# PacificBiosciences/pb-StarPhase

Measured on AMD Instinct MI355X. Metric: HiFi reads/sec diplotyped (HLA+CYP2D6), higher is better.
Workload: dtype int32; 1 GPU; BASELINE configs[1] + configs[2] as ONE sample per step: HLA-A/-B 10000 HiFi reads vs IMGT/HLA v0.14.1 (11,199 DNA alleles) + CYP2D6 2000 targeted reads (39 templates), the six configs[2] scenarios in turn; a new sample uploaded every step; reads -> diplotypes; hla_reads=10000, cyp2d6_reads=2000, cyp2d6_lanes=6, hla_lanes=2, cyp2d6_consensus=launch pairs

## Files before the change

pb-starphase_amd/csrc/sp_api.hip:

```cpp
#include "sp_internal.h"
#include <algorithm>
#include <thread>
#include <atomic>
#include <cstring>
#include <new>
#include <unistd.h>

extern "C" {

int32_t sp_abi_version(void) { return SP_ABI_VERSION; }

int32_t sp_device_count(int32_t* count) {
    int n = 0;
    hipError_t e = hipGetDeviceCount(&n);
    if (count) *count = (e == hipSuccess) ? n : 0;
    return e == hipSuccess ? SP_OK : SP_ERR_NO_DEVICE;
}

int32_t sp_ctx_create(int32_t device, void* stream, sp_ctx** out) {
    if (!out) return SP_ERR_INVALID_ARG;
    *out = nullptr;
    static std::atomic<int> effective{-1};
    bool by_library = false;
    if (effective.load() < 0) {
        bool hip_up = false;
        char link[64];
        for (int fd = 0; fd < 1024 && !hip_up; ++fd) {
            char path[64]; std::snprintf(path, sizeof path, "/proc/self/fd/%d", fd);
            const ssize_t k = readlink(path, link, sizeof link - 1);
            if (k > 0) { link[k] = 0; hip_up = std::strcmp(link, "/dev/kfd") == 0; }
        }
        const char* had = std::getenv("GPU_MAX_HW_QUEUES");
        if (!had && !hip_up) { (void)setenv("GPU_MAX_HW_QUEUES", "16", 0); by_library = true; }
        const char* now = std::getenv("GPU_MAX_HW_QUEUES");
        effective.store(now ? std::atoi(now) : (hip_up ? 0 : 4));
    }
    const int hw_queues = effective.load() > 0 ? effective.load() : 4;
    int n = 0;
    if (hipGetDeviceCount(&n) != hipSuccess || n <= 0 || device < 0 || device >= n) return SP_ERR_NO_DEVICE;
    if (hipSetDevice(device) != hipSuccess) return SP_ERR_NO_DEVICE;
    hipDeviceProp_t prop;
    if (hipGetDeviceProperties(&prop, device) != hipSuccess) return SP_ERR_NO_DEVICE;
    if (std::strncmp(prop.gcnArchName, "gfx950", 6) != 0) return SP_ERR_NO_DEVICE;
    sp_ctx* ctx = new (std::nothrow) sp_ctx();
    if (!ctx) return SP_ERR_OUT_OF_MEMORY;
    ctx->device = device;
    ctx->num_cus = prop.multiProcessorCount > 0 ? prop.multiProcessorCount : 256;
    static bool set_here = false;
    if (by_library) set_here = true;
    ctx->hw_queues = hw_queues; ctx->hw_queues_by_library = set_here;
    ctx->hw_queues_effective = effective.load();
    { const char* kc = std::getenv("SP_K8_COMPOUND"); if (kc && *kc) ctx->k8_compound = std::atoi(kc); }
    { const char* ks = std::getenv("SP_K8_SIDE_ORDERS"); if (ks && *ks) ctx->k8_side_orders = std::max(0, std::min(3, std::atoi(ks))); }
    { const char* kp = std::getenv("SP_K8_PERSISTENT"); if (kp && *kp) ctx->k8_persistent = std::atoi(kp); }
    if (effective.load() == 0)
        ctx->warning = "the HIP runtime was initialised before the library's first context and GPU_MAX_HW_QUEUES was not set: the process's streams share the runtime's 4 hardware queues; "
                       "export GPU_MAX_HW_QUEUES=16 (or more) before the process initialises HIP";
    else if (hw_queues < 16)
        ctx->warning = "GPU_MAX_HW_QUEUES=" + std::to_string(hw_queues) + ": the library's streams share " + std::to_string(hw_queues) +
                       " hardware queues; export GPU_MAX_HW_QUEUES=16 (or more) before the process initialises HIP";
    if (stream) { ctx->stream = (hipStream_t)stream; ctx->own_stream = false; }
    else {
        if (hipStreamCreateWithFlags(&ctx->stream, hipStreamNonBlocking) != hipSuccess) { delete ctx; return SP_ERR_HIP; }
        ctx->own_stream = true;
    }
    if (hipEventCreate(&ctx->ev0) != hipSuccess || hipEventCreate(&ctx->ev1) != hipSuccess) { delete ctx; return SP_ERR_HIP; }
    *out = ctx;
    return SP_OK;
}

int32_t sp_ctx_get_info(const sp_ctx* ctx, sp_ctx_info* out) {
    if (!ctx || !out) return SP_ERR_INVALID_ARG;
    std::memset(out, 0, sizeof *out);
    out->device = ctx->device; out->num_cus = ctx->num_cus; out->hw_queues = ctx->hw_queues; out->hw_queues_set_by_library = ctx->hw_queues_by_library ? 1 : 0;
    std::snprintf(out->warning, sizeof out->warning, "%s", ctx->warning.c_str());
    return SP_OK;
}

static int32_t upload_finish(sp_seqset* s);
void sp_ctx_destroy(sp_ctx* ctx) {
    if (!ctx) return;
    for (sp_ctx*& h : ctx->helper) if (h) { sp_ctx_destroy(h); h = nullptr; }
    hipSetDevice(ctx->device);
    if (ctx->uploading) (void)upload_finish(ctx->uploading);
    if (ctx->copy_stream) { hipStreamSynchronize(ctx->copy_stream); hipStreamDestroy(ctx->copy_stream); ctx->copy_stream = nullptr; }
    if (ctx->ctl_stream) { hipStreamSynchronize(ctx->ctl_stream); hipStreamDestroy(ctx->ctl_stream); ctx->ctl_stream = nullptr; }
    if (ctx->ev_fork) hipEventDestroy(ctx->ev_fork);
    if (ctx->ev_join) hipEventDestroy(ctx->ev_join);
    hipStreamSynchronize(ctx->stream);
    for (sp_seqset* s : ctx->live_sets) {
        for (void* p : { (void*)s->d_words, (void*)s->d_nplane, (void*)s->d_word_off, (void*)s->d_len, (void*)s->d_kcode, (void*)s->d_kpos, (void*)s->d_koff }) if (p) ctx->dev_cap.erase(p);
        s->ctx = nullptr;
    }
    for (auto& kv : ctx->dev_cap) (void)hipFree(kv.first);
    if (ctx->scratch) hipFree(ctx->scratch);
    for (auto& kv : ctx->pool) if (kv.second.first) hipFree(kv.second.first);
    for (auto& kv : ctx->host_pool) if (kv.second.first) hipHostFree(kv.second.first);
    sp_profile_flush(ctx);
    for (hipEvent_t e : ctx->prof_free) hipEventDestroy(e);
    if (ctx->ev0) hipEventDestroy(ctx->ev0);
    if (ctx->ev1) hipEventDestroy(ctx->ev1);
    if (ctx->own_stream && ctx->stream) hipStreamDestroy(ctx->stream);
    delete ctx;
}

}
sp_ctx* sp_ctx_helper(sp_ctx* ctx, int i) {
    if (i < 0 || i > 6) return nullptr;
    if (!ctx->helper[i] && sp_ctx_create(ctx->device, nullptr, &ctx->helper[i]) != SP_OK) ctx->helper[i] = nullptr;
    if (ctx->helper[i]) { ctx->helper[i]->profiling = ctx->profiling; ctx->helper[i]->k5_block_pairs = ctx->k5_block_pairs; ctx->helper[i]->k8_persistent = ctx->k8_persistent; ctx->helper[i]->k8_side_orders = ctx->k8_side_orders; ctx->helper[i]->k8_compound = ctx->k8_compound; ctx->helper[i]->k8_side_max_blocks = ctx->k8_side_max_blocks; ctx->helper[i]->mm2_rescore = ctx->mm2_rescore; ctx->helper[i]->profile_rescore_counts = ctx->profile_rescore_counts; ctx->helper[i]->k1_best_n = ctx->k1_best_n; }
    return ctx->helper[i];
}
void sp_profile_merge(sp_ctx* into, sp_ctx* from) {
    sp_profile_flush(from);
    for (auto& kv : from->prof) { ProfileEntry& e = into->prof[kv.first]; e.ms += kv.second.ms; e.launches += kv.second.launches; e.cells += kv.second.cells; }
    from->prof.clear();
}
extern "C" {

int32_t sp_struct_size(const char* name) {
    if (!name) return -1;
#define SP_SZ(T) if (std::strcmp(name, #T) == 0) return (int32_t)sizeof(T);
    SP_SZ(sp_ctx_info)
    SP_SZ(sp_pair)
    SP_SZ(sp_aln)
    SP_SZ(sp_hla_db_desc)
    SP_SZ(sp_hla_realign)
    SP_SZ(sp_k1_seed_hit)
    SP_SZ(sp_hla_best)
    SP_SZ(sp_chain_problem)
    SP_SZ(sp_chain_result)
    SP_SZ(sp_region_hit)
    SP_SZ(sp_cyp_problem)
    SP_SZ(sp_cyp_call)
    SP_SZ(sp_cyp_locus)
    SP_SZ(sp_cyp_gene_def)
    SP_SZ(sp_cyp_config)
    SP_SZ(sp_cyp_db_stats)
    SP_SZ(sp_variant_problem)
    SP_SZ(sp_variant_result)
    SP_SZ(sp_sv_definitions)
    SP_SZ(sp_cons_config)
    SP_SZ(sp_cons_result)
    SP_SZ(sp_cons_problem)
    SP_SZ(sp_cons_output)
    SP_SZ(sp_priority_problem)
    SP_SZ(sp_priority_job)
    SP_SZ(sp_hla_call_config)
    SP_SZ(sp_hla_call)
    SP_SZ(sp_diplotype_settings)
    SP_SZ(sp_sample_inputs)
    SP_SZ(sp_starphase_timing)
    SP_SZ(sp_cyp_read_mapping)
    SP_SZ(sp_database_metadata)
    SP_SZ(sp_database_stats)
    SP_SZ(sp_gene_region)
    SP_SZ(sp_variant_detail)
    SP_SZ(sp_bam_read)
    SP_SZ(sp_affine_opts)
    SP_SZ(sp_affine_aln)
    SP_SZ(sp_k1_seed_info)
    SP_SZ(sp_cyp_region_variants)
    SP_SZ(sp_chain_build_info)
    SP_SZ(sp_variant_gene_stats)
    SP_SZ(sp_vcf_allele)
    SP_SZ(sp_vcf_deletion)
    SP_SZ(sp_mapping_stats)
    SP_SZ(sp_hla_rev_hit)
    SP_SZ(sp_batch_options)
    SP_SZ(sp_starphase_batch_timing)
    SP_SZ(sp_hla_alleles_stats)
    SP_SZ(sp_hla_cfg_mapping)
    SP_SZ(sp_hla_cfg_gene)
    SP_SZ(sp_pileup_col)
    SP_SZ(sp_support_summary)
    SP_SZ(sp_support_entry)
    SP_SZ(sp_pileup_ins)
    SP_SZ(sp_support_hap)
    SP_SZ(sp_support_hap_head)
#undef SP_SZ
    return -1;
}

const char* sp_last_error(const sp_ctx* ctx) { return ctx ? ctx->err.c_str() : "null context"; }

int32_t sp_ctx_synchronize(sp_ctx* ctx) {
    if (!ctx) return SP_ERR_INVALID_ARG;
    SP_HIP_CHECK(ctx, hipStreamSynchronize(ctx->stream));
    return SP_OK;
}

int32_t sp_ctx_set_option(sp_ctx* ctx, const char* name, int64_t value) {
    if (!ctx || !name) return SP_ERR_INVALID_ARG;
    if (std::strcmp(name, "hla_split_genes") == 0) { ctx->split_genes = value != 0; return SP_OK; }
    if (std::strcmp(name, "k1_best_n") == 0) { if (value < 0 || value > 8) return sp_fail(ctx, SP_ERR_INVALID_ARG, "sp_ctx_set_option: k1_best_n is 0..8"); ctx->k1_best_n = (int)value; for (sp_ctx* h : ctx->helper) if (h) h->k1_best_n = ctx->k1_best_n; return SP_OK; }
    if (std::strcmp(name, "profile_rescore_counts") == 0) { ctx->profile_rescore_counts = value != 0; for (sp_ctx* h : ctx->helper) if (h) h->profile_rescore_counts = ctx->profile_rescore_counts; return SP_OK; }
    if (std::strcmp(name, "mm2_rescore") == 0) { ctx->mm2_rescore = (int)value; for (sp_ctx* h : ctx->helper) if (h) h->mm2_rescore = ctx->mm2_rescore; return SP_OK; }
    if (std::strcmp(name, "k8_side_orders") == 0) { if (value < 0 || value > 3) return sp_fail(ctx, SP_ERR_INVALID_ARG, "sp_ctx_set_option: k8_side_orders is 0 .. 3"); ctx->k8_side_orders = (int)value; for (sp_ctx* h : ctx->helper) if (h) h->k8_side_orders = ctx->k8_side_orders; return SP_OK; }
    if (std::strcmp(name, "k8_compound") == 0) { ctx->k8_compound = (int)value; for (sp_ctx* h : ctx->helper) if (h) h->k8_compound = ctx->k8_compound; return SP_OK; }
    if (std::strcmp(name, "k8_side_max_blocks") == 0) { if (value < 0) return sp_fail(ctx, SP_ERR_INVALID_ARG, "sp_ctx_set_option: k8_side_max_blocks >= 0"); ctx->k8_side_max_blocks = (int)value; for (sp_ctx* h : ctx->helper) if (h) h->k8_side_max_blocks = ctx->k8_side_max_blocks; return SP_OK; }
    if (std::strcmp(name, "k8_persistent") == 0) { if (value < 0 || value > 2) return sp_fail(ctx, SP_ERR_INVALID_ARG, "sp_ctx_set_option: k8_persistent is 0 (never), 1 (whenever a batch fits) or 2 (the library decides)"); ctx->k8_persistent = (int)value; ctx->k8_persist_backoff = 0; ctx->k8_persist_failures = 0; for (sp_ctx* h : ctx->helper) if (h) h->k8_persistent = ctx->k8_persistent; return SP_OK; }
    if (std::strcmp(name, "cons_retry_ladder") == 0) { ctx->cons_retry_ladder = value != 0; for (sp_ctx* h : ctx->helper) if (h) h->cons_retry_ladder = ctx->cons_retry_ladder; return SP_OK; }
    if (std::strcmp(name, "k5_block_pairs") == 0) { if (value < 0 || value > (1 << 20)) return sp_fail(ctx, SP_ERR_INVALID_ARG, "sp_ctx_set_option: k5_block_pairs is 0..1048576"); ctx->k5_block_pairs = (int)value; for (sp_ctx* h : ctx->helper) if (h) h->k5_block_pairs = ctx->k5_block_pairs; return SP_OK; }
    if (std::strcmp(name, "cyp_cohort_min_group") == 0) { if (value < 1 || value > 64) return sp_fail(ctx, SP_ERR_INVALID_ARG, "sp_ctx_set_option: cyp_cohort_min_group is 1..64"); ctx->cyp_cohort_min_group = (int)value; return SP_OK; }
    if (std::strcmp(name, "cyp_cohort_streams") == 0) { if (value < 1 || value > 8) return sp_fail(ctx, SP_ERR_INVALID_ARG, "sp_ctx_set_option: cyp_cohort_streams is 1..8"); ctx->cyp_cohort_streams = (int)value; return SP_OK; }
    if (std::strcmp(name, "hla_split_streams") == 0) { if (value < 1 || value > 4) return sp_fail(ctx, SP_ERR_INVALID_ARG, "sp_ctx_set_option: hla_split_streams is 1..4"); ctx->split_streams = (int)value; return SP_OK; }
    return sp_fail(ctx, SP_ERR_INVALID_ARG, std::string("sp_ctx_set_option: unknown option ") + name);
}

int32_t sp_profile_reset(sp_ctx* ctx) {
    if (!ctx) return SP_ERR_INVALID_ARG;
    for (sp_ctx* h : ctx->helper) if (h) sp_profile_reset(h);
    sp_profile_flush(ctx); ctx->prof.clear();
    unsigned long long* c = sp_counters(ctx);
    if (c) { hipSetDevice(ctx->device); hipMemsetAsync(c, 0, SPC_N * sizeof(unsigned long long), ctx->stream); }
    return SP_OK;
}

int32_t sp_profile_get(sp_ctx* ctx, const char* kernel, double* total_ms, uint64_t* launches, uint64_t* cells) {
    if (!ctx || !kernel) return SP_ERR_INVALID_ARG;
    sp_profile_flush(ctx);
    for (sp_ctx* h : ctx->helper) if (h) sp_profile_merge(ctx, h);
    static const struct { const char* name; int idx; } counters[] = {
        {"count:k1_cells_active", SPC_K1_ACTIVE}, {"count:k1_cells_executed", SPC_K1_EXECUTED}, {"count:k1_cells_resumed", SPC_K1_RESUMED},
        {"count:k1_cells_bytes", SPC_K1_BYTES}, {"count:cons_launches", SPC_CONS_LAUNCHES}, {"count:cons_columns", SPC_CONS_COLUMNS},
        {"count:dbg0", 6}, {"count:dbg1", 7}, {"count:dbg2", 8}, {"count:dbg3", 9}, {"count:dbg4", 10}, {"count:dbg5", 11}, {"count:dbg6", 12}, {"count:dbg7", 13} };
    for (const auto& c : counters) if (std::strcmp(kernel, c.name) == 0) {
        unsigned long long v = 0; unsigned long long* d = sp_counters(ctx);
        if (d) { hipSetDevice(ctx->device); if (hipMemcpyAsync(&v, d + c.idx, 8, hipMemcpyDeviceToHost, ctx->stream) != hipSuccess || hipStreamSynchronize(ctx->stream) != hipSuccess) return sp_fail(ctx, SP_ERR_HIP, "sp_profile_get: counter read failed"); }
        for (sp_ctx* h : ctx->helper) if (h) {
            unsigned long long hv = 0; unsigned long long* hd = sp_counters(h);
            if (hd && hipMemcpyAsync(&hv, hd + c.idx, 8, hipMemcpyDeviceToHost, h->stream) == hipSuccess && hipStreamSynchronize(h->stream) == hipSuccess) v += hv;
        }
        if (total_ms) *total_ms = 0.0;
        if (launches) *launches = 0;
        if (cells) *cells = v;
        return SP_OK;
    }
    if (std::strcmp(kernel, "pool:device") == 0) {
        uint64_t allocs = ctx->pool_allocs, bytes = ctx->scratch_bytes;
        for (const auto& b : ctx->pool) bytes += b.second.second;
        for (sp_ctx* h : ctx->helper) if (h) { allocs += h->pool_allocs; bytes += h->scratch_bytes; for (const auto& b : h->pool) bytes += b.second.second; }
        if (total_ms) *total_ms = 0.0;
        if (launches) *launches = allocs;
        if (cells) *cells = bytes;
        return SP_OK;
    }
    auto it = ctx->prof.find(kernel);
    ProfileEntry e; if (it != ctx->prof.end()) e = it->second;
    if (total_ms) *total_ms = e.ms;
    if (launches) *launches = e.launches;
    if (cells) *cells = e.cells;
    return SP_OK;
}


struct sp_upload {
    std::thread th;
    int32_t rc = SP_OK; std::string err;
    int format = SP_SEQ_ASCII;
    const uint8_t* src = nullptr; uint64_t src_bytes = 0;
    std::vector<uint64_t> rel;
    uint8_t* d_stage = nullptr; uint64_t* d_off = nullptr; uint32_t* d_flag = nullptr;
    uint8_t* ring = nullptr; size_t chunk = 0; int slots = 0;
    hipEvent_t slot_ev[4] = { nullptr, nullptr, nullptr, nullptr };
    size_t wbytes = 0;
};

static constexpr size_t UPLOAD_CHUNK = (size_t)8 << 20;
static constexpr int UPLOAD_SLOTS = 4;

static void upload_run(sp_seqset* s) {
    sp_upload* u = s->up; sp_ctx* ctx = s->ctx;
    hipStream_t st = ctx->copy_stream;
    auto bad = [&](hipError_t e, const char* what) { if (e != hipSuccess && u->rc == SP_OK) { u->rc = SP_ERR_HIP; u->err = std::string(what) + ": " + hipGetErrorString(e); } return e != hipSuccess; };
    if (bad(hipSetDevice(ctx->device), "hipSetDevice")) return;
    const uint32_t n = s->n;
    bad(hipMemcpyAsync(s->d_word_off, s->h_word_off.data(), ((size_t)n + 1) * sizeof(uint64_t), hipMemcpyHostToDevice, st), "offsets");
    if (n) bad(hipMemcpyAsync(s->d_len, s->h_len.data(), (size_t)n * sizeof(int32_t), hipMemcpyHostToDevice, st), "lengths");
    bad(hipMemsetAsync(s->d_words, 0, u->wbytes, st), "clear");
    if (u->src_bytes && u->rc == SP_OK) {
        bad(hipMemcpyAsync(u->d_off, u->rel.data(), ((size_t)n + 1) * 8, hipMemcpyHostToDevice, st), "staged offsets");
        bad(hipMemsetAsync(u->d_flag, 0, 4, st), "flag");
        int k = 0;
        for (uint64_t at = 0; at < u->src_bytes && u->rc == SP_OK; at += u->chunk, ++k) {
            const int slot = k % u->slots;
            const size_t len = (size_t)std::min<uint64_t>(u->chunk, u->src_bytes - at);
            if (k >= u->slots && bad(hipEventSynchronize(u->slot_ev[slot]), "staging slot")) break;
            std::memcpy(u->ring + (size_t)slot * u->chunk, u->src + at, len);
            if (bad(hipMemcpyAsync(u->d_stage + at, u->ring + (size_t)slot * u->chunk, len, hipMemcpyHostToDevice, st), "payload")) break;
            bad(hipEventRecord(u->slot_ev[slot], st), "staging event");
        }
        if (u->rc == SP_OK && sp_launch_pack_on(st, ctx->num_cus, u->format, u->d_stage, u->d_off, s->d_word_off, s->d_len, n, s->d_words, nullptr, u->d_flag) != SP_OK) { u->rc = SP_ERR_HIP; u->err = "pack kernel launch"; }
        uint32_t flag = 0;
        if (u->rc == SP_OK && u->format != SP_SEQ_PACKED2) {
            bad(hipMemcpyAsync(&flag, u->d_flag, 4, hipMemcpyDeviceToHost, st), "flag read");
            bad(hipStreamSynchronize(st), "upload");
            if (u->rc == SP_OK && flag) {
                s->has_n = true;
                if (!(s->d_nplane = (uint32_t*)sp_dev_alloc(ctx, u->wbytes))) { u->rc = SP_ERR_OUT_OF_MEMORY; u->err = "seqset nplane"; }
                else {
                    bad(hipMemsetAsync(s->d_nplane, 0, u->wbytes, st), "clear N plane");
                    if (sp_launch_pack_on(st, ctx->num_cus, u->format, u->d_stage, u->d_off, s->d_word_off, s->d_len, n, nullptr, s->d_nplane, u->d_flag) != SP_OK) { u->rc = SP_ERR_HIP; u->err = "pack kernel launch"; }
                }
            }
        }
    }
    bad(hipStreamSynchronize(st), "upload");
}

static int32_t upload_finish(sp_seqset* s) {
    sp_upload* u = s->up;
    if (!u) return s->up_rc == SP_OK ? SP_OK : sp_fail(s->ctx, s->up_rc, "seqset upload: " + s->up_err);
    if (u->th.joinable()) u->th.join();
    sp_ctx* ctx = s->ctx;
    if (ctx->uploading == s) ctx->uploading = nullptr;
    s->up_rc = u->rc; s->up_err = u->err;
    for (hipEvent_t e : u->slot_ev) if (e) hipEventDestroy(e);
    delete u; s->up = nullptr;
    return s->up_rc == SP_OK ? SP_OK : sp_fail(ctx, s->up_rc, "seqset upload: " + s->up_err);
}

static int32_t upload_start(sp_ctx* ctx, int32_t format, const void* data, const uint64_t* offsets, const uint32_t* lengths, uint32_t n, sp_seqset** out) {
    if (!ctx || !out || (n && (!data || !offsets)) || format < SP_SEQ_ASCII || format > SP_SEQ_PACKED2 || (format != SP_SEQ_ASCII && n && !lengths)) return SP_ERR_INVALID_ARG;
    *out = nullptr;
    hipSetDevice(ctx->device);
    if (ctx->uploading) (void)upload_finish(ctx->uploading);
    sp_seqset* s = new (std::nothrow) sp_seqset();
    if (!s) return sp_fail(ctx, SP_ERR_OUT_OF_MEMORY, "seqset");
    s->ctx = ctx; s->n = n;
    s->h_len.resize(n); s->h_word_off.resize((size_t)n + 1);
    uint64_t total_words = 0;
    const uint64_t per_byte = format == SP_SEQ_ASCII ? 1 : format == SP_SEQ_BAM4 ? 2 : 4;
    for (uint32_t i = 0; i < n; ++i) {
        if (offsets[i + 1] < offsets[i]) { delete s; return sp_fail(ctx, SP_ERR_INVALID_ARG, "seqset: offsets must not decrease"); }
        const uint64_t bytes = offsets[i + 1] - offsets[i];
        uint64_t len = lengths ? lengths[i] : bytes;
        if (len > bytes * per_byte) { delete s; return sp_fail(ctx, SP_ERR_INVALID_ARG, "seqset: a sequence is longer than its bytes"); }
        if (len > 65534) { len = 0; s->n_skipped += 1; }
        s->h_len[i] = (int32_t)len;
        s->max_len = std::max<int32_t>(s->max_len, (int32_t)len);
        s->h_word_off[i] = total_words;
        const uint64_t w = (len + 15) / 16 + 2;
        total_words += (w + 3) & ~3ull;
    }
    s->h_word_off[n] = total_words;
    { std::lock_guard<std::mutex> g(ctx->dev_cache_mu); ctx->live_sets.insert(s); }
    auto fail = [&](const char* what) { sp_seqset_free(s); return sp_fail(ctx, SP_ERR_OUT_OF_MEMORY, what); };
    const size_t wbytes = (total_words + SP_SEQ_PAD_WORDS) * sizeof(uint32_t);
    if (!(s->d_words = (uint32_t*)sp_dev_alloc(ctx, wbytes))) return fail("seqset words");
    if (!(s->d_word_off = (uint64_t*)sp_dev_alloc(ctx, ((size_t)n + 1) * sizeof(uint64_t)))) return fail("seqset offsets");
    if (!(s->d_len = (int32_t*)sp_dev_alloc(ctx, std::max<size_t>(1, n) * sizeof(int32_t)))) return fail("seqset lengths");
    if (!ctx->copy_stream && hipStreamCreateWithFlags(&ctx->copy_stream, hipStreamNonBlocking) != hipSuccess) { sp_seqset_free(s); return sp_fail(ctx, SP_ERR_HIP, "copy stream"); }
    sp_upload* u = new (std::nothrow) sp_upload();
    if (!u) return fail("seqset upload");
    s->up = u; u->format = format; u->wbytes = wbytes;
    const uint64_t src_bytes = n ? offsets[n] - offsets[0] : 0;
    u->src = (const uint8_t*)data + (n ? offsets[0] : 0); u->src_bytes = src_bytes;
    if (src_bytes) {
        u->rel.resize((size_t)n + 1);
        for (uint32_t i = 0; i <= n; ++i) u->rel[i] = offsets[i] - offsets[0];
        u->chunk = std::min<size_t>(UPLOAD_CHUNK, (size_t)((src_bytes + 4095) & ~4095ull));
        u->slots = UPLOAD_SLOTS;
        u->d_stage = (uint8_t*)sp_pool(ctx, "upload_ascii", src_bytes);
        u->d_off = (uint64_t*)sp_pool(ctx, "upload_off", ((size_t)n + 1) * 8);
        u->d_flag = (uint32_t*)sp_pool(ctx, "upload_flag", 4);
        u->ring = (uint8_t*)sp_host_pool(ctx, "upload_ring", UPLOAD_CHUNK * UPLOAD_SLOTS);
        if (!u->d_stage || !u->d_off || !u->d_flag || !u->ring) return fail("seqset staging");
        for (int k = 0; k < u->slots; ++k) if (hipEventCreateWithFlags(&u->slot_ev[k], hipEventDisableTiming) != hipSuccess) { sp_seqset_free(s); return sp_fail(ctx, SP_ERR_HIP, "staging events"); }
    }
    ctx->uploading = s;
    try { u->th = std::thread(upload_run, s); }
    catch (...) { ctx->uploading = nullptr; sp_seqset_free(s); return sp_fail(ctx, SP_ERR_OUT_OF_MEMORY, "seqset upload thread"); }
    *out = s;
    return SP_OK;
}

int32_t sp_seqset_upload_async(sp_ctx* ctx, int32_t format, const void* data, const uint64_t* offsets, const uint32_t* lengths, uint32_t n, sp_seqset** out) {
    return upload_start(ctx, format, data, offsets, lengths, n, out);
}

int32_t sp_seqset_wait(sp_seqset* s) {
    if (!s) return SP_ERR_INVALID_ARG;
    return upload_finish(s);
}

int32_t sp_seqset_upload_format(sp_ctx* ctx, int32_t format, const void* data, const uint64_t* offsets, const uint32_t* lengths, uint32_t n, sp_seqset** out) {
    const int32_t rc = upload_start(ctx, format, data, offsets, lengths, n, out);
    if (rc != SP_OK) return rc;
    const int32_t rc2 = upload_finish(*out);
    if (rc2 != SP_OK) { sp_seqset_free(*out); *out = nullptr; }
    return rc2;
}

int32_t sp_seqset_upload(sp_ctx* ctx, const char* bases, const uint64_t* offsets, uint32_t n, sp_seqset** out) {
    return sp_seqset_upload_format(ctx, SP_SEQ_ASCII, bases, offsets, nullptr, n, out);
}

}
static size_t dev_round(size_t bytes) {
    size_t g = 4096; while (g * 16 < bytes) g <<= 1;
    return (std::max<size_t>(bytes, 1) + g - 1) / g * g;
}
void* sp_dev_alloc(sp_ctx* ctx, size_t bytes) {
    const size_t want = dev_round(bytes);
    {
        std::lock_guard<std::mutex> g(ctx->dev_cache_mu);
        auto it = ctx->dev_cache.lower_bound(want);
        if (it != ctx->dev_cache.end() && it->first <= 2 * want) { void* p = it->second; ctx->dev_cache_bytes -= it->first; ctx->dev_cache.erase(it); return p; }
    }
    void* p = nullptr;
    if (hipMalloc(&p, want) != hipSuccess) {
        std::vector<void*> idle;
        { std::lock_guard<std::mutex> g(ctx->dev_cache_mu); for (auto& kv : ctx->dev_cache) { idle.push_back(kv.second); ctx->dev_cap.erase(kv.second); } ctx->dev_cache.clear(); ctx->dev_cache_bytes = 0; }
        for (void* q : idle) (void)hipFree(q);
        if (hipMalloc(&p, want) != hipSuccess) return nullptr;
    }
    std::lock_guard<std::mutex> g(ctx->dev_cache_mu);
    ctx->dev_cap[p] = want;
    return p;
}
void sp_dev_release(sp_ctx* ctx, void* p) {
    if (!p) return;
    constexpr size_t MAX_BYTES = (size_t)2 << 30, MAX_BUFFERS = 4096;
    {
        std::lock_guard<std::mutex> g(ctx->dev_cache_mu);
        auto it = ctx->dev_cap.find(p);
        if (it == ctx->dev_cap.end()) { (void)hipFree(p); return; }
        if (ctx->dev_cache.size() < MAX_BUFFERS && ctx->dev_cache_bytes + it->second <= MAX_BYTES) { ctx->dev_cache.emplace(it->second, p); ctx->dev_cache_bytes += it->second; return; }
        ctx->dev_cap.erase(it);
    }
    (void)hipFree(p);
}
extern "C" {

int32_t sp_seqset_skipped(const sp_seqset* s, uint32_t* n_skipped) { if (!s || !n_skipped) return SP_ERR_INVALID_ARG; *n_skipped = s->n_skipped; return SP_OK; }

void sp_seqset_free(sp_seqset* s) {
    if (!s) return;
    if (s->ctx) hipSetDevice(s->ctx->device);
    if (s->up) { (void)upload_finish(s); }
    if (s->ctx) {
        (void)hipStreamSynchronize(s->ctx->stream);
        { std::lock_guard<std::mutex> g(s->ctx->dev_cache_mu); s->ctx->live_sets.erase(s); }
        sp_dev_release(s->ctx, s->d_words); sp_dev_release(s->ctx, s->d_nplane); sp_dev_release(s->ctx, s->d_word_off); sp_dev_release(s->ctx, s->d_len);
        sp_dev_release(s->ctx, s->d_kcode); sp_dev_release(s->ctx, s->d_kpos); sp_dev_release(s->ctx, s->d_koff);
    } else {
        if (s->d_words) hipFree(s->d_words);
        if (s->d_nplane) hipFree(s->d_nplane);
        if (s->d_word_off) hipFree(s->d_word_off);
        if (s->d_len) hipFree(s->d_len);
        if (s->d_kcode) hipFree(s->d_kcode);
        if (s->d_kpos) hipFree(s->d_kpos);
        if (s->d_koff) hipFree(s->d_koff);
    }
    delete s;
}

int32_t sp_seqset_count(const sp_seqset* s, uint32_t* n) { if (!s || !n) return SP_ERR_INVALID_ARG; *n = s->n; return SP_OK; }
int32_t sp_seqset_length(const sp_seqset* s, uint32_t idx, uint32_t* len) {
    if (!s || !len || idx >= s->n) return SP_ERR_INVALID_ARG;
    *len = (uint32_t)s->h_len[idx]; return SP_OK;
}

}

void sp_profile_flush(sp_ctx* ctx) {
    for (auto& p : ctx->prof_pending) {
        hipEventSynchronize(p.e1);
        float ms = 0; hipEventElapsedTime(&ms, p.e0, p.e1);
        auto& e = ctx->prof[p.name]; e.ms += ms; e.launches += 1; e.cells += p.cells;
        ctx->prof_free.push_back(p.e0); ctx->prof_free.push_back(p.e1);
    }
    ctx->prof_pending.clear();
}

int sp_seqset_build_index(sp_ctx* ctx, sp_seqset* s);
static void kmer_tables(const sp_seqset* s, std::vector<uint64_t>& koff, std::vector<uint32_t>& kcode, std::vector<int32_t>& kpos);

int sp_seqset_fetch_host(sp_ctx* ctx, sp_seqset* s) {
    if (!s->h_words.empty()) return SP_OK;
    hipSetDevice(ctx->device);
    const size_t plane_words = (size_t)s->h_word_off[s->n] + SP_SEQ_PAD_WORDS;
    s->h_words.assign(plane_words * (s->has_n ? 2 : 1), 0);
    if (hipMemcpy(s->h_words.data(), s->d_words, plane_words * 4, hipMemcpyDeviceToHost) != hipSuccess) return sp_fail(ctx, SP_ERR_HIP, "fetch packed words");
    if (s->has_n && hipMemcpy(s->h_words.data() + plane_words, s->d_nplane, plane_words * 4, hipMemcpyDeviceToHost) != hipSuccess) return sp_fail(ctx, SP_ERR_HIP, "fetch N plane");
    return SP_OK;
}

int sp_seqset_make_small(sp_ctx* ctx, const char* prefix, const char* bases, const uint64_t* offsets, uint32_t n, bool with_index, sp_seqset* out) {
    hipSetDevice(ctx->device);
    *out = sp_seqset();
    sp_seqset& s = *out;
    s.ctx = ctx; s.n = n;
    s.h_len.resize(n); s.h_word_off.resize((size_t)n + 1);
    uint64_t total_words = 0;
    for (uint32_t i = 0; i < n; ++i) {
        const uint64_t len = offsets[i + 1] - offsets[i];
        if (offsets[i + 1] < offsets[i] || len > 65534) return sp_fail(ctx, SP_ERR_TOO_LONG, "seqset: sequence longer than 65,534 bases");
        s.h_len[i] = (int32_t)len; s.max_len = std::max<int32_t>(s.max_len, (int32_t)len);
        s.h_word_off[i] = total_words;
        total_words += (((len + 15) / 16 + 2) + 3) & ~3ull;
    }
    s.h_word_off[n] = total_words;
    const size_t plane_words = (size_t)total_words + SP_SEQ_PAD_WORDS;
    std::vector<uint32_t> words(plane_words, 0), nplane(plane_words, 0);
    std::atomic<bool> any_n(false);
    auto pack_one = [&](uint32_t i) {
        const char* src = bases + offsets[i];
        uint32_t* w = words.data() + s.h_word_off[i]; uint32_t* np = nplane.data() + s.h_word_off[i];
        for (int b = 0; b < s.h_len[i]; ++b) {
            uint32_t c = 0;
            switch (src[b]) { case 'A': case 'a': c = 0; break; case 'C': case 'c': c = 1; break; case 'G': case 'g': c = 2; break; case 'T': case 't': c = 3; break;
                              default: np[b >> 4] |= 1u << ((b & 15) << 1); any_n.store(true, std::memory_order_relaxed); }
            w[b >> 4] |= c << ((b & 15) << 1);
        }
    };
    const uint32_t pack_threads = n >= 32 ? std::min<uint32_t>(8, std::max<uint32_t>(1, std::thread::hardware_concurrency())) : 1;
    if (pack_threads > 1) {
        std::vector<std::thread> pool;
        for (uint32_t t = 0; t < pack_threads; ++t) pool.emplace_back([&, t]() { for (uint32_t i = t; i < n; i += pack_threads) pack_one(i); });
        for (auto& th : pool) th.join();
    } else for (uint32_t i = 0; i < n; ++i) pack_one(i);
    s.has_n = any_n.load();
    s.h_words = words;
    if (s.has_n) s.h_words.insert(s.h_words.end(), nplane.begin(), nplane.end());
    std::vector<uint64_t> koff; std::vector<uint32_t> kcode; std::vector<int32_t> kpos;
    if (with_index) kmer_tables(&s, koff, kcode, kpos);
    auto up16 = [](size_t x) { return (x + 15) & ~(size_t)15; };
    const size_t b_words = plane_words * 4, b_npl = s.has_n ? plane_words * 4 : 0, b_off = ((size_t)n + 1) * 8, b_len = std::max<size_t>(1, n) * 4;
    const size_t b_kc = with_index ? std::max<size_t>(1, kcode.size()) * 4 : 0, b_kp = with_index ? std::max<size_t>(1, kpos.size()) * 4 : 0;
    const size_t b_ko = with_index ? koff.size() * 8 : 0;
    const size_t o_words = 0, o_npl = o_words + up16(b_words), o_off = o_npl + up16(b_npl), o_len = o_off + up16(b_off);
    const size_t o_kc = o_len + up16(b_len), o_kp = o_kc + up16(b_kc), o_ko = o_kp + up16(b_kp), total = o_ko + up16(b_ko);
    const std::string px(prefix);
    char* dev = (char*)sp_pool(ctx, (px + "_all").c_str(), total);
    char* stage = (char*)sp_host_pool(ctx, (px + "_stage").c_str(), total);
    if (!dev || !stage) return sp_fail(ctx, SP_ERR_OUT_OF_MEMORY, "small seqset");
    std::memcpy(stage + o_words, words.data(), b_words);
    if (s.has_n) std::memcpy(stage + o_npl, nplane.data(), b_npl);
    std::memcpy(stage + o_off, s.h_word_off.data(), b_off);
    if (n) std::memcpy(stage + o_len, s.h_len.data(), (size_t)n * 4);
    if (with_index) {
        if (!kcode.empty()) { std::memcpy(stage + o_kc, kcode.data(), kcode.size() * 4); std::memcpy(stage + o_kp, kpos.data(), kpos.size() * 4); }
        std::memcpy(stage + o_ko, koff.data(), b_ko);
    }
    s.d_words = (uint32_t*)(dev + o_words);
    s.d_nplane = s.has_n ? (uint32_t*)(dev + o_npl) : nullptr;
    s.d_word_off = (uint64_t*)(dev + o_off);
    s.d_len = (int32_t*)(dev + o_len);
    if (with_index) { s.d_kcode = (uint32_t*)(dev + o_kc); s.d_kpos = (int32_t*)(dev + o_kp); s.d_koff = (uint64_t*)(dev + o_ko); s.has_index = true; }
    hipMemcpyAsync(dev, stage, total, hipMemcpyHostToDevice, ctx->stream);
    SP_HIP_CHECK(ctx, hipStreamSynchronize(ctx->stream));
    return SP_OK;
}

std::string sp_seqset_decode(sp_ctx* ctx, const sp_seqset* s, uint32_t i) {
    if (sp_seqset_fetch_host(ctx, const_cast<sp_seqset*>(s)) != SP_OK || i >= s->n) return std::string();
    const size_t plane_words = (size_t)s->h_word_off[s->n] + SP_SEQ_PAD_WORDS;
    const uint32_t* w = s->h_words.data() + s->h_word_off[i];
    const uint32_t* np = s->has_n ? s->h_words.data() + plane_words + s->h_word_off[i] : nullptr;
    std::string out((size_t)s->h_len[i], 'N');
    for (int h = 0; h < s->h_len[i]; ++h) {
        const uint32_t sh = (uint32_t)(h & 15) << 1;
        if (np && ((np[h >> 4] >> sh) & 1u)) continue;
        out[h] = "ACGT"[(w[h >> 4] >> sh) & 3u];
    }
    return out;
}

static void kmer_tables(const sp_seqset* s, std::vector<uint64_t>& koff, std::vector<uint32_t>& kcode, std::vector<int32_t>& kpos) {
    const size_t plane_words = (size_t)s->h_word_off[s->n] + SP_SEQ_PAD_WORDS;
    koff.assign((size_t)s->n + 1, 0); kcode.clear(); kpos.clear();
    std::vector<std::vector<uint32_t>> codes(s->n); std::vector<std::vector<int32_t>> poss(s->n);
    auto one = [&](uint32_t i) {
        std::vector<uint32_t>& c0 = codes[i]; std::vector<int32_t>& p0 = poss[i];
        std::vector<uint32_t> c1; std::vector<int32_t> p1;
        const uint32_t* w = s->h_words.data() + s->h_word_off[i];
        const uint32_t* np = s->has_n ? s->h_words.data() + plane_words + s->h_word_off[i] : nullptr;
        const int len = s->h_len[i];
        for (int j = 0; j + SP_KMER <= len; ++j) {
            const int wi = j >> 4; const int sh = (j & 15) << 1;
            auto fetch = [&](const uint32_t* p) -> uint32_t {
                uint64_t v = ((uint64_t)p[wi + 1] << 32) | p[wi];
                return (uint32_t)(v >> sh);
            };
            if (np && fetch(np)) continue;
            c0.push_back(fetch(w)); p0.push_back(j);
        }
        const size_t m = c0.size();
        c1.resize(m); p1.resize(m);
        for (int pass = 0; pass < 3; ++pass) {
            const int shift = pass * 11; const uint32_t mask = pass == 2 ? 0x3FFu : 0x7FFu;
            uint32_t count[2049] = {0};
            for (size_t x = 0; x < m; ++x) ++count[((c0[x] >> shift) & mask) + 1];
            for (int b = 0; b < 2048; ++b) count[b + 1] += count[b];
            for (size_t x = 0; x < m; ++x) { const uint32_t at = count[(c0[x] >> shift) & mask]++; c1[at] = c0[x]; p1[at] = p0[x]; }
            c0.swap(c1); p0.swap(p1);
        }
    };
    const uint32_t n_threads = s->n >= 32 ? std::min<uint32_t>(8, std::max<uint32_t>(1, std::thread::hardware_concurrency())) : 1;
    if (n_threads > 1) {
        std::vector<std::thread> pool;
        for (uint32_t t = 0; t < n_threads; ++t) pool.emplace_back([&, t]() { for (uint32_t i = t; i < s->n; i += n_threads) one(i); });
        for (auto& th : pool) th.join();
    } else for (uint32_t i = 0; i < s->n; ++i) one(i);
    size_t total = 0;
    for (uint32_t i = 0; i < s->n; ++i) { koff[i] = total; total += codes[i].size(); }
    koff[s->n] = total;
    kcode.resize(total); kpos.resize(total);
    for (uint32_t i = 0; i < s->n; ++i) if (!codes[i].empty()) {
        std::memcpy(kcode.data() + koff[i], codes[i].data(), codes[i].size() * 4); std::memcpy(kpos.data() + koff[i], poss[i].data(), poss[i].size() * 4);
    }
}

int sp_seqset_build_index(sp_ctx* ctx, sp_seqset* s) {
    if (s->has_index) return SP_OK;
    hipSetDevice(ctx->device);
    const size_t plane_words = (size_t)s->h_word_off[s->n] + SP_SEQ_PAD_WORDS;
    if (s->h_words.empty()) {
        s->h_words.assign(plane_words * (s->has_n ? 2 : 1), 0);
        hipMemcpy(s->h_words.data(), s->d_words, plane_words * 4, hipMemcpyDeviceToHost);
        if (s->has_n) hipMemcpy(s->h_words.data() + plane_words, s->d_nplane, plane_words * 4, hipMemcpyDeviceToHost);
    }
    std::vector<uint64_t> koff; std::vector<uint32_t> kcode; std::vector<int32_t> kpos;
    kmer_tables(s, koff, kcode, kpos);
    size_t ne = std::max<size_t>(1, kcode.size());
    sp_ctx* owner = s->ctx ? s->ctx : ctx;
    s->d_kcode = (uint32_t*)sp_dev_alloc(owner, ne * 4); s->d_kpos = (int32_t*)sp_dev_alloc(owner, ne * 4); s->d_koff = (uint64_t*)sp_dev_alloc(owner, koff.size() * 8);
    if (!s->d_kcode || !s->d_kpos || !s->d_koff)
        return sp_fail(ctx, SP_ERR_OUT_OF_MEMORY, "k-mer index");
    if (!kcode.empty()) {
        hipMemcpy(s->d_kcode, kcode.data(), kcode.size() * 4, hipMemcpyHostToDevice);
        hipMemcpy(s->d_kpos, kpos.data(), kpos.size() * 4, hipMemcpyHostToDevice);
    }
    hipMemcpy(s->d_koff, koff.data(), koff.size() * 8, hipMemcpyHostToDevice);
    s->has_index = true;
    return SP_OK;
}

extern "C" {

int32_t sp_anchor_batch_topk(sp_ctx* ctx, const sp_seqset* A, const sp_seqset* B,
                             const uint32_t* a_idx, const uint32_t* b_idx, uint64_t n_pairs, int32_t topk,
                             int32_t* diag_out, int32_t* votes_out) {
    if (!ctx || !A || !B || (n_pairs && (!a_idx || !b_idx || !diag_out || !votes_out))) return SP_ERR_INVALID_ARG;
    if (topk < 1 || topk > 8) return sp_fail(ctx, SP_ERR_INVALID_ARG, "anchor: topk must be 1..8");
    if (n_pairs == 0) return SP_OK;
    hipSetDevice(ctx->device);
    for (uint64_t i = 0; i < n_pairs; ++i) if (a_idx[i] >= A->n || b_idx[i] >= B->n) return sp_fail(ctx, SP_ERR_INVALID_ARG, "anchor: index out of range");
    int rc = sp_seqset_build_index(ctx, const_cast<sp_seqset*>(A));
    if (rc) return rc;
    const size_t nb = n_pairs * 4, nbk = nb * (size_t)topk;
    uint32_t* d_a = (uint32_t*)sp_pool(ctx, "anchor_a", nb); uint32_t* d_b = (uint32_t*)sp_pool(ctx, "anchor_b", nb);
    int32_t* d_d = (int32_t*)sp_pool(ctx, "anchor_d", nbk); int32_t* d_v = (int32_t*)sp_pool(ctx, "anchor_v", nbk);
    if (!d_a || !d_b || !d_d || !d_v) return sp_fail(ctx, SP_ERR_OUT_OF_MEMORY, "anchor buffers");
    hipMemcpyAsync(d_a, a_idx, nb, hipMemcpyHostToDevice, ctx->stream);
    hipMemcpyAsync(d_b, b_idx, nb, hipMemcpyHostToDevice, ctx->stream);
    rc = sp_launch_anchor(ctx, A, B, d_a, d_b, n_pairs, d_d, d_v, topk);
    if (rc == SP_OK) {
        hipMemcpyAsync(diag_out, d_d, nbk, hipMemcpyDeviceToHost, ctx->stream);
        hipMemcpyAsync(votes_out, d_v, nbk, hipMemcpyDeviceToHost, ctx->stream);
        if (hipStreamSynchronize(ctx->stream) != hipSuccess) rc = sp_fail(ctx, SP_ERR_HIP, "anchor: stream sync failed");
    }
    return rc;
}

int32_t sp_anchor_batch(sp_ctx* ctx, const sp_seqset* A, const sp_seqset* B,
                        const uint32_t* a_idx, const uint32_t* b_idx, uint64_t n_pairs,
                        int32_t* diag_out, int32_t* votes_out) {
    return sp_anchor_batch_topk(ctx, A, B, a_idx, b_idx, n_pairs, 1, diag_out, votes_out);
}

int32_t sp_align_batch(sp_ctx* ctx, const sp_seqset* A, const sp_seqset* B,
                       const sp_pair* pairs, uint64_t n_pairs,
                       sp_aln* out, uint32_t* events, uint32_t events_stride) {
    if (!ctx || !A || !B || (n_pairs && (!pairs || !out))) return SP_ERR_INVALID_ARG;
    if (events && (events_stride == 0 || events_stride > SP_MAX_ED)) return sp_fail(ctx, SP_ERR_INVALID_ARG, "align: events_stride must be 1..SP_MAX_ED");
    if (n_pairs == 0) return SP_OK;
    hipSetDevice(ctx->device);
    std::vector<CellDesc> cells(n_pairs);
    for (uint64_t i = 0; i < n_pairs; ++i) {
        if (pairs[i].a >= A->n || pairs[i].b >= B->n) return sp_fail(ctx, SP_ERR_INVALID_ARG, "align: index out of range");
        if (pairs[i].max_ed < 0 || pairs[i].max_ed > SP_MAX_ED) return sp_fail(ctx, SP_ERR_INVALID_ARG, "align: max_ed must be 0..SP_MAX_ED");
        cells[i] = CellDesc{pairs[i].a, pairs[i].b, pairs[i].diag, pairs[i].max_ed, 0, -1};
    }
    CellDesc* d_cells = (CellDesc*)sp_pool(ctx, "align_cells", n_pairs * sizeof(CellDesc)); sp_aln* d_out = (sp_aln*)sp_pool(ctx, "align_out", n_pairs * sizeof(sp_aln));
    uint32_t* d_ev = events ? (uint32_t*)sp_pool(ctx, "align_ev", n_pairs * (size_t)events_stride * 4) : nullptr;
    int rc = SP_OK;
    if (!d_cells || !d_out || (events && !d_ev)) {
        rc = sp_fail(ctx, SP_ERR_OUT_OF_MEMORY, "align buffers");
    } else {
        hipMemcpyAsync(d_cells, cells.data(), n_pairs * sizeof(CellDesc), hipMemcpyHostToDevice, ctx->stream);
        if (events) hipMemsetAsync(d_ev, 0, n_pairs * (size_t)events_stride * 4, ctx->stream);
        rc = sp_launch_cells(ctx, A, B, d_cells, n_pairs, d_out, d_ev, events_stride, events ? "align_trace" : "align", 2);
        if (rc == SP_OK) {
            hipMemcpyAsync(out, d_out, n_pairs * sizeof(sp_aln), hipMemcpyDeviceToHost, ctx->stream);
            if (events) hipMemcpyAsync(events, d_ev, n_pairs * (size_t)events_stride * 4, hipMemcpyDeviceToHost, ctx->stream);
            if (hipStreamSynchronize(ctx->stream) != hipSuccess) rc = sp_fail(ctx, SP_ERR_HIP, std::string("align: ") + hipGetErrorString(hipGetLastError()));
        }
    }
    return rc;
}

}
```

pb-starphase_amd/csrc/sp_hla_seed.hip:

```cpp
#include <cstring>
#include <cstdio>
#include "sp_internal.h"
#include <rocprim/rocprim.hpp>
#include <algorithm>
#include <cmath>

#ifndef SP_DP_EXP
#define SP_DP_EXP 0
#endif
namespace {

constexpr int MZ_K = 19, MZ_W = 19;
constexpr uint64_t MZ_MASK = (1ull << (2 * MZ_K)) - 1;
constexpr int MIN_MID_OCC = 50, MAX_MID_OCC = 500, MAX_MAX_OCC = 4095;
constexpr float MID_OCC_FRAC = 2e-4f;
constexpr int CH_MAX_GAP = 10000, CH_BW = 500, CH_MAX_SKIP = 25, CH_MAX_ITER = 5000, CH_MIN_CNT = 3, CH_MIN_SCORE = 40;
constexpr float MASK_LEVEL = 0.5f, PRI_RATIO = 0.8f;
constexpr int MIN_DP_MAX = 200;

constexpr int BUCKET_BITS = 18;
constexpr uint64_t H_PAL = 1ull << 40;
constexpr uint64_t H_NONE = ~0ull;
constexpr int TILE = 1024, HALO = MZ_W - 1;
constexpr int SEL_CAP = SP_K1_SEL;
constexpr int PRIM_CAP = 64;

struct IndexView {
    const uint64_t* keys; const uint32_t* start; const uint32_t* occ; const uint32_t* bucket;
    uint32_t n_keys; int32_t mid_occ; uint32_t n_seqs;
};

__host__ __device__ __forceinline__ uint64_t mix64(uint64_t key) {
    key = (~key + (key << 21)) & MZ_MASK;
    key = key ^ key >> 24;
    key = ((key + (key << 3)) + (key << 8)) & MZ_MASK;
    key = key ^ key >> 14;
    key = ((key + (key << 2)) + (key << 4)) & MZ_MASK;
    key = key ^ key >> 28;
    key = (key + (key << 31)) & MZ_MASK;
    return key;
}
__device__ __forceinline__ uint64_t rev_digits(uint64_t v) {
    v = ((v >> 2) & 0x3333333333333333ull) | ((v & 0x3333333333333333ull) << 2);
    v = ((v >> 4) & 0x0F0F0F0F0F0F0F0Full) | ((v & 0x0F0F0F0F0F0F0F0Full) << 4);
    return __builtin_bswap64(v);
}
__device__ __forceinline__ uint64_t bits38(const uint32_t* __restrict__ w, int start) {
    const int wi = start >> 4, sh = (start & 15) << 1;
    const uint64_t lo = (uint64_t)w[wi] | ((uint64_t)w[wi + 1] << 32);
    uint64_t e = lo >> sh;
    if (sh) e |= (uint64_t)w[wi + 2] << (64 - sh);
    return e & MZ_MASK;
}
__device__ __forceinline__ uint64_t kmer_hash(const uint32_t* __restrict__ w, const uint32_t* __restrict__ np, int len, int i, uint8_t& z) {
    z = 0;
    if (i < MZ_K - 1 || i >= len) return H_NONE;
    const int start = i - (MZ_K - 1);
    if (np && bits38(np, start)) return H_NONE;
    const uint64_t e = bits38(w, start);
    const uint64_t fw = rev_digits(e) >> (64 - 2 * MZ_K), rv = (~e) & MZ_MASK;
    if (fw == rv) return H_PAL;
    z = fw < rv ? 0 : 1;
    return mix64(z ? rv : fw);
}
__device__ __forceinline__ bool is_minimizer(const uint64_t* __restrict__ h, int c) {
    const uint64_t hp = h[c];
    if (hp >= H_PAL) return false;
    int l = 0; bool lb = false;
    for (; l < HALO; ++l) { const uint64_t v = h[c - 1 - l]; if (v == H_NONE) { lb = true; break; } if (v < hp) break; }
    int r = 0; bool rb = false, tie = false;
    for (; r < HALO; ++r) { const uint64_t v = h[c + 1 + r]; if (v == H_NONE) { rb = true; break; } if (v < hp) break; if (v == hp) tie = true; }
    if (l + r >= MZ_W - 1) return true;
    return lb && rb && !tie;
}
#ifndef SP_MZ_QUICK
#define SP_MZ_QUICK 5
#endif
constexpr int MZ_QUICK = SP_MZ_QUICK;
__device__ __forceinline__ void tile_minimizers(const uint64_t* __restrict__ h, int lo, int len, uint8_t* __restrict__ mzf, uint16_t* __restrict__ cand, uint32_t* __restrict__ n_cand) {
    if (threadIdx.x == 0) *n_cand = 0;
    __syncthreads();
    for (int j = threadIdx.x; j < TILE; j += 256) {
        const int c = HALO + j;
        const uint64_t hp = h[c];
        uint8_t f = 0;
        if (lo + j < len && hp < H_PAL) {
            int l = MZ_QUICK, r = MZ_QUICK; bool lb = false, rb = false, tie = false;
#pragma unroll
            for (int x = MZ_QUICK - 1; x >= 0; --x) {
                const uint64_t vl = h[c - 1 - x], vr = h[c + 1 + x];
                if (vl == H_NONE) { l = x; lb = true; } else if (vl < hp) { l = x; lb = false; }
                if (vr == H_NONE) { r = x; rb = true; } else if (vr < hp) { r = x; rb = false; }
            }
            if (l < MZ_QUICK && r < MZ_QUICK) {
                if (lb && rb) { for (int x = 0; x < r; ++x) tie |= h[c + 1 + x] == hp; f = tie ? 0 : 1; }
            } else cand[atomicAdd(n_cand, 1u)] = (uint16_t)c;
        }
        mzf[j] = f;
    }
    __syncthreads();
    const uint32_t nc = *n_cand;
    for (uint32_t i = threadIdx.x; i < nc; i += 256) { const int c = cand[i]; mzf[c - HALO] = is_minimizer(h, c) ? 1 : 0; }
    __syncthreads();
}
__device__ __forceinline__ uint32_t block_rank(bool flag, uint32_t* wave_tot, uint32_t& total) {
    const unsigned long long b = __ballot(flag);
    const int lane = threadIdx.x & 63, wave = threadIdx.x >> 6, nw = blockDim.x >> 6;
    const uint32_t within = (uint32_t)__builtin_popcountll(b & ((1ull << lane) - 1ull));
    __syncthreads();
    if (lane == 0) wave_tot[wave] = (uint32_t)__builtin_popcountll(b);
    __syncthreads();
    uint32_t base = 0, tot = 0;
    for (int x = 0; x < nw; ++x) { const uint32_t c = wave_tot[x]; if (x < wave) base += c; tot += c; }
    total = tot;
    return base + within;
}
__device__ __forceinline__ void index_lookup(const IndexView& ix, uint64_t hash, uint32_t& st, uint32_t& n) {
    const uint32_t b = (uint32_t)(hash >> (2 * MZ_K - BUCKET_BITS));
    uint32_t lo = ix.bucket[b], hi = ix.bucket[b + 1];
    while (lo < hi) { const uint32_t mid = (lo + hi) >> 1; if (ix.keys[mid] < hash) lo = mid + 1; else hi = mid; }
    if (lo < ix.n_keys && lo < ix.bucket[b + 1] && ix.keys[lo] == hash) { st = ix.start[lo]; n = ix.start[lo + 1] - st; } else { st = 0; n = 0; }
}

template <bool FILL>
__global__ __launch_bounds__(256) void mz_sketch_kernel(SeqSetView S, const uint32_t* __restrict__ seq_of, uint32_t n, uint32_t* __restrict__ cnt, const uint64_t* __restrict__ off,
                                                        uint64_t* __restrict__ keys, uint32_t* __restrict__ occ) {
    __shared__ uint64_t h[TILE + 2 * HALO];
    __shared__ uint8_t zs[TILE + 2 * HALO];
    __shared__ uint8_t mzf[TILE];
    __shared__ uint16_t cand[TILE];
    __shared__ uint32_t wave_tot[4], n_cand;
    const uint32_t rid = blockIdx.x;
    if (rid >= n) return;
    const uint32_t s = seq_of ? seq_of[rid] : rid;
    const int len = S.len[s];
    const uint32_t* w = S.words + S.word_off[s];
    const uint32_t* np = S.nplane ? S.nplane + S.word_off[s] : nullptr;
    uint32_t running = 0;
    for (int lo = 0; lo < len; lo += TILE) {
        __syncthreads();
        for (int c = threadIdx.x; c < TILE + 2 * HALO; c += 256) { uint8_t z; h[c] = kmer_hash(w, np, len, lo - HALO + c, z); zs[c] = z; }
        __syncthreads();
        tile_minimizers(h, lo, len, mzf, cand, &n_cand);
        for (int j = 0; j < TILE; j += 256) {
            const int c = HALO + j + (int)threadIdx.x, pos = lo + j + (int)threadIdx.x;
            const bool flag = pos < len && mzf[j + (int)threadIdx.x] != 0;
            uint32_t total;
            const uint32_t rk = block_rank(flag, wave_tot, total);
            if (FILL && flag) {
                keys[off[rid] + running + rk] = h[c];
                occ[off[rid] + running + rk] = rid << 17 | (uint32_t)pos << 1 | zs[c];
            }
            running += total;
        }
    }
    if (!FILL && threadIdx.x == 0) cnt[rid] = running;
}

struct SeedCounters { unsigned long long seeds, anchors; uint32_t max_anchors, max_seeds, overflow_reads, seed_overflow, rev_selected, wide_cells; unsigned long long t[8]; };
#ifdef SP_K1S_TIMING
#define K1S_T(i) do { if (threadIdx.x == 0) { const unsigned long long now_ = wall_clock64(); atomicAdd(&ctr->t[i], now_ - t_last); t_last = now_; } } while (0)
#else
#define K1S_T(i) do { } while (0)
#endif
#ifdef SP_K1S_TIMING
#define K1S_TW(i) do { if (lane == 0) { const unsigned long long now_ = wall_clock64(); atomicAdd(&ctr->t[i], now_ - t_last); t_last = now_; } } while (0)
#else
#define K1S_TW(i) do { } while (0)
#endif

__global__ __launch_bounds__(256) void k1s_seed_kernel(SeqSetView reads, IndexView ix, uint32_t n_reads, int sd_cap, uint4* __restrict__ seeds, uint32_t seed_cap,
                                                       uint2* __restrict__ read_seed, uint32_t* __restrict__ read_anchors, SeedCounters* __restrict__ ctr) {
    extern __shared__ uint32_t lds[];
    uint64_t* h = reinterpret_cast<uint64_t*>(lds);
    uint32_t* sd_q = lds + 2 * (TILE + 2 * HALO);
    uint32_t* sd_st = sd_q + sd_cap;
    uint16_t* sd_n = reinterpret_cast<uint16_t*>(sd_st + sd_cap);
    uint8_t* zs = reinterpret_cast<uint8_t*>(sd_n + sd_cap);
    uint8_t* keep = zs + TILE + 2 * HALO + 8;
    __shared__ uint32_t wave_tot[4], s_sum[4], n_cand;
    __shared__ unsigned long long s_base;
    __shared__ uint8_t mzf[TILE];
    __shared__ uint16_t cand[TILE];
    const uint32_t r = blockIdx.x;
    if (r >= n_reads) return;
    const int len = reads.len[r];
    const uint32_t* w = reads.words + reads.word_off[r];
    const uint32_t* np = reads.nplane ? reads.nplane + reads.word_off[r] : nullptr;
    uint32_t ns = 0; bool over = false;
    for (int lo = 0; lo < len; lo += TILE) {
        __syncthreads();
        for (int c = threadIdx.x; c < TILE + 2 * HALO; c += 256) { uint8_t z; h[c] = kmer_hash(w, np, len, lo - HALO + c, z); zs[c] = z; }
        __syncthreads();
        tile_minimizers(h, lo, len, mzf, cand, &n_cand);
        for (int j = 0; j < TILE; j += 256) {
            const int c = HALO + j + (int)threadIdx.x, pos = lo + j + (int)threadIdx.x;
            bool flag = pos < len && mzf[j + (int)threadIdx.x] != 0;
            uint32_t st = 0, n = 0;
            if (flag) { index_lookup(ix, h[c], st, n); flag = n > 0; }
            uint32_t total;
            const uint32_t rk = block_rank(flag, wave_tot, total);
            if (flag && ns + rk < (uint32_t)sd_cap) { sd_q[ns + rk] = (uint32_t)pos << 1 | zs[c]; sd_st[ns + rk] = st; sd_n[ns + rk] = (uint16_t)(n > 0xFFFFu ? 0xFFFFu : n); }
            if (ns + total > (uint32_t)sd_cap) over = true;
            ns += total;
        }
    }
    if (over) ns = (uint32_t)sd_cap;
    __syncthreads();
    const int max_occ = ix.mid_occ;
    for (uint32_t j = threadIdx.x; j < ns; j += 256) {
        const uint32_t nj = sd_n[j];
        uint8_t k = 1;
        if ((int)nj > max_occ) {
            int a = (int)j - 1; while (a >= 0 && (int)sd_n[a] > max_occ) --a;
            uint32_t b = j + 1; while (b < ns && (int)sd_n[b] > max_occ) ++b;
            const int ps = a < 0 ? 0 : (int)(sd_q[a] >> 1), pe = b == ns ? len : (int)(sd_q[b] >> 1);
            int kp = (2 * (pe - ps) + 499) / 1000;
            if (kp > 128) kp = 128;
            k = 0;
            if (kp > 0 && nj <= (uint32_t)MAX_MAX_OCC) {
                int rank = 0;
                for (uint32_t x = (uint32_t)(a + 1); x < b && rank < kp; ++x) { const uint32_t nx = sd_n[x]; if (nx < nj || (nx == nj && x < j)) ++rank; }
                k = rank < kp ? 1 : 0;
            }
        }
        keep[j] = k;
    }
    __syncthreads();
    uint32_t kept = 0, mine = 0;
    for (uint32_t j = threadIdx.x; j < ns; j += 256) if (keep[j]) { ++kept; mine += sd_n[j]; }
    for (int o = 32; o > 0; o >>= 1) { kept += __shfl_xor(kept, o); mine += __shfl_xor(mine, o); }
    __syncthreads();
    if ((threadIdx.x & 63) == 0) { wave_tot[threadIdx.x >> 6] = kept; s_sum[threadIdx.x >> 6] = mine; }
    __syncthreads();
    kept = wave_tot[0] + wave_tot[1] + wave_tot[2] + wave_tot[3];
    const uint32_t tot = s_sum[0] + s_sum[1] + s_sum[2] + s_sum[3];
    __syncthreads();
    if (threadIdx.x == 0) s_base = kept ? atomicAdd(&ctr->seeds, (unsigned long long)kept) : 0ull;
    __syncthreads();
    const unsigned long long base = s_base;
    const bool fits = base + kept <= seed_cap;
    uint32_t done = 0;
    for (uint32_t j0 = 0; j0 < ns && fits; j0 += 256) {
        const uint32_t j = j0 + threadIdx.x;
        const bool flag = j < ns && keep[j];
        uint32_t total;
        const uint32_t rk = block_rank(flag, wave_tot, total);
        if (flag) seeds[base + done + rk] = make_uint4(sd_q[j], sd_st[j], sd_n[j], 0u);
        done += total;
    }
    if (threadIdx.x == 0) {
        read_seed[r] = fits ? make_uint2((uint32_t)base, kept) : make_uint2(0u, 0u);
        read_anchors[r] = fits ? tot : 0u;
        if (fits && tot) { atomicAdd(&ctr->anchors, (unsigned long long)tot); atomicMax(&ctr->max_anchors, tot); atomicMax(&ctr->max_seeds, kept); }
        if (over) atomicAdd(&ctr->overflow_reads, 1u);
        if (!fits) atomicAdd(&ctr->seed_overflow, 1u);
    }
}

struct SChain { int32_t score, f_end; uint32_t key, end, first, cnt; };
struct SGroup { uint32_t read, key, off, cnt; };
struct SSel { int32_t rid, rev, score, cnt, diag, qs, qe, rs, re, n_chains; };
struct SDp { uint32_t key; int32_t f; int16_t p; uint16_t t; };

constexpr int CH_THREADS = 256;
constexpr int WIN_KEYS = 12288;

__device__ __forceinline__ int32_t chain_sc(uint32_t ai, uint32_t aj, const int32_t* __restrict__ pen) {
    const int32_t dq = (int32_t)(ai & 0xFFFFu) - (int32_t)(aj & 0xFFFFu);
    if (dq <= 0 || dq > CH_MAX_GAP) return INT32_MIN;
    const int32_t dr = (int32_t)(ai >> 16) - (int32_t)(aj >> 16);
    if (dr == 0) return INT32_MIN;
    const int32_t dd = dr > dq ? dr - dq : dq - dr;
    if (dd > CH_BW) return INT32_MIN;
    const int32_t dg = dr < dq ? dr : dq;
    int32_t sc = MZ_K < dg ? MZ_K : dg;
    if (dd || dg > MZ_K) sc -= pen[dd];
    return sc;
}

__device__ __forceinline__ uint32_t block_scan(uint32_t v, uint32_t* wave_tot, uint32_t& total) {
    uint32_t incl = v;
    for (int o = 1; o < 64; o <<= 1) { const uint32_t t = __shfl_up(incl, o); if ((int)(threadIdx.x & 63) >= o) incl += t; }
    __syncthreads();
    if ((threadIdx.x & 63) == 63) wave_tot[threadIdx.x >> 6] = incl;
    __syncthreads();
    uint32_t base = 0, tot = 0;
    for (int wv = 0; wv < CH_THREADS / 64; ++wv) { const uint32_t c = wave_tot[wv]; if (wv < (int)(threadIdx.x >> 6)) base += c; tot += c; }
    total = tot;
    return base + incl;
}

__device__ __forceinline__ int block_argmax(bool have, unsigned long long k1, unsigned long long k2, int idx, unsigned long long* r1, unsigned long long* r2, int* ri) {
    for (int o = 32; o > 0; o >>= 1) {
        const bool oh = __shfl_xor((int)have, o) != 0;
        const unsigned long long o1 = __shfl_xor(k1, o), o2 = __shfl_xor(k2, o); const int oi = __shfl_xor(idx, o);
        if (oh && (!have || o1 > k1 || (o1 == k1 && o2 > k2))) { have = true; k1 = o1; k2 = o2; idx = oi; }
    }
    __syncthreads();
    if ((threadIdx.x & 63) == 0) { const int wv = threadIdx.x >> 6; r1[wv] = k1; r2[wv] = k2; ri[wv] = have ? idx : -1; }
    __syncthreads();
    int best = -1; unsigned long long b1 = 0, b2 = 0;
    for (int wv = 0; wv < CH_THREADS / 64; ++wv) if (ri[wv] >= 0 && (best < 0 || r1[wv] > b1 || (r1[wv] == b1 && r2[wv] > b2))) { best = ri[wv]; b1 = r1[wv]; b2 = r2[wv]; }
    return best;
}

__device__ __forceinline__ void chain_interval(const SChain& c, int qlen, int& qs, int& qe, int& rs, int& re) {
    rs = (int)(c.first >> 16) + 1 - MZ_K; re = (int)(c.end >> 16) + 1;
    const int s = (int)(c.first & 0xFFFFu) + 1 - MZ_K, e = (int)(c.end & 0xFFFFu) + 1;
    if (c.key >> 15) { qs = qlen - e; qe = qlen - s; } else { qs = s; qe = e; }
}

struct BatchCursors { unsigned long long groups_anchors; uint32_t chains, dp_chunk, big_items, big_members, big_chunk, pad; };
struct SBigItem { SGroup g; uint32_t member_off, n_members, pad0, pad1; };
struct SMember { uint32_t read, key, shift, pad; };

__global__ __launch_bounds__(CH_THREADS) void k1s_group_kernel(SeqSetView reads, IndexView ix, uint32_t r0, uint32_t n_batch, const uint4* __restrict__ seeds, const uint2* __restrict__ read_seed,
                                                               uint32_t* __restrict__ anchors, uint32_t anchor_cap, SGroup* __restrict__ groups, uint32_t group_cap,
                                                               uint3* __restrict__ read_chain, BatchCursors* __restrict__ cur, SeedCounters* __restrict__ ctr) {
    extern __shared__ uint32_t tab[];
    __shared__ uint32_t s_hist[256], s_hista[256], s_first[256];
    __shared__ uint32_t s_scan[CH_THREADS / 64];
    __shared__ unsigned long long s_base;
    const int tid = threadIdx.x;
    const uint32_t r = r0 + blockIdx.x;
    if (blockIdx.x >= n_batch) return;
    const uint2 rs_ = read_seed[r];
    const uint32_t s0 = rs_.x, K = rs_.y;
    const int qlen = reads.len[r];
    uint32_t n_groups_read = 0, n_anchors_read = 0;
    unsigned long long t_last = 0;
#ifdef SP_K1S_TIMING
    t_last = wall_clock64();
#endif
    (void)t_last;
    bool any_rev = false;
    for (int rev = 0; rev < 2 && K; ++rev) {
        if (rev == 1 && !any_rev) break;
        for (uint32_t rid_lo = 0; rid_lo < ix.n_seqs; rid_lo += WIN_KEYS) {
            const uint32_t rid_hi = rid_lo + WIN_KEYS < ix.n_seqs ? rid_lo + WIN_KEYS : ix.n_seqs, W = rid_hi - rid_lo;
            __syncthreads();
            for (uint32_t i = tid; i < W; i += CH_THREADS) tab[i] = 0;
            __syncthreads();
            uint32_t other = 0;
            for (uint32_t s = 0; s < K; ++s) {
                const uint4 sd = seeds[s0 + s];
                const uint32_t strand = sd.x & 1u;
                for (uint32_t k = tid; k < sd.z; k += CH_THREADS) {
                    const uint32_t o = ix.occ[sd.y + k], rid = o >> 17;
                    if (rid < rid_lo || rid >= rid_hi) continue;
                    if ((int)((o & 1u) != strand) == rev) atomicAdd(&tab[rid - rid_lo], 1u); else ++other;
                }
            }
            if (rev == 0) any_rev |= __syncthreads_or(other != 0) != 0; else __syncthreads();
            K1S_T(0);
            const uint32_t per = (W + CH_THREADS - 1) / CH_THREADS, lo = (uint32_t)tid * per, hi = lo + per < W ? lo + per : W;
            s_hist[tid] = 0; s_hista[tid] = 0;
            __syncthreads();
            uint32_t my_g = 0;
            for (uint32_t i = lo; i < hi; ++i) { const uint32_t c = tab[i]; if (c >= (uint32_t)CH_MIN_CNT) { ++my_g; const uint32_t k = 255 - (c > 255 ? 255 : c); atomicAdd(&s_hist[k], 1u); atomicAdd(&s_hista[k], c); } }
            __syncthreads();
            uint32_t tot_a, tot_g;
            {
                const uint32_t vg = s_hist[tid], va = s_hista[tid];
                const uint32_t ig = block_scan(vg, s_scan, tot_g), ia = block_scan(va, s_scan, tot_a);
                __syncthreads();
                s_hist[tid] = ig - vg; s_hista[tid] = ia - va; s_first[tid] = ig - vg;
                __syncthreads();
            }
            (void)my_g;
            if (tot_g == 0) { K1S_T(1); continue; }
            if (tid == 0) s_base = atomicAdd(&cur->groups_anchors, (unsigned long long)tot_g << 32 | tot_a);
            __syncthreads();
            const unsigned long long base = s_base;
            const uint32_t base_g = (uint32_t)(base >> 32), base_a = (uint32_t)base;
            const bool fits = (unsigned long long)base_a + tot_a <= anchor_cap && (unsigned long long)base_g + tot_g <= group_cap;
            if (!fits) { if (tid == 0) atomicAdd(&ctr->overflow_reads, 1u); continue; }
            for (uint32_t i = lo; i < hi; ++i) {
                const uint32_t c = tab[i];
                if (c < (uint32_t)CH_MIN_CNT) { tab[i] = 0xFFFFFFFFu; continue; }
                const uint32_t k = 255 - (c > 255 ? 255 : c);
                const uint32_t slot = atomicAdd(&s_hist[k], 1u);
                const uint32_t a_off = base_a + (c < 255 ? s_hista[k] + (slot - s_first[k]) * c : atomicAdd(&s_hista[k], c));
                SGroup g; g.read = r; g.key = (uint32_t)rev << 15 | (rid_lo + i); g.off = a_off; g.cnt = c;
                groups[base_g + slot] = g;
                tab[i] = a_off;
            }
            __syncthreads();
            K1S_T(1);
            for (uint32_t s = 0; s < K; ++s) {
                const uint4 sd = seeds[s0 + s];
                const uint32_t strand = sd.x & 1u, qpos = sd.x >> 1;
                const uint32_t qp = rev ? (uint32_t)(qlen - ((int)qpos + 1 - MZ_K) - 1) : qpos;
                for (uint32_t k = tid; k < sd.z; k += CH_THREADS) {
                    const uint32_t o = ix.occ[sd.y + k], rid = o >> 17;
                    if ((int)((o & 1u) != strand) == rev && rid >= rid_lo && rid < rid_hi && tab[rid - rid_lo] != 0xFFFFFFFFu) {
                        const uint32_t slot = atomicAdd(&tab[rid - rid_lo], 1u);
                        anchors[slot] = ((o >> 1) & 0xFFFFu) << 16 | (qp & 0xFFFFu);
                    }
                }
            }
            __syncthreads();
            K1S_T(2);
            n_groups_read += tot_g; n_anchors_read += tot_a;
            K1S_T(3);
        }
    }
    if (tid == 0) {
        const uint32_t cap = n_groups_read ? n_anchors_read / CH_MIN_CNT : 0u;
        const uint32_t off = cap ? atomicAdd(&cur->chains, cap) : 0u;
        read_chain[r] = make_uint3(off, cap, 0u);
    }
}

constexpr int DP_REG_MAX = 26;
constexpr int DP_BIG_MAX = 4096;
constexpr int DP_BIG_WORDS = 3 * DP_BIG_MAX;
constexpr int DP_WAVE_WORDS = DP_REG_MAX * 32 * 2;

template <int N> __device__ __forceinline__ void sort_network(uint32_t (&k)[N]) {
#pragma unroll
    for (int size = 2; size <= N; size <<= 1) {
#pragma unroll
        for (int stride = size >> 1; stride > 0; stride >>= 1) {
#pragma unroll
            for (int i = 0; i < N; ++i) {
                const int l = i ^ stride;
                if (l > i) {
                    const bool up = (i & size) == 0;
                    const uint32_t a = k[i], b = k[l];
                    const uint32_t lo = a < b ? a : b, hi = a < b ? b : a;
                    k[i] = up ? lo : hi; k[l] = up ? hi : lo;
                }
            }
        }
    }
}
template <int N> __device__ __forceinline__ uint32_t pick_key(const uint32_t (&k)[N], int idx) {
    uint32_t v = k[0];
#pragma unroll
    for (int i = 1; i < N; ++i) v = idx == i ? k[i] : v;
    return v;
}

__device__ __forceinline__ void emit_chains(bool have, const SGroup& grp, int sc, int zf, uint32_t end_key, uint32_t first_key, int cnt, SChain* __restrict__ chains, uint32_t chain_cap,
                                            uint3* __restrict__ read_chain, int lane) {
    unsigned long long todo = __ballot(have);
    while (todo) {
        const int leader = __builtin_ctzll(todo);
        const uint32_t r0 = (uint32_t)__builtin_amdgcn_readlane((int)grp.read, leader);
        const unsigned long long same = __ballot(have && grp.read == r0);
        uint32_t base = 0;
        if (lane == leader) base = atomicAdd(&read_chain[r0].z, (uint32_t)__builtin_popcountll(same));
        base = (uint32_t)__builtin_amdgcn_readlane((int)base, leader);
        if (have && grp.read == r0) {
            const uint3 rc = read_chain[r0];
            const uint32_t at = base + (uint32_t)__builtin_popcountll(same & ((1ull << lane) - 1ull));
            if (at < rc.y && rc.x + at < chain_cap) { SChain c; c.score = sc; c.f_end = zf; c.key = grp.key; c.end = end_key; c.first = first_key; c.cnt = (uint32_t)cnt; chains[rc.x + at] = c; }
        }
        todo &= ~same;
    }
}

template <int NS, int ND>
__device__ __forceinline__ void dp_in_registers(const SGroup& grp, int n, const uint32_t* __restrict__ anchors, const int32_t* __restrict__ pen, uint32_t* __restrict__ wl, int lane,
                                                SChain* __restrict__ chains, uint32_t chain_cap, uint3* __restrict__ read_chain) {
    uint32_t k[NS];
#pragma unroll
    for (int i = 0; i < NS; ++i) k[i] = i < n ? anchors[grp.off + i] : 0xFFFFFFFFu;
#if SP_DP_EXP == 1
    if (k[0] == 12345u) wl[lane] = k[NS - 1];
    return;
#endif
    sort_network<NS>(k);
#if SP_DP_EXP == 2
    if (k[0] == 12345u) wl[lane] = k[NS - 1];
    return;
#endif
    int f[ND]; int p[ND];
#pragma unroll
    for (int i = 0; i < ND; ++i) {
        int fi = MZ_K, pi = 0xFF;
        const int ri = (int)(k[i] >> 16), qi = (int)(k[i] & 0xFFFFu);
#pragma unroll
        for (int j = i - 1; j >= 0; --j) {
            const int dq = qi - (int)(k[j] & 0xFFFFu), dr = ri - (int)(k[j] >> 16);
            const int dd = dr > dq ? dr - dq : dq - dr, dg = dr < dq ? dr : dq;
            const bool ok = dq > 0 && dq <= CH_MAX_GAP && dr != 0 && dr <= CH_MAX_GAP && dd <= CH_BW;
            const int cand = f[j] + (MZ_K < dg ? MZ_K : dg) - pen[dd <= CH_BW ? dd : 0];
            const bool better = ok && cand > fi;
            fi = better ? cand : fi; pi = better ? j : pi;
        }
        f[i] = fi; p[i] = pi;
        if (i < n) wl[i * 64 + lane] = (uint32_t)fi << 8 | (uint32_t)pi;
    }
#if SP_DP_EXP == 3
    return;
#endif
    auto F = [&](int i) { return (int)((wl[i * 64 + lane] >> 8) & 0xFFFFu); };
    auto P = [&](int i) { const int v = (int)(wl[i * 64 + lane] & 0xFFu); return v == 0xFF ? -1 : v; };
    auto T = [&](int i) { return (int)(wl[i * 64 + lane] >> 24); };
    auto setT = [&](int i, int t) { wl[i * 64 + lane] = (wl[i * 64 + lane] & 0x00FFFFFFu) | (uint32_t)t << 24; };
    bool active = n > 0;
    while (__ballot(active)) {
        bool have = false; int sc = 0, zf = 0, cnt = 0; uint32_t end_key = 0, first_key = 0;
        if (active) {
            int zi = -1;
            for (int i = 0; i < n; ++i) { const uint32_t v = wl[i * 64 + lane]; const int fi = (int)((v >> 8) & 0xFFFFu); if ((v >> 24) == 0 && fi >= CH_MIN_SCORE && (zi < 0 || fi >= zf)) { zi = i; zf = fi; } }
            if (zi < 0) active = false;
            else {
                int i = zi, end_i = -1, max_i = zi, max_s = 0;
                do {
                    setT(i, 2); end_i = i = P(i);
                    const int s2 = i < 0 ? zf : zf - F(i);
                    if (s2 > max_s) { max_s = s2; max_i = i; }
                    else if (max_s - s2 > CH_BW) break;
                } while (i >= 0 && (T(i) & 3) == 0);
                for (i = zi; i >= 0 && i != end_i; i = P(i)) setT(i, 0);
                end_i = max_i;
                int first = zi;
                for (i = zi; i != end_i; i = P(i)) { setT(i, 1); first = i; ++cnt; }
                sc = i < 0 ? zf : zf - F(i);
                if (cnt == 0) setT(zi, 4);
                have = sc >= CH_MIN_SCORE && cnt >= CH_MIN_CNT;
                if (have) { end_key = pick_key<NS>(k, zi); first_key = pick_key<NS>(k, first); }
            }
        }
        emit_chains(have, grp, sc, zf, end_key, first_key, cnt, chains, chain_cap, read_chain, lane);
    }
}

__device__ __forceinline__ void wave_sync_lds() {
    __builtin_amdgcn_fence(__ATOMIC_RELEASE, "wavefront");
    __builtin_amdgcn_wave_barrier();
    __builtin_amdgcn_fence(__ATOMIC_ACQUIRE, "wavefront");
}
__device__ __forceinline__ void dp_in_lds_rows(const SGroup& grp, int n, int mx, const uint32_t* __restrict__ anchors, const int32_t* __restrict__ pen, unsigned long long* __restrict__ wl, int lane,
                                               SChain* __restrict__ chains, uint32_t chain_cap, uint3* __restrict__ read_chain) {
    uint32_t k[32];
#pragma unroll
    for (int i = 0; i < 32; ++i) k[i] = i < n ? anchors[grp.off + i] : 0xFFFFFFFFu;
    sort_network<32>(k);
    const int n_all = n, col = lane & 31;
    for (int half = 0; half < 2; ++half) {
    n = (lane >> 5) == half ? n_all : 0;
#pragma unroll
    for (int i = 0; i < DP_REG_MAX; ++i) if (i < n) wl[i * 32 + col] = k[i];
    for (int i = 0; i < mx; ++i) {
        if (i >= n) continue;
        const uint32_t ki = (uint32_t)wl[i * 32 + col];
        const int ri = (int)(ki >> 16), qi = (int)(ki & 0xFFFFu);
        int fi = MZ_K, pi = 0xFF;
#pragma unroll 4
        for (int j = i - 1; j >= 0; --j) {
            const unsigned long long e = wl[j * 32 + col];
            const int dq = qi - (int)((uint32_t)e & 0xFFFFu), dr = ri - (int)((uint32_t)e >> 16);
            const int dd = dr > dq ? dr - dq : dq - dr, dg = dr < dq ? dr : dq;
            const bool ok = dq > 0 && dq <= CH_MAX_GAP && dr != 0 && dr <= CH_MAX_GAP && dd <= CH_BW;
            const int cand = (int)((e >> 32) & 0xFFFFu) + (MZ_K < dg ? MZ_K : dg) - pen[dd <= CH_BW ? dd : 0];
            const bool better = ok && cand > fi;
            fi = better ? cand : fi; pi = better ? j : pi;
        }
        wl[i * 32 + col] = (unsigned long long)ki | (unsigned long long)fi << 32 | (unsigned long long)pi << 48;
    }
    auto F = [&](int i) { return (int)((wl[i * 32 + col] >> 32) & 0xFFFFu); };
    auto P = [&](int i) { const int v = (int)((wl[i * 32 + col] >> 48) & 0xFFu); return v == 0xFF ? -1 : v; };
    auto T = [&](int i) { return (int)(wl[i * 32 + col] >> 56); };
    auto setT = [&](int i, int t) { wl[i * 32 + col] = (wl[i * 32 + col] & 0x00FFFFFFFFFFFFFFull) | (unsigned long long)t << 56; };
    bool active = n > 0;
    while (__ballot(active)) {
        bool have = false; int sc = 0, zf = 0, cnt = 0; uint32_t end_key = 0, first_key = 0;
        if (active) {
            int zi = -1;
            for (int i = 0; i < n; ++i) { const unsigned long long v = wl[i * 32 + col]; const int fi = (int)((v >> 32) & 0xFFFFu); if ((v >> 56) == 0 && fi >= CH_MIN_SCORE && (zi < 0 || fi >= zf)) { zi = i; zf = fi; } }
            if (zi < 0) active = false;
            else {
                int i = zi, end_i = -1, max_i = zi, max_s = 0;
                do {
                    setT(i, 2); end_i = i = P(i);
                    const int s2 = i < 0 ? zf : zf - F(i);
                    if (s2 > max_s) { max_s = s2; max_i = i; }
                    else if (max_s - s2 > CH_BW) break;
                } while (i >= 0 && (T(i) & 3) == 0);
                for (i = zi; i >= 0 && i != end_i; i = P(i)) setT(i, 0);
                end_i = max_i;
                int first = zi;
                for (i = zi; i != end_i; i = P(i)) { setT(i, 1); first = i; ++cnt; }
                sc = i < 0 ? zf : zf - F(i);
                if (cnt == 0) setT(zi, 4);
                have = sc >= CH_MIN_SCORE && cnt >= CH_MIN_CNT;
                if (have) { end_key = (uint32_t)wl[zi * 32 + col]; first_key = (uint32_t)wl[first * 32 + col]; }
            }
        }
        emit_chains(have, grp, sc, zf, end_key, first_key, cnt, chains, chain_cap, read_chain, lane);
    }
    wave_sync_lds();
    }
}

template <int CTRL, int ROW_MASK> __device__ __forceinline__ int dpp_move(int fill, int src) { return __builtin_amdgcn_update_dpp(fill, src, CTRL, ROW_MASK, 0xf, false); }
__device__ __forceinline__ int wave_prefix_max(int v) {
    const int NEG = INT32_MIN;
    int t;
    t = dpp_move<0x111, 0xf>(NEG, v); v = t > v ? t : v;
    t = dpp_move<0x112, 0xf>(NEG, v); v = t > v ? t : v;
    t = dpp_move<0x114, 0xf>(NEG, v); v = t > v ? t : v;
    t = dpp_move<0x118, 0xf>(NEG, v); v = t > v ? t : v;
    t = dpp_move<0x142, 0xa>(NEG, v); v = t > v ? t : v;
    t = dpp_move<0x143, 0xc>(NEG, v); v = t > v ? t : v;
    return v;
}
__device__ __forceinline__ void wave_prefix_maps(int& a, int& b) {
    const int NEG = -(1 << 20);
#define SP_MAP_STEP(CTRL, MASK) { const int ta = dpp_move<CTRL, MASK>(0, a), tb = dpp_move<CTRL, MASK>(NEG, b); const int nb = tb + a > b ? tb + a : b; a = ta + a; b = nb; }
    SP_MAP_STEP(0x111, 0xf) SP_MAP_STEP(0x112, 0xf) SP_MAP_STEP(0x114, 0xf) SP_MAP_STEP(0x118, 0xf) SP_MAP_STEP(0x142, 0xa) SP_MAP_STEP(0x143, 0xc)
#undef SP_MAP_STEP
}

__device__ __forceinline__ void wave_sync() {
    __builtin_amdgcn_fence(__ATOMIC_RELEASE, "wavefront");
    __builtin_amdgcn_wave_barrier();
    __builtin_amdgcn_fence(__ATOMIC_ACQUIRE, "wavefront");
}

__device__ __forceinline__ void dp_by_wave(const SGroup& grp, SDp* __restrict__ a, const uint32_t* __restrict__ anchors, const int32_t* __restrict__ pen,
                                           SChain* __restrict__ chains, uint32_t chain_cap, uint3* __restrict__ read_chain, int lane, SeedCounters* __restrict__ ctr,
                                           bool member, const SGroup& mine, uint32_t shift) {
    const int n = (int)grp.cnt;
    unsigned long long t_last = 0;
#ifdef SP_K1S_TIMING
    t_last = wall_clock64();
#endif
    (void)t_last; (void)ctr;
    for (int i = lane; i < n; i += 64) a[i].key = anchors[grp.off + i];
    wave_sync();
    for (int i = lane; i < n; i += 64) { const uint32_t kx = a[i].key; int rk = 0; for (int j = 0; j < n; ++j) rk += a[j].key < kx ? 1 : 0; a[i].f = rk; }
    wave_sync();
    for (int i = lane; i < n; i += 64) { uint32_t* dst = reinterpret_cast<uint32_t*>(&a[a[i].f].p); *dst = a[i].key; }
    wave_sync();
    for (int i = lane; i < n; i += 64) { a[i].key = *reinterpret_cast<uint32_t*>(&a[i].p); }
    wave_sync();
    for (int i = lane; i < n; i += 64) { a[i].t = 0; a[i].p = -1; a[i].f = 0; }
    wave_sync();
    int st = 0, max_ii = -1;
    for (int i = 0; i < n; ++i) {
        const uint32_t ai = a[i].key; const int ri = (int)(ai >> 16);
        while (st < i && ri > (int)(a[st].key >> 16) + CH_MAX_GAP) ++st;
        if (i - st > CH_MAX_ITER) st = i - CH_MAX_ITER;
        int max_f = MZ_K, max_j = -1, n_skip = 0, end_j = st - 1;
        for (int jb = i - 1; jb >= st; jb -= 64) {
            const int j = jb - lane;
            const bool in = j >= st;
            SDp aj; aj.key = 0; aj.f = 0; aj.p = -1; aj.t = 0;
            if (in) aj = a[j];
            int32_t sc = in ? chain_sc(ai, aj.key, pen) : INT32_MIN;
            const bool valid = sc != INT32_MIN;
            const int v = valid ? sc + aj.f : INT32_MIN;
            if (valid && aj.p >= 0) a[aj.p].t = (uint16_t)(i + 1);
            wave_sync();
            const bool marked = in && a[j].t == (uint16_t)(i + 1);
            int before = dpp_move<0x138, 0xf>(INT32_MIN, wave_prefix_max(v));
            before = before > max_f ? before : max_f;
            const bool isnew = valid && v > before;
            int ca = isnew ? -1 : (valid && marked ? 1 : 0), cb = isnew ? 0 : -(1 << 20);
            wave_prefix_maps(ca, cb);
            const int n_after = n_skip + ca > cb ? n_skip + ca : cb;
            const unsigned long long brk = __ballot(valid && !isnew && marked && n_after > CH_MAX_SKIP);
            const int lb = brk ? __builtin_ctzll(brk) : 64;
            const unsigned long long news = __ballot(isnew) & (lb >= 63 ? ~0ull : ((2ull << lb) - 1ull));
            if (news) { const int ln = 63 - __builtin_clzll(news); max_f = __builtin_amdgcn_readlane(v, ln); max_j = jb - ln; }
            if (brk) { end_j = jb - lb; n_skip = __builtin_amdgcn_readlane(n_after, lb); break; }
            const int last = jb - st < 63 ? jb - st : 63;
            n_skip = __builtin_amdgcn_readlane(n_after, last);
            end_j = st - 1;
        }
        if (max_ii < 0 || ri - (int)(a[max_ii].key >> 16) > CH_MAX_GAP) {
            int bf = INT32_MIN, bj = -1;
            for (int j = i - 1 - lane; j >= st; j -= 64) { const int fj = a[j].f; if (fj > bf) { bf = fj; bj = j; } }
            for (int o = 32; o > 0; o >>= 1) { const int of = __shfl_xor(bf, o), oj = __shfl_xor(bj, o); if (of > bf || (of == bf && oj > bj)) { bf = of; bj = oj; } }
            max_ii = bj;
        }
        if (max_ii >= 0 && max_ii < end_j) {
            const int32_t tmp = chain_sc(ai, a[max_ii].key, pen);
            if (tmp != INT32_MIN && max_f < tmp + a[max_ii].f) { max_f = tmp + a[max_ii].f; max_j = max_ii; }
        }
        wave_sync();
        if (lane == 0) { a[i].f = max_f; a[i].p = (int16_t)max_j; }
        wave_sync();
        if (max_ii < 0 || (ri - (int)(a[max_ii].key >> 16) <= CH_MAX_GAP && a[max_ii].f < max_f)) max_ii = i;
    }
    for (int i = lane; i < n; i += 64) a[i].t = 0;
    wave_sync();
    for (;;) {
        int zf = INT32_MIN, zi = -1;
        for (int i = lane; i < n; i += 64) { const int fi = a[i].f; if (a[i].t == 0 && fi >= CH_MIN_SCORE && (fi > zf || (fi == zf && i > zi))) { zf = fi; zi = i; } }
        for (int o = 32; o > 0; o >>= 1) { const int of = __shfl_xor(zf, o), oi = __shfl_xor(zi, o); if (of > zf || (of == zf && oi > zi)) { zf = of; zi = oi; } }
        if (zi < 0) break;
        int i = zi, end_i = -1, max_i = zi, max_s = 0;
        do {
            a[i].t = 2;
            end_i = i = a[i].p;
            const int s2 = i < 0 ? zf : zf - a[i].f;
            if (s2 > max_s) { max_s = s2; max_i = i; }
            else if (max_s - s2 > CH_BW) break;
        } while (i >= 0 && (a[i].t & 3) == 0);
        for (i = zi; i >= 0 && i != end_i; i = a[i].p) a[i].t = 0;
        end_i = max_i;
        int cnt = 0, first = zi;
        for (i = zi; i != end_i; i = a[i].p) { a[i].t = 1; first = i; ++cnt; }
        const int sc = i < 0 ? zf : zf - a[i].f;
        if (cnt == 0) a[zi].t = 4;
        wave_sync();
        emit_chains(member && sc >= CH_MIN_SCORE && cnt >= CH_MIN_CNT, mine, sc, zf, a[zi].key + (shift << 16), a[first].key + (shift << 16), cnt, chains, chain_cap, read_chain, lane);
    }
    wave_sync();
}

__device__ __forceinline__ int rl(int v, int lane_idx) { return __builtin_amdgcn_readlane(v, __builtin_amdgcn_readfirstlane(lane_idx)); }

__device__ __forceinline__ void dp_by_wave_regs(const SGroup& grp, const uint32_t* __restrict__ anchors, const int32_t* __restrict__ pen, SChain* __restrict__ chains, uint32_t chain_cap,
                                                uint3* __restrict__ read_chain, int lane, bool member, const SGroup& mine, uint32_t shift) {
    const int n = (int)grp.cnt;
    const int my_j = 63 - lane;
    uint32_t raw = lane < n ? anchors[grp.off + lane] : 0xFFFFFFFFu;
    int rank = 0;
    for (int x = 0; x < n; ++x) { const uint32_t kx = (uint32_t)__builtin_amdgcn_readlane((int)raw, x); rank += kx < raw ? 1 : 0; }
    const int dst = lane < n ? 63 - rank : lane - n;
    const uint32_t key = (uint32_t)__builtin_amdgcn_ds_permute(dst << 2, (int)raw);
    int f = 0, p = -1;
    int st = 0, max_ii = -1;
    for (int i = 0; i < n; ++i) {
        const uint32_t ai = (uint32_t)rl((int)key, 63 - i); const int ri = (int)(ai >> 16);
        while (st < i && ri > (int)((uint32_t)rl((int)key, 63 - st) >> 16) + CH_MAX_GAP) ++st;
        int max_f = MZ_K, max_j = -1, end_j = st - 1;
        if (i > st && i <= CH_MAX_SKIP) {
            const bool in = my_j >= st && my_j < i;
            const int32_t sc = in ? chain_sc(ai, key, pen) : INT32_MIN;
            const int v = sc != INT32_MIN ? sc + f : INT32_MIN;
            const int m = __builtin_amdgcn_readlane(wave_prefix_max(v), 63);
            if (m > max_f) { max_f = m; max_j = 63 - (int)__builtin_ctzll(__ballot(v == m)); }
        } else if (i > st) {
            const bool in = my_j >= st && my_j < i;
            const int32_t sc = in ? chain_sc(ai, key, pen) : INT32_MIN;
            const bool valid = sc != INT32_MIN;
            const int v = valid ? sc + f : INT32_MIN;
            const bool sends = valid && p >= 0;
            const int got = __builtin_amdgcn_ds_permute((sends ? 63 - p : 63 - i) << 2, sends ? 1 : 0);
            const bool marked = in && got == 1;
            int before = dpp_move<0x138, 0xf>(INT32_MIN, wave_prefix_max(v));
            before = before > max_f ? before : max_f;
            const bool isnew = valid && v > before;
            int ca = isnew ? -1 : (valid && marked ? 1 : 0), cb = isnew ? 0 : -(1 << 20);
            wave_prefix_maps(ca, cb);
            const int n_after = ca > cb ? ca : cb;
            const unsigned long long brk = __ballot(valid && !isnew && marked && n_after > CH_MAX_SKIP);
            const int lb = brk ? __builtin_ctzll(brk) : 64;
            const unsigned long long news = __ballot(isnew) & (lb >= 63 ? ~0ull : ((2ull << lb) - 1ull));
            if (news) { const int ln = 63 - __builtin_clzll(news); max_f = rl(v, ln); max_j = 63 - ln; }
            if (brk) end_j = 63 - lb;
        }
        if (max_ii < 0 || ri - (int)((uint32_t)rl((int)key, 63 - max_ii) >> 16) > CH_MAX_GAP) {
            const bool in = my_j >= st && my_j < i;
            int bk = in ? (f << 8 | my_j) : -1;
            for (int o = 32; o > 0; o >>= 1) { const int t = __shfl_xor(bk, o); bk = t > bk ? t : bk; }
            max_ii = bk < 0 ? -1 : (bk & 0xFF);
        }
        if (max_ii >= 0 && max_ii < end_j) {
            const int32_t tmp = chain_sc(ai, (uint32_t)rl((int)key, 63 - max_ii), pen);
            const int fm = rl(f, 63 - max_ii);
            if (tmp != INT32_MIN && max_f < tmp + fm) { max_f = tmp + fm; max_j = max_ii; }
        }
        if (my_j == i) { f = max_f; p = max_j; }
        if (max_ii < 0 || (ri - (int)((uint32_t)rl((int)key, 63 - max_ii) >> 16) <= CH_MAX_GAP && rl(f, 63 - max_ii) < max_f)) max_ii = i;
    }
    int t = 0;
    for (;;) {
        int bk = (my_j < n && t == 0 && f >= CH_MIN_SCORE) ? (f << 8 | my_j) : -1;
        for (int o = 32; o > 0; o >>= 1) { const int x = __shfl_xor(bk, o); bk = x > bk ? x : bk; }
        if (bk < 0) break;
        const int zi = bk & 0xFF, zf = bk >> 8;
        int i = zi, end_i = -1, max_i = zi, max_s = 0;
        do {
            if (my_j == i) t = 2;
            end_i = i = rl(p, 63 - i);
            const int s2 = i < 0 ? zf : zf - rl(f, 63 - i);
            if (s2 > max_s) { max_s = s2; max_i = i; }
            else if (max_s - s2 > CH_BW) break;
        } while (i >= 0 && (rl(t, 63 - i) & 3) == 0);
        for (i = zi; i >= 0 && i != end_i; i = rl(p, 63 - i)) { if (my_j == i) t = 0; }
        end_i = max_i;
        int cnt = 0, first = zi;
        for (i = zi; i != end_i; i = rl(p, 63 - i)) { if (my_j == i) t = 1; first = i; ++cnt; }
        const int sc = i < 0 ? zf : zf - rl(f, 63 - i);
        if (cnt == 0 && my_j == zi) t = 4;
        const uint32_t end_key = (uint32_t)rl((int)key, 63 - zi), first_key = (uint32_t)rl((int)key, 63 - first);
        emit_chains(member && sc >= CH_MIN_SCORE && cnt >= CH_MIN_CNT, mine, sc, zf, end_key + (shift << 16), first_key + (shift << 16), cnt, chains, chain_cap, read_chain, lane);
    }
}

__global__ __launch_bounds__(CH_THREADS) void k1s_dp_kernel(const SGroup* __restrict__ groups, const uint32_t* __restrict__ anchors, const int32_t* __restrict__ pen_tab,
                                                            BatchCursors* __restrict__ cur, SChain* __restrict__ chains, uint32_t chain_cap, uint3* __restrict__ read_chain,
                                                            SBigItem* __restrict__ items, SMember* __restrict__ members, uint32_t big_cap, SeedCounters* __restrict__ ctr) {
    extern __shared__ uint32_t lds[];
    int32_t* pen = reinterpret_cast<int32_t*>(lds);
    const int tid = threadIdx.x, lane = tid & 63, wave = tid >> 6;
    uint32_t* wl = lds + 512 + wave * DP_WAVE_WORDS;
    for (int i = tid; i <= CH_BW; i += CH_THREADS) pen[i] = pen_tab[i];
    __syncthreads();
    const uint32_t n_groups = (uint32_t)(cur->groups_anchors >> 32);
    unsigned long long t_last = 0;
#ifdef SP_K1S_TIMING
    t_last = wall_clock64();
#endif
    (void)t_last;
    const uint32_t n_tasks = (n_groups + 63) / 64;
    uint32_t pow2 = 1; while (pow2 < n_tasks) pow2 <<= 1;
    const uint32_t n_waves = gridDim.x * (CH_THREADS / 64);
    for (uint32_t k = blockIdx.x * (CH_THREADS / 64) + wave; k < pow2; k += n_waves) {
        const uint32_t task = (k * 0x9E3779B1u) & (pow2 - 1);
        if (task >= n_tasks) continue;
        const uint32_t g0 = task * 64;
        const uint32_t gi = g0 + lane;
        SGroup grp; grp.read = 0; grp.key = 0; grp.off = 0; grp.cnt = 0;
        if (gi < n_groups) grp = groups[gi];
        const int n = (int)grp.cnt;
        const int small_n = n <= DP_REG_MAX ? n : 0;
        int mx = small_n;
        for (int o = 32; o > 0; o >>= 1) { const int t = __shfl_xor(mx, o); mx = t > mx ? t : mx; }
        K1S_TW(7);
#if SP_DP_EXP == 5
        if (mx > 8) { }
        else
#endif
        if (mx > 8) dp_in_lds_rows(grp, small_n, mx, anchors, pen, reinterpret_cast<unsigned long long*>(wl), lane, chains, chain_cap, read_chain);
        else if (mx > 4) dp_in_registers<8, 8>(grp, small_n, anchors, pen, wl, lane, chains, chain_cap, read_chain);
        else if (mx > 0) dp_in_registers<4, 4>(grp, small_n, anchors, pen, wl, lane, chains, chain_cap, read_chain);
#ifdef SP_K1S_TIMING
        if (lane == 0) { const unsigned long long now_ = wall_clock64(); atomicAdd(&ctr->t[mx > 8 ? 5 : 4], now_ - t_last); t_last = now_; }
#endif
#if SP_DP_EXP == 4
        const unsigned long long big = 0;
#else
        const unsigned long long big = __ballot(n > DP_REG_MAX);
#endif
        if (!big) continue;
        unsigned long long h1 = 0, h2 = 0; uint32_t min_r = 0;
        for (unsigned long long todo = big; todo; todo &= todo - 1) {
            const int l = __builtin_ctzll(todo);
            const uint32_t off = (uint32_t)__builtin_amdgcn_readlane((int)grp.off, l), cnt = (uint32_t)__builtin_amdgcn_readlane((int)grp.cnt, l);
            uint32_t mn = 0xFFFFu;
            for (uint32_t i = lane; i < cnt; i += 64) { const uint32_t r = anchors[off + i] >> 16; mn = r < mn ? r : mn; }
            for (int o = 32; o > 0; o >>= 1) { const uint32_t t = (uint32_t)__shfl_xor((int)mn, o); mn = t < mn ? t : mn; }
            unsigned long long s1 = 0, s2 = 0;
            for (uint32_t i = lane; i < cnt; i += 64) {
                const unsigned long long x = anchors[off + i] - (mn << 16);
                s1 += mix64((x ^ 0x9E3779B97F4A7C15ull) & MZ_MASK) * 0x9E3779B97F4A7C15ull + x;
                unsigned long long y = (x + 0x632BE59BD9B4E019ull) * 0xD6E8FEB86659FD93ull; y ^= y >> 32; y *= 0xD6E8FEB86659FD93ull; y ^= y >> 32;
                s2 += y;
            }
            for (int o = 32; o > 0; o >>= 1) { s1 += __shfl_xor(s1, o); s2 += __shfl_xor(s2, o); }
            if (lane == l) { h1 = s1; h2 = s2; min_r = mn; }
        }
        int rep = -1;
        for (unsigned long long todo = big; todo; todo &= todo - 1) {
            const int l = __builtin_ctzll(todo);
            const unsigned long long b1 = __shfl(h1, l), b2 = __shfl(h2, l);
            const int bn = __builtin_amdgcn_readlane(n, l);
            if (rep < 0 && n > DP_REG_MAX && n == bn && h1 == b1 && h2 == b2) rep = l;
        }
        const unsigned long long reps = __ballot(n > DP_REG_MAX && rep == lane);
        uint32_t item0 = 0, mem0 = 0;
        if (lane == 0) { item0 = atomicAdd(&cur->big_items, (uint32_t)__builtin_popcountll(reps)); mem0 = atomicAdd(&cur->big_members, (uint32_t)__builtin_popcountll(big)); }
        item0 = (uint32_t)__builtin_amdgcn_readfirstlane((int)item0); mem0 = (uint32_t)__builtin_amdgcn_readfirstlane((int)mem0);
        uint32_t k_item = 0, k_mem = 0;
        for (unsigned long long todo = reps; todo; todo &= todo - 1) {
            const int l = __builtin_ctzll(todo);
            const unsigned long long mem = __ballot(n > DP_REG_MAX && rep == l);
            const uint32_t rep_min = (uint32_t)__builtin_amdgcn_readlane((int)min_r, l);
            if (item0 + k_item < big_cap && mem0 + k_mem + (uint32_t)__builtin_popcountll(mem) <= big_cap) {
                if (rep == l && n > DP_REG_MAX) {
                    SMember m; m.read = grp.read; m.key = grp.key; m.shift = min_r - rep_min; m.pad = 0;
                    members[mem0 + k_mem + (uint32_t)__builtin_popcountll(mem & ((1ull << lane) - 1ull))] = m;
                }
                if (lane == l) { SBigItem it; it.g = grp; it.member_off = mem0 + k_mem; it.n_members = (uint32_t)__builtin_popcountll(mem); it.pad0 = it.pad1 = 0; items[item0 + k_item] = it; }
            } else if (lane == l) atomicAdd(&ctr->overflow_reads, 1u);
            ++k_item; k_mem += (uint32_t)__builtin_popcountll(mem);
        }
        K1S_TW(6);
    }
}

template <bool LONG>
__global__ __launch_bounds__(LONG ? 64 : CH_THREADS) void k1s_dp_big_kernel(const SBigItem* __restrict__ items, const SMember* __restrict__ members, const uint32_t* __restrict__ anchors,
                                                                            const int32_t* __restrict__ pen_tab, BatchCursors* __restrict__ cur, uint32_t big_cap, SChain* __restrict__ chains,
                                                                            uint32_t chain_cap, uint3* __restrict__ read_chain, SeedCounters* __restrict__ ctr) {
    extern __shared__ uint32_t lds[];
    int32_t* pen = reinterpret_cast<int32_t*>(lds);
    const int tid = threadIdx.x, lane = tid & 63, wave = tid >> 6;
    uint32_t* wl = lds + 512;
    for (int i = tid; i <= CH_BW; i += (int)blockDim.x) pen[i] = pen_tab[i];
    __syncthreads();
    const uint32_t n_items = cur->big_items < big_cap ? cur->big_items : big_cap;
    uint32_t pow2 = 1; while (pow2 < n_items) pow2 <<= 1;
    const uint32_t n_waves = gridDim.x * (blockDim.x / 64);
    for (uint32_t k = blockIdx.x * (blockDim.x / 64) + wave; k < pow2; k += n_waves) {
        const uint32_t x = (k * 0x9E3779B1u) & (pow2 - 1);
        if (x >= n_items) continue;
        const SBigItem it = items[x];
        if ((it.g.cnt > 64) != LONG) continue;
        if (LONG && it.g.cnt > (uint32_t)DP_BIG_MAX) { if (lane == 0) atomicAdd(&ctr->overflow_reads, 1u); continue; }
        for (uint32_t m0 = 0; m0 < it.n_members; m0 += 64) {
            const bool member = m0 + lane < it.n_members;
            SGroup mine = it.g; uint32_t shift = 0;
            if (member) { const SMember m = members[it.member_off + m0 + lane]; mine.read = m.read; mine.key = m.key; shift = m.shift; }
            if (!LONG) dp_by_wave_regs(it.g, anchors, pen, chains, chain_cap, read_chain, lane, member, mine, shift);
            else dp_by_wave(it.g, reinterpret_cast<SDp*>(wl), anchors, pen, chains, chain_cap, read_chain, lane, ctr, member, mine, shift);
        }
    }
}

__global__ __launch_bounds__(CH_THREADS) void k1s_select_kernel(SeqSetView reads, uint32_t r0, uint32_t n_batch, const SChain* __restrict__ chains, int32_t* __restrict__ parent,
                                                                const uint3* __restrict__ read_chain, SSel* __restrict__ sel, uint32_t* __restrict__ sel_cnt,
                                                                SeedCounters* __restrict__ ctr, int best_n, SChain* __restrict__ dbg_chains, int32_t* __restrict__ dbg_parent,
                                                                uint32_t* __restrict__ dbg_n, uint32_t dbg_read) {
    __shared__ unsigned long long s_r1[CH_THREADS / 64], s_r2[CH_THREADS / 64];
    __shared__ int s_ri[CH_THREADS / 64];
    __shared__ int s_prim[PRIM_CAP];
    __shared__ int s_sel[PRIM_CAP + 8];
    const int tid = threadIdx.x;
    if (blockIdx.x >= n_batch) return;
    const uint32_t r = r0 + blockIdx.x;
    const int qlen = reads.len[r];
    const uint3 rc = read_chain[r];
    uint32_t nc = rc.z;
    if (nc > rc.y) { nc = rc.y; if (tid == 0) atomicAdd(&ctr->overflow_reads, 1u); }
    const SChain* sc_chain = chains + rc.x; int32_t* sc_parent = parent + rc.x;
    auto k1_of = [](const SChain& c) { return (unsigned long long)(uint32_t)c.score << 32 | (uint32_t)c.f_end; };
    auto k2_of = [](const SChain& c) { return (unsigned long long)c.key << 32 | c.end; };
    for (uint32_t i = tid; i < nc; i += CH_THREADS) sc_parent[i] = -1;
    __syncthreads();
    int n_prim = 0;
    while (n_prim < PRIM_CAP) {
        bool have = false; unsigned long long b1 = 0, b2 = 0; int bi = -1;
        for (uint32_t i = tid; i < nc; i += CH_THREADS) if (sc_parent[i] == -1) {
            const SChain c = sc_chain[i]; const unsigned long long a1 = k1_of(c), a2 = k2_of(c);
            if (!have || a1 > b1 || (a1 == b1 && a2 > b2)) { have = true; b1 = a1; b2 = a2; bi = (int)i; }
        }
        const int P = block_argmax(have, b1, b2, bi, s_r1, s_r2, s_ri);
        if (P < 0) break;
        if (tid == 0) { sc_parent[P] = P; s_prim[n_prim] = P; }
        ++n_prim;
        const SChain pc = sc_chain[P];
        int pqs, pqe, prs, pre; chain_interval(pc, qlen, pqs, pqe, prs, pre);
        __syncthreads();
        for (uint32_t i = tid; i < nc; i += CH_THREADS) if (sc_parent[i] == -1) {
            int qs, qe, rs, re; chain_interval(sc_chain[i], qlen, qs, qe, rs, re);
            const int mn = (pqe - pqs) < (qe - qs) ? (pqe - pqs) : (qe - qs);
            const int ol = (qe < pqe ? qe : pqe) - (qs > pqs ? qs : pqs);
            if (ol > 0 && (float)ol > MASK_LEVEL * (float)mn) sc_parent[i] = P;
        }
        __syncthreads();
    }
    int n_sec = 0;
    for (; n_sec < best_n; ++n_sec) {
        bool have = false; unsigned long long b1 = 0, b2 = 0; int bi = -1;
        for (uint32_t i = tid; i < nc; i += CH_THREADS) {
            const int p = sc_parent[i];
            if (p < 0 || p == (int)i) continue;
            const SChain c = sc_chain[i], pc = sc_chain[p];
            if (!((float)c.score >= (float)pc.score * PRI_RATIO || c.score + 2 * MZ_K >= pc.score)) continue;
            int qs, qe, rs, re, pqs, pqe, prs, pre; chain_interval(c, qlen, qs, qe, rs, re); chain_interval(pc, qlen, pqs, pqe, prs, pre);
            if (qs == pqs && qe == pqe && (c.key & 0x7FFFu) == (pc.key & 0x7FFFu) && rs == prs && re == pre) continue;
            const unsigned long long a1 = k1_of(c), a2 = k2_of(c);
            if (!have || a1 > b1 || (a1 == b1 && a2 > b2)) { have = true; b1 = a1; b2 = a2; bi = (int)i; }
        }
        const int S = block_argmax(have, b1, b2, bi, s_r1, s_r2, s_ri);
        if (S < 0) break;
        if (tid == 0) { sc_parent[S] = -2 - sc_parent[S]; s_sel[n_prim + n_sec] = S; }
        __syncthreads();
    }
    __syncthreads();
    if (dbg_chains && r == dbg_read) {
        for (uint32_t i = tid; i < nc; i += CH_THREADS) { dbg_chains[i] = sc_chain[i]; dbg_parent[i] = sc_parent[i]; }
        if (tid == 0) *dbg_n = nc;
    }
    if (tid == 0) {
        int n = 0;
        for (int i = 0; i < n_prim; ++i) s_sel[n++] = s_prim[i];
        for (int i = 0; i < n_sec; ++i) s_sel[n++] = s_sel[n_prim + i];
        for (int i = 1; i < n; ++i) {
            const int x = s_sel[i]; const SChain cx = sc_chain[x]; int j = i - 1;
            while (j >= 0) { const SChain cj = sc_chain[s_sel[j]]; if (k1_of(cj) > k1_of(cx) || (k1_of(cj) == k1_of(cx) && k2_of(cj) > k2_of(cx))) break; s_sel[j + 1] = s_sel[j]; --j; }
            s_sel[j + 1] = x;
        }
        if (n > SEL_CAP || n_prim >= PRIM_CAP) atomicAdd(&ctr->overflow_reads, 1u);
        if (n > SEL_CAP) n = SEL_CAP;
        uint32_t n_rev = 0;
        for (int i = 0; i < n; ++i) {
            const SChain c = sc_chain[s_sel[i]];
            SSel o; o.rid = (int32_t)(c.key & 0x7FFFu); o.rev = (int32_t)(c.key >> 15); o.score = c.score; o.cnt = (int32_t)c.cnt; o.n_chains = (int32_t)nc;
            chain_interval(c, qlen, o.qs, o.qe, o.rs, o.re);
            const int d0 = (int)(c.first & 0xFFFFu) - (int)(c.first >> 16), d1 = (int)(c.end & 0xFFFFu) - (int)(c.end >> 16);
            o.diag = (d0 + d1) >> 1;
            sel[(size_t)r * SEL_CAP + i] = o;
            n_rev += (uint32_t)o.rev;
        }
        sel_cnt[r] = (uint32_t)n;
        if (n_rev) atomicAdd(&ctr->rev_selected, n_rev);
    }
}

__global__ void k1s_cells_kernel(const SSel* __restrict__ sel, const uint32_t* __restrict__ sel_cnt, uint32_t n_reads, const uint32_t* __restrict__ rid_allele,
                                 const int32_t* __restrict__ allele_len, int rev, CellDesc* __restrict__ cells) {
    const uint32_t x = blockIdx.x * blockDim.x + threadIdx.x;
    if (x >= n_reads * SEL_CAP) return;
    const uint32_t r = x / SEL_CAP, s = x % SEL_CAP;
    CellDesc c; c.a = 0; c.b = r; c.diag = SP_NO_DIAG; c.max_ed = 0; c.b_lo = 0; c.b_hi = -1;
    if (s < sel_cnt[r]) {
        const SSel q = sel[x];
        if (q.rev == rev) {
            c.a = rid_allele[q.rid]; c.diag = q.diag;
            int cap = (int)(0.03 * (double)allele_len[c.a]) + 1; if (cap > SP_MAX_ED) cap = SP_MAX_ED;
            c.max_ed = cap;
        }
    }
    cells[x] = c;
}
constexpr int K1S_WIDE_SHIFT = 32;
__global__ void k1s_rescore_cells_kernel(const CellDesc* __restrict__ cells, const sp_aln* __restrict__ alns, uint32_t n, CellDesc* __restrict__ out, int wide, SeedCounters* __restrict__ ctr) {
    const uint32_t x = blockIdx.x * blockDim.x + threadIdx.x;
    if (x >= n) return;
    CellDesc c = cells[x];
    const sp_aln a = alns[x];
    bool is_wide = false;
    if (c.diag != SP_NO_DIAG && a.ok) { const int shift = (a.b_end - a.a_end) - (a.b_start - a.a_start); is_wide = shift > K1S_WIDE_SHIFT || shift < -K1S_WIDE_SHIFT; }
    if (c.diag == SP_NO_DIAG || !a.ok || is_wide != (wide != 0)) { c.diag = wide ? SP_NO_DIAG : 0; c.max_ed = -1; }
    else { c.diag = ((a.b_start - a.a_start) + (a.b_end - a.a_end)) / 2; c.max_ed = 127; }
    out[x] = c;
    if (!wide && is_wide && ctr) atomicAdd(&ctr->wide_cells, 1u);
}
__global__ void k1s_merge_wide_kernel(const CellDesc* __restrict__ wide_cells, const sp_affine_aln* __restrict__ af_wide, uint32_t n, sp_affine_aln* __restrict__ af) {
    const uint32_t x = blockIdx.x * blockDim.x + threadIdx.x;
    if (x < n && wide_cells[x].diag != SP_NO_DIAG) af[x] = af_wide[x];
}
__global__ void k1s_merge_rev_kernel(const SSel* __restrict__ sel, const uint32_t* __restrict__ sel_cnt, uint32_t n_reads, const sp_aln* __restrict__ aln_rev,
                                     const sp_affine_aln* __restrict__ af_rev, sp_aln* __restrict__ aln, sp_affine_aln* __restrict__ af) {
    const uint32_t x = blockIdx.x * blockDim.x + threadIdx.x;
    if (x >= n_reads * SEL_CAP) return;
    const uint32_t r = x / SEL_CAP, s = x % SEL_CAP;
    if (s < sel_cnt[r] && sel[x].rev) { aln[x] = aln_rev[x]; af[x] = af_rev[x]; }
}
__global__ __launch_bounds__(256) void k1s_revcomp_kernel(SeqSetView reads, const SSel* __restrict__ sel, const uint32_t* __restrict__ sel_cnt, uint32_t* __restrict__ words,
                                                          uint32_t* __restrict__ nplane) {
    const uint32_t r = blockIdx.x;
    bool need = false;
    for (uint32_t s = 0; s < sel_cnt[r]; ++s) need |= sel[(size_t)r * SEL_CAP + s].rev != 0;
    const int len = reads.len[r];
    const uint64_t wo = reads.word_off[r];
    const int nw = (len + 15) >> 4;
    if (!need) return;
    const uint32_t* w = reads.words + wo; const uint32_t* np = reads.nplane ? reads.nplane + wo : nullptr;
    for (int x = threadIdx.x; x < nw + 2; x += 256) {
        uint32_t out = 0, outn = 0;
        for (int b = 0; b < 16; ++b) {
            const int pos = x * 16 + b, src = len - 1 - pos;
            if (pos >= len) break;
            const uint32_t base = (w[src >> 4] >> ((src & 15) << 1)) & 3u;
            out |= (3u - base) << (b << 1);
            if (np) outn |= ((np[src >> 4] >> ((src & 15) << 1)) & 1u) << (b << 1);
        }
        if (np) { const uint32_t m = outn | (outn << 1); out &= ~m; }
        words[wo + x] = out;
        if (nplane) nplane[wo + x] = outn;
    }
}

__device__ __forceinline__ double seed_score_value(int len, int nm, int unmapped) { double num = (double)(nm + unmapped); if (num < 0.1) num = 0.1; return num / (double)len; }

__global__ void k1s_pick_kernel(SeqSetView reads, const SSel* __restrict__ sel, const uint32_t* __restrict__ sel_cnt, uint32_t n_reads, const sp_aln* __restrict__ alns,
                                const sp_affine_aln* __restrict__ afs, const uint32_t* __restrict__ rid_allele, const int32_t* __restrict__ allele_len, int best_n,
                                int32_t* __restrict__ best_out, sp_k1_seed_info* __restrict__ info, sp_aln* __restrict__ win_aln, sp_affine_aln* __restrict__ win_af,
                                sp_k1_seed_hit* __restrict__ dbg_hits, uint32_t* __restrict__ dbg_n, uint32_t dbg_read, sp_hla_rev_hit* __restrict__ rev_out) {
    const uint32_t r = blockIdx.x * blockDim.x + threadIdx.x;
    if (r >= n_reads) return;
    const int qlen = reads.len[r];
    const uint32_t ns = sel_cnt[r];
    struct Hit { int slot, rid, rev, score, dp, nm, qs, qe, rs, re, tl, parent; };
    Hit h[SEL_CAP]; int nh = 0;
    for (uint32_t s = 0; s < ns; ++s) {
        const size_t x = (size_t)r * SEL_CAP + s;
        const SSel q = sel[x]; const sp_aln a = alns[x]; const sp_affine_aln f = afs[x];
        if (!a.ok || f.score < MIN_DP_MAX || f.score <= 0) continue;
        Hit t; t.slot = (int)s; t.rid = q.rid; t.rev = q.rev; t.score = q.score; t.dp = f.score; t.nm = f.nm; t.rs = f.b_start; t.re = f.b_end;
        if (q.rev) { t.qs = qlen - f.a_end; t.qe = qlen - f.a_start; } else { t.qs = f.a_start; t.qe = f.a_end; }
        t.tl = allele_len[rid_allele[q.rid]]; t.parent = 0;
        int j = nh - 1;
        while (j >= 0 && h[j].dp < t.dp) { h[j + 1] = h[j]; --j; }
        h[j + 1] = t; ++nh;
    }
    for (int i = 0; i < nh; ++i) {
        h[i].parent = i;
        for (int j = 0; j < i; ++j) {
            if (h[j].parent != j) continue;
            const int mn = (h[j].qe - h[j].qs) < (h[i].qe - h[i].qs) ? (h[j].qe - h[j].qs) : (h[i].qe - h[i].qs);
            const int ol = (h[i].qe < h[j].qe ? h[i].qe : h[j].qe) - (h[i].qs > h[j].qs ? h[i].qs : h[j].qs);
            if (ol > 0 && (float)ol > MASK_LEVEL * (float)mn) { h[i].parent = j; break; }
        }
    }
    int pick = -1, n_out = 0, n2 = 0; double best = 1.0;
    int rpick = -1; double rbest = 1.0;
    for (int i = 0; i < nh; ++i) {
        const int p = h[i].parent;
        bool keep = p == i;
        if (!keep && ((float)h[i].score >= (float)h[p].score * PRI_RATIO || h[i].score + 2 * MZ_K >= h[p].score) && n2 < best_n &&
            !(h[i].qs == h[p].qs && h[i].qe == h[p].qe && h[i].rid == h[p].rid && h[i].rs == h[p].rs && h[i].re == h[p].re)) { keep = true; ++n2; }
        if (!keep) continue;
        const int tl = h[i].tl, um = tl - (h[i].re - h[i].rs), nm = h[i].nm;
        const double pen = seed_score_value(tl, nm, um), ed = seed_score_value(tl - um, nm, 0);
        if (pen <= 0.5 && ed <= 0.03 && ed < best) { best = ed; pick = i; }
        if (rev_out && tl > 0 && tl - um > 0 && pen <= 0.5 && ed <= 0.03 && ed < rbest) { rbest = ed; rpick = i; }
        if (dbg_hits && r == dbg_read) {
            sp_k1_seed_hit d; const size_t x = (size_t)r * SEL_CAP + h[i].slot; const SSel q = sel[x]; const sp_aln a = alns[x];
            d.allele = (int32_t)rid_allele[h[i].rid]; d.rev = h[i].rev; d.chain_score = q.score; d.n_seeds = q.cnt; d.t_len = tl; d.sel_rank = h[i].slot; d.diag = q.diag;
            d.ok = a.ok; d.cell_nm = a.nm; d.a_start = a.a_start; d.a_end = a.a_end; d.b_start = a.b_start; d.b_end = a.b_end;
            d.dp_max = h[i].dp; d.nm = nm; d.t_start = h[i].rs; d.t_end = h[i].re; d.q_start = h[i].qs; d.q_end = h[i].qe; d.primary = p == i ? 1 : 0;
            dbg_hits[n_out] = d;
        }
        ++n_out;
    }
    if (dbg_hits && r == dbg_read) *dbg_n = (uint32_t)n_out;
    sp_k1_seed_info o; o.n_chains = ns ? sel[(size_t)r * SEL_CAP].n_chains : 0; o.n_selected = (int32_t)ns; o.n_mappings = n_out; o.pick = pick; o.chain_score = 0; o.rev = 0;
    sp_aln wa; wa.ok = 0; wa.nm = 0; wa.a_start = wa.a_end = wa.b_start = wa.b_end = wa.a_len = wa.b_len = 0;
    sp_affine_aln wf; wf.score = 0; wf.nm = 0; wf.a_start = wf.a_end = wf.b_start = wf.b_end = 0;
    int32_t b = -1;
    if (pick >= 0) {
        const size_t x = (size_t)r * SEL_CAP + h[pick].slot;
        o.chain_score = h[pick].score; o.rev = h[pick].rev;
        if (!h[pick].rev) { b = (int32_t)rid_allele[h[pick].rid]; wa = alns[x]; wf = afs[x]; }
    }
    best_out[r] = b; info[r] = o; win_aln[r] = wa; win_af[r] = wf;
    if (rev_out) {
        sp_hla_rev_hit v; v.allele = -1; v.t_len = v.nm = v.t_start = v.t_end = v.reserved_ = 0;
        if (rpick >= 0 && h[rpick].rev) { v.allele = (int32_t)rid_allele[h[rpick].rid]; v.t_len = h[rpick].tl; v.nm = h[rpick].nm; v.t_start = h[rpick].rs; v.t_end = h[rpick].re; }
        rev_out[r] = v;
    }
}

}

struct K1Seed {
    uint32_t n_seqs = 0, n_keys = 0; uint64_t n_mz = 0; int32_t mid_occ = 0;
    uint32_t* d_rid_allele = nullptr;
    uint64_t* d_keys = nullptr; uint32_t* d_start = nullptr; uint32_t* d_occ = nullptr; uint32_t* d_bucket = nullptr; int32_t* d_pen = nullptr;
    IndexView view() const { return IndexView{ d_keys, d_start, d_occ, d_bucket, n_keys, mid_occ, n_seqs }; }
};

void sp_k1_seed_free(K1Seed* s) {
    if (!s) return;
    (void)hipFree(s->d_rid_allele); (void)hipFree(s->d_keys); (void)hipFree(s->d_start); (void)hipFree(s->d_occ); (void)hipFree(s->d_bucket); (void)hipFree(s->d_pen);
    delete s;
}

void sp_k1_seed_stats(const K1Seed* s, int64_t out[4]) { out[0] = (int64_t)s->n_mz; out[1] = s->n_keys; out[2] = s->mid_occ; out[3] = s->n_seqs; }

template <typename T> static T* seed_dev_copy(const std::vector<T>& v) {
    T* d = nullptr;
    if (hipMalloc(&d, std::max<size_t>(1, v.size()) * sizeof(T)) != hipSuccess) return nullptr;
    if (!v.empty()) (void)hipMemcpy(d, v.data(), v.size() * sizeof(T), hipMemcpyHostToDevice);
    return d;
}

int sp_k1_seed_build(sp_ctx* ctx, const sp_seqset* alleles, K1Seed** out) {
    *out = nullptr;
    (void)hipSetDevice(ctx->device);
    std::vector<uint32_t> rid_allele;
    for (uint32_t a = 0; a < alleles->n; ++a) if (alleles->h_len[a] > 0) rid_allele.push_back(a);
    const uint32_t n = (uint32_t)rid_allele.size();
    if (n == 0) return sp_fail(ctx, SP_ERR_INVALID_ARG, "seeded K1: the database has no DNA allele");
    if (n >= (1u << 15) || alleles->max_len > 65535) return sp_fail(ctx, SP_ERR_TOO_LONG, "seeded K1: at most 32,767 DNA alleles of at most 65,535 bases");
    K1Seed* s = new (std::nothrow) K1Seed();
    if (!s) return sp_fail(ctx, SP_ERR_OUT_OF_MEMORY, "seeded K1: index");
    s->n_seqs = n;
    std::vector<void*> temps;
    auto grab = [&](size_t bytes) -> void* { void* q = nullptr; if (hipMalloc(&q, std::max<size_t>(bytes, 16)) != hipSuccess) return nullptr; temps.push_back(q); return q; };
    auto fail = [&](const char* what) { for (void* q : temps) (void)hipFree(q); sp_k1_seed_free(s); return sp_fail(ctx, SP_ERR_HIP, what); };
    hipStream_t st = ctx->stream;
    s->d_rid_allele = seed_dev_copy(rid_allele);
    uint32_t* d_cnt = (uint32_t*)grab((size_t)n * 4); uint64_t* d_off = (uint64_t*)grab(((size_t)n + 1) * 8);
    if (!s->d_rid_allele || !d_cnt || !d_off) return fail("seeded K1: index buffers");
    hipLaunchKernelGGL(mz_sketch_kernel<false>, dim3(n), dim3(256), 0, st, alleles->view(), s->d_rid_allele, n, d_cnt, (const uint64_t*)nullptr, (uint64_t*)nullptr, (uint32_t*)nullptr);
    std::vector<uint32_t> cnt(n);
    if (hipMemcpyAsync(cnt.data(), d_cnt, (size_t)n * 4, hipMemcpyDeviceToHost, st) != hipSuccess || hipStreamSynchronize(st) != hipSuccess) return fail("seeded K1: sketch counts");
    std::vector<uint64_t> off((size_t)n + 1, 0);
    for (uint32_t i = 0; i < n; ++i) off[i + 1] = off[i] + cnt[i];
    const uint64_t total = off[n];
    if (total == 0 || total >= (1ull << 32)) return fail("seeded K1: nothing to index");
    s->n_mz = total;
    uint64_t* d_k = (uint64_t*)grab(total * 8); uint64_t* d_ks = (uint64_t*)grab(total * 8); uint32_t* d_o = (uint32_t*)grab(total * 4);
    if (!d_k || !d_ks || !d_o || hipMalloc(&s->d_occ, total * 4) != hipSuccess) return fail("seeded K1: index tables");
    if (hipMemcpyAsync(d_off, off.data(), ((size_t)n + 1) * 8, hipMemcpyHostToDevice, st) != hipSuccess) return fail("seeded K1: offsets");
    hipLaunchKernelGGL(mz_sketch_kernel<true>, dim3(n), dim3(256), 0, st, alleles->view(), s->d_rid_allele, n, (uint32_t*)nullptr, d_off, d_k, d_o);
    size_t bytes = 0;
    if (rocprim::radix_sort_pairs(nullptr, bytes, d_k, d_ks, d_o, s->d_occ, (size_t)total, 0, 2 * MZ_K, st) != hipSuccess) return fail("seeded K1: sort size");
    void* ws = grab(bytes);
    if (!ws || rocprim::radix_sort_pairs(ws, bytes, d_k, d_ks, d_o, s->d_occ, (size_t)total, 0, 2 * MZ_K, st) != hipSuccess) return fail("seeded K1: sort");
    std::vector<uint64_t> ks(total);
    if (hipMemcpyAsync(ks.data(), d_ks, total * 8, hipMemcpyDeviceToHost, st) != hipSuccess || hipStreamSynchronize(st) != hipSuccess) return fail("seeded K1: sorted keys");
    std::vector<uint64_t> keys; std::vector<uint32_t> start;
    for (uint64_t i = 0; i < total; ++i) if (i == 0 || ks[i] != ks[i - 1]) { keys.push_back(ks[i]); start.push_back((uint32_t)i); }
    start.push_back((uint32_t)total);
    const size_t nk = keys.size();
    s->n_keys = (uint32_t)nk;
    {
        std::vector<uint32_t> c(nk);
        for (size_t i = 0; i < nk; ++i) c[i] = start[i + 1] - start[i];
        std::sort(c.begin(), c.end());
        int64_t kth = (int64_t)((1.0 - (double)MID_OCC_FRAC) * (double)nk);
        if (kth >= (int64_t)nk) kth = (int64_t)nk - 1;
        int32_t mid = (int32_t)c[(size_t)kth] + 1;
        if (mid < MIN_MID_OCC) mid = MIN_MID_OCC;
        if (mid > MAX_MID_OCC) mid = MAX_MID_OCC;
        s->mid_occ = mid;
    }
    std::vector<uint32_t> bucket(((size_t)1 << BUCKET_BITS) + 1, 0);
    {
        size_t k = 0;
        for (size_t b = 0; b <= ((size_t)1 << BUCKET_BITS); ++b) {
            while (k < nk && (keys[k] >> (2 * MZ_K - BUCKET_BITS)) < b) ++k;
            bucket[b] = (uint32_t)k;
        }
    }
    std::vector<int32_t> pen(CH_BW + 1, 0);
    {
        const float pen_gap = 0.01f * 0.8f * (float)MZ_K;
        for (int dd = 1; dd <= CH_BW; ++dd) { const float lin = pen_gap * (float)dd; const float lg = log2f((float)(dd + 1)); pen[dd] = (int32_t)(lin + .5f * lg); }
    }
    s->d_keys = seed_dev_copy(keys); s->d_start = seed_dev_copy(start); s->d_bucket = seed_dev_copy(bucket); s->d_pen = seed_dev_copy(pen);
    for (void* q : temps) (void)hipFree(q);
    temps.clear();
    if (!s->d_keys || !s->d_start || !s->d_bucket || !s->d_pen) { sp_k1_seed_free(s); return sp_fail(ctx, SP_ERR_OUT_OF_MEMORY, "seeded K1: index upload"); }
    *out = s;
    return SP_OK;
}

int sp_k1_seed_sketch(sp_ctx* ctx, const sp_seqset* set, uint32_t idx, uint64_t* hash, int32_t* end_pos, uint8_t* strand, uint32_t cap, uint32_t* n_out) {
    (void)hipSetDevice(ctx->device);
    const uint32_t maxn = (uint32_t)std::max(1, set->h_len[idx]);
    uint32_t* d_seq = (uint32_t*)sp_pool(ctx, "k1s_sk_seq", 4); uint32_t* d_cnt = (uint32_t*)sp_pool(ctx, "k1s_sk_cnt", 4); uint64_t* d_off = (uint64_t*)sp_pool(ctx, "k1s_sk_off", 8);
    uint64_t* d_k = (uint64_t*)sp_pool(ctx, "k1s_sk_k", (size_t)maxn * 8); uint32_t* d_o = (uint32_t*)sp_pool(ctx, "k1s_sk_o", (size_t)maxn * 4);
    if (!d_seq || !d_cnt || !d_off || !d_k || !d_o) return sp_fail(ctx, SP_ERR_OUT_OF_MEMORY, "sketch buffers");
    const uint64_t zero = 0;
    SP_HIP_CHECK(ctx, hipMemcpyAsync(d_seq, &idx, 4, hipMemcpyHostToDevice, ctx->stream));
    SP_HIP_CHECK(ctx, hipMemcpyAsync(d_off, &zero, 8, hipMemcpyHostToDevice, ctx->stream));
    hipLaunchKernelGGL(mz_sketch_kernel<false>, dim3(1), dim3(256), 0, ctx->stream, set->view(), d_seq, 1u, d_cnt, (const uint64_t*)nullptr, (uint64_t*)nullptr, (uint32_t*)nullptr);
    hipLaunchKernelGGL(mz_sketch_kernel<true>, dim3(1), dim3(256), 0, ctx->stream, set->view(), d_seq, 1u, (uint32_t*)nullptr, d_off, d_k, d_o);
    uint32_t n = 0;
    SP_HIP_CHECK(ctx, hipMemcpyAsync(&n, d_cnt, 4, hipMemcpyDeviceToHost, ctx->stream));
    SP_HIP_CHECK(ctx, hipStreamSynchronize(ctx->stream));
    *n_out = n;
    const uint32_t m = std::min(n, cap);
    std::vector<uint64_t> k(m); std::vector<uint32_t> o(m);
    if (m) { SP_HIP_CHECK(ctx, hipMemcpy(k.data(), d_k, (size_t)m * 8, hipMemcpyDeviceToHost)); SP_HIP_CHECK(ctx, hipMemcpy(o.data(), d_o, (size_t)m * 4, hipMemcpyDeviceToHost)); }
    for (uint32_t i = 0; i < m; ++i) { if (hash) hash[i] = k[i]; if (end_pos) end_pos[i] = (int32_t)((o[i] >> 1) & 0xFFFFu); if (strand) strand[i] = (uint8_t)(o[i] & 1u); }
    return SP_OK;
}

int sp_k1_seed_map(sp_ctx* ctx, const K1Seed* idx, const sp_seqset* alleles, const sp_seqset* reads, int best_n, int32_t* d_best, sp_k1_seed_info* d_info,
                   sp_aln* d_win_aln, sp_affine_aln* d_win_af, const K1SeedDebug* dbg, sp_hla_rev_hit* d_rev) {
    const uint32_t R = reads->n;
    if (R == 0) return SP_OK;
    (void)hipSetDevice(ctx->device);
    if (reads->max_len > 65535) return sp_fail(ctx, SP_ERR_TOO_LONG, "seeded K1: reads of up to 65,535 bases");
    const IndexView ix = idx->view();
    SeedCounters* d_ctr = (SeedCounters*)sp_pool(ctx, "k1s_ctr", sizeof(SeedCounters));
    uint2* d_read_seed = (uint2*)sp_pool(ctx, "k1s_read_seed", (size_t)R * 8);
    uint32_t* d_read_anchors = (uint32_t*)sp_pool(ctx, "k1s_read_anchors", (size_t)R * 4);
    if (!d_ctr || !d_read_seed || !d_read_anchors) return sp_fail(ctx, SP_ERR_OUT_OF_MEMORY, "seeded K1: buffers");
    const int sd_cap = std::min(13000, reads->max_len / 6 + 64);
    const size_t seed_lds = (size_t)(2 * (TILE + 2 * HALO)) * 4 + (size_t)sd_cap * (4 + 4 + 2 + 1) + (TILE + 2 * HALO) + 64;
    SP_HIP_CHECK(ctx, hipFuncSetAttribute((const void*)k1s_seed_kernel, hipFuncAttributeMaxDynamicSharedMemorySize, (int)seed_lds));
    SeedCounters hc;
    uint32_t seed_cap = (uint32_t)std::min<size_t>(0xFFFFFFF0u, (size_t)R * 96 + 4096);
    uint4* d_seeds = nullptr;
    for (int attempt = 0; attempt < 2; ++attempt) {
        d_seeds = (uint4*)sp_pool(ctx, "k1s_seeds", (size_t)seed_cap * 16);
        if (!d_seeds) return sp_fail(ctx, SP_ERR_OUT_OF_MEMORY, "seeded K1: seed list");
        SP_HIP_CHECK(ctx, hipMemsetAsync(d_ctr, 0, sizeof(SeedCounters), ctx->stream));
        {
            ProfScope ps(ctx, "k1s_seeds", R);
            hipLaunchKernelGGL(k1s_seed_kernel, dim3(R), dim3(256), seed_lds, ctx->stream, reads->view(), ix, R, sd_cap, d_seeds, seed_cap, d_read_seed, d_read_anchors, d_ctr);
        }
        SP_HIP_CHECK(ctx, hipGetLastError());
        SP_HIP_CHECK(ctx, hipMemcpyAsync(&hc, d_ctr, sizeof(hc), hipMemcpyDeviceToHost, ctx->stream));
        SP_HIP_CHECK(ctx, hipStreamSynchronize(ctx->stream));
        if (hc.seed_overflow == 0) break;
        if (attempt == 1 || hc.seeds > 0xFFFFFFF0ull) return sp_fail(ctx, SP_ERR_OUT_OF_MEMORY, "seeded K1: seed list overflow");
        seed_cap = (uint32_t)hc.seeds + 1024;
    }
    uint32_t* d_sel_cnt = (uint32_t*)sp_pool(ctx, "k1s_sel_cnt", (size_t)R * 4);
    SSel* d_sel = (SSel*)sp_pool(ctx, "k1s_sel", (size_t)R * SEL_CAP * sizeof(SSel));
    uint3* d_read_chain = (uint3*)sp_pool(ctx, "k1s_read_chain", (size_t)R * sizeof(uint3));
    BatchCursors* d_cur = (BatchCursors*)sp_pool(ctx, "k1s_cursors", sizeof(BatchCursors));
    uint32_t* h_anchors = (uint32_t*)sp_host_pool(ctx, "k1s_read_anchors", (size_t)R * 4);
    if (!d_sel_cnt || !d_sel || !d_read_chain || !d_cur || !h_anchors) return sp_fail(ctx, SP_ERR_OUT_OF_MEMORY, "seeded K1: selection");
    SP_HIP_CHECK(ctx, hipMemcpyAsync(h_anchors, d_read_anchors, (size_t)R * 4, hipMemcpyDeviceToHost, ctx->stream));
    SP_HIP_CHECK(ctx, hipStreamSynchronize(ctx->stream));
    const uint64_t batch_anchors = std::max<uint64_t>(hc.max_anchors, 64ull << 20);
    const uint64_t a_cap = std::min<uint64_t>(hc.anchors, batch_anchors + hc.max_anchors), g_cap = a_cap / CH_MIN_CNT + 1;
    if (a_cap >= (1ull << 32)) return sp_fail(ctx, SP_ERR_TOO_LONG, "seeded K1: a read with more than 4 G anchors");
    uint32_t r_batch_max = 0;
    for (uint32_t r0 = 0; r0 < R;) { uint64_t a = 0; uint32_t r1 = r0; while (r1 < R && (r1 == r0 || a + h_anchors[r1] <= batch_anchors)) a += h_anchors[r1++]; r_batch_max = std::max(r_batch_max, r1 - r0); r0 = r1; }
    const uint64_t c_cap = g_cap;
    uint32_t* d_anchors = (uint32_t*)sp_pool(ctx, "k1s_anchors", std::max<uint64_t>(a_cap, 1) * 4);
    SGroup* d_groups = (SGroup*)sp_pool(ctx, "k1s_groups", g_cap * sizeof(SGroup));
    SChain* d_chains = (SChain*)sp_pool(ctx, "k1s_chains", c_cap * sizeof(SChain));
    int32_t* d_parent = (int32_t*)sp_pool(ctx, "k1s_parent", c_cap * 4);
    const uint64_t big_cap = a_cap / (DP_REG_MAX + 1) + 64;
    SBigItem* d_items = (SBigItem*)sp_pool(ctx, "k1s_big_items", big_cap * sizeof(SBigItem));
    SMember* d_members = (SMember*)sp_pool(ctx, "k1s_big_members", big_cap * sizeof(SMember));
    if (!d_anchors || !d_groups || !d_chains || !d_parent || !d_items || !d_members) return sp_fail(ctx, SP_ERR_OUT_OF_MEMORY, "seeded K1: chain buffers");
    const size_t group_lds = (size_t)WIN_KEYS * 4, dp_lds = (size_t)(512 + (CH_THREADS / 64) * DP_WAVE_WORDS) * 4;
    SP_HIP_CHECK(ctx, hipFuncSetAttribute((const void*)k1s_group_kernel, hipFuncAttributeMaxDynamicSharedMemorySize, (int)group_lds));
    SP_HIP_CHECK(ctx, hipFuncSetAttribute((const void*)k1s_dp_kernel, hipFuncAttributeMaxDynamicSharedMemorySize, (int)dp_lds));
    const size_t big_lds = (size_t)(512 + DP_BIG_WORDS) * 4;
    SP_HIP_CHECK(ctx, hipFuncSetAttribute((const void*)k1s_dp_big_kernel<true>, hipFuncAttributeMaxDynamicSharedMemorySize, (int)big_lds));
    SChain* dbg_chains = nullptr; int32_t* dbg_parent = nullptr; uint32_t* dbg_n = nullptr;
    if (dbg) {
        dbg_chains = (SChain*)sp_pool(ctx, "k1s_dbg_chains", g_cap * sizeof(SChain)); dbg_parent = (int32_t*)sp_pool(ctx, "k1s_dbg_parent", g_cap * 4);
        dbg_n = (uint32_t*)sp_pool(ctx, "k1s_dbg_n", 8);
        if (!dbg_chains || !dbg_parent || !dbg_n) return sp_fail(ctx, SP_ERR_OUT_OF_MEMORY, "seeded K1: debug buffers");
        SP_HIP_CHECK(ctx, hipMemsetAsync(dbg_n, 0, 8, ctx->stream));
    }
    for (uint32_t r0 = 0; r0 < R;) {
        uint64_t a = 0; uint32_t r1 = r0;
        while (r1 < R && (r1 == r0 || a + h_anchors[r1] <= batch_anchors)) a += h_anchors[r1++];
        const uint32_t nb_reads = r1 - r0;
        SP_HIP_CHECK(ctx, hipMemsetAsync(d_cur, 0, sizeof(BatchCursors), ctx->stream));
        {
            ProfScope ps(ctx, "k1s_groups", a);
            hipLaunchKernelGGL(k1s_group_kernel, dim3(nb_reads), dim3(CH_THREADS), group_lds, ctx->stream, reads->view(), ix, r0, nb_reads, d_seeds, d_read_seed, d_anchors, (uint32_t)a_cap,
                               d_groups, (uint32_t)g_cap, d_read_chain, d_cur, d_ctr);
        }
        {
            ProfScope ps(ctx, "k1s_dp", a);
            hipLaunchKernelGGL(k1s_dp_kernel, dim3((unsigned)ctx->num_cus * 8), dim3(CH_THREADS), dp_lds, ctx->stream, d_groups, d_anchors, idx->d_pen, d_cur, d_chains, (uint32_t)c_cap, d_read_chain, d_items, d_members, (uint32_t)big_cap, d_ctr);
        }
        {
            ProfScope ps(ctx, "k1s_dp_big", a);
            hipLaunchKernelGGL(k1s_dp_big_kernel<false>, dim3((unsigned)ctx->num_cus * 8), dim3(CH_THREADS), 512 * 4, ctx->stream, d_items, d_members, d_anchors, idx->d_pen, d_cur, (uint32_t)big_cap,
                               d_chains, (uint32_t)c_cap, d_read_chain, d_ctr);
            hipLaunchKernelGGL(k1s_dp_big_kernel<true>, dim3((unsigned)ctx->num_cus * 3), dim3(64), big_lds, ctx->stream, d_items, d_members, d_anchors, idx->d_pen, d_cur, (uint32_t)big_cap,
                               d_chains, (uint32_t)c_cap, d_read_chain, d_ctr);
        }
        {
            ProfScope ps(ctx, "k1s_select", nb_reads);
            hipLaunchKernelGGL(k1s_select_kernel, dim3(nb_reads), dim3(CH_THREADS), 0, ctx->stream, reads->view(), r0, nb_reads, d_chains, d_parent, d_read_chain, d_sel, d_sel_cnt, d_ctr, best_n,
                               dbg_chains, dbg_parent, dbg_n, dbg ? dbg->read : 0xFFFFFFFFu);
        }
        SP_HIP_CHECK(ctx, hipGetLastError());
        r0 = r1;
    }
    const uint64_t NC = (uint64_t)R * SEL_CAP;
    CellDesc* d_cells = (CellDesc*)sp_pool(ctx, "k1s_cells", NC * sizeof(CellDesc)); CellDesc* d_rc = (CellDesc*)sp_pool(ctx, "k1s_rc", NC * sizeof(CellDesc));
    sp_aln* d_aln = (sp_aln*)sp_pool(ctx, "k1s_aln", NC * sizeof(sp_aln)); sp_affine_aln* d_af = (sp_affine_aln*)sp_pool(ctx, "k1s_af_out", NC * sizeof(sp_affine_aln));
    if (!d_cells || !d_rc || !d_aln || !d_af) return sp_fail(ctx, SP_ERR_OUT_OF_MEMORY, "seeded K1: cells");
    const sp_affine_opts ao = { 1, 4, 6, 2, 26, 1, 1 };
    const unsigned nb = (unsigned)((NC + 255) / 256);
    hipLaunchKernelGGL(k1s_cells_kernel, dim3(nb), dim3(256), 0, ctx->stream, d_sel, d_sel_cnt, R, idx->d_rid_allele, alleles->d_len, 0, d_cells);
    const uint32_t ev_stride = (uint32_t)std::min<int64_t>(SP_MAX_ED, (int64_t)(0.03 * (double)alleles->max_len) + 2);
    uint32_t* d_ev = (uint32_t*)sp_pool(ctx, "k1s_ev", NC * (size_t)ev_stride * 4);
    if (!d_ev) return sp_fail(ctx, SP_ERR_OUT_OF_MEMORY, "seeded K1: cell events");
    int rc = sp_launch_cells(ctx, alleles, reads, d_cells, NC, d_aln, d_ev, ev_stride, "k1s_cells", 1);
    if (rc != SP_OK) return rc;
    hipLaunchKernelGGL(k1s_rescore_cells_kernel, dim3(nb), dim3(256), 0, ctx->stream, d_cells, d_aln, (uint32_t)NC, d_rc, 0, d_ctr);
    rc = sp_rescore_mappings(ctx, alleles, reads, d_rc, d_aln, NC, true, ao, 64, d_af, "k1s_af", ev_stride, 0, d_aln, d_ev);
    if (rc != SP_OK) return rc;
    SP_HIP_CHECK(ctx, hipMemcpyAsync(&hc, d_ctr, sizeof(hc), hipMemcpyDeviceToHost, ctx->stream));
    SP_HIP_CHECK(ctx, hipStreamSynchronize(ctx->stream));
#ifdef SP_K1S_TIMING
    fprintf(stderr, "k1s_group phases (100 MHz ticks summed over workgroups): count %llu scan %llu scatter %llu records %llu; dp kernel waves: task + load %llu, up to 8 anchors %llu, 9..26 %llu, signatures of the large %llu\n", hc.t[0], hc.t[1], hc.t[2], hc.t[3], hc.t[7], hc.t[4], hc.t[5], hc.t[6]);
#endif
    if (hc.overflow_reads) {
        ctx->prof["k1s_truncated_reads"].cells += hc.overflow_reads;
        ctx->warning = "seeded K1: " + std::to_string(hc.overflow_reads) + " capacity events (seed / anchor / chain lists of a read cut short) in the last sp_hla_realign_reads call: "
                       "those reads were mapped from truncated lists; k1_best_n 0 (the exhaustive search) has no such bounds";
    }
    if (hc.wide_cells) {
        sp_affine_aln* d_afw = (sp_affine_aln*)sp_pool(ctx, "k1s_af_wide", NC * sizeof(sp_affine_aln));
        if (!d_afw) return sp_fail(ctx, SP_ERR_OUT_OF_MEMORY, "seeded K1: wide re-score");
        hipLaunchKernelGGL(k1s_rescore_cells_kernel, dim3(nb), dim3(256), 0, ctx->stream, d_cells, d_aln, (uint32_t)NC, d_rc, 1, (SeedCounters*)nullptr);
        rc = sp_rescore_mappings(ctx, alleles, reads, d_rc, d_aln, NC, true, ao, 256, d_afw, "k1s_afw", 128, 1);
        if (rc != SP_OK) return rc;
        hipLaunchKernelGGL(k1s_merge_wide_kernel, dim3(nb), dim3(256), 0, ctx->stream, d_rc, d_afw, (uint32_t)NC, d_af);
    }
    if (hc.rev_selected) {
        const size_t words = (size_t)reads->h_word_off[R] + SP_SEQ_PAD_WORDS;
        uint32_t* d_rw = (uint32_t*)sp_pool(ctx, "k1s_rev_words", words * 4);
        uint32_t* d_rn = reads->d_nplane ? (uint32_t*)sp_pool(ctx, "k1s_rev_nplane", words * 4) : nullptr;
        CellDesc* d_cells2 = (CellDesc*)sp_pool(ctx, "k1s_cells_rev", NC * sizeof(CellDesc));
        sp_aln* d_aln2 = (sp_aln*)sp_pool(ctx, "k1s_aln_rev", NC * sizeof(sp_aln)); sp_affine_aln* d_af2 = (sp_affine_aln*)sp_pool(ctx, "k1s_af_rev", NC * sizeof(sp_affine_aln));
        if (!d_rw || (reads->d_nplane && !d_rn) || !d_cells2 || !d_aln2 || !d_af2) return sp_fail(ctx, SP_ERR_OUT_OF_MEMORY, "seeded K1: reverse strand");
        SP_HIP_CHECK(ctx, hipMemsetAsync(d_rw, 0, words * 4, ctx->stream));
        if (d_rn) SP_HIP_CHECK(ctx, hipMemsetAsync(d_rn, 0, words * 4, ctx->stream));
        hipLaunchKernelGGL(k1s_revcomp_kernel, dim3(R), dim3(256), 0, ctx->stream, reads->view(), d_sel, d_sel_cnt, d_rw, d_rn);
        sp_seqset rset;
        rset.ctx = reads->ctx; rset.n = R; rset.has_n = reads->has_n; rset.max_len = reads->max_len; rset.d_words = d_rw; rset.d_nplane = d_rn; rset.d_word_off = reads->d_word_off; rset.d_len = reads->d_len;
        rset.h_len = reads->h_len; rset.h_word_off = reads->h_word_off;
        hipLaunchKernelGGL(k1s_cells_kernel, dim3(nb), dim3(256), 0, ctx->stream, d_sel, d_sel_cnt, R, idx->d_rid_allele, alleles->d_len, 1, d_cells2);
        rc = sp_launch_cells(ctx, alleles, &rset, d_cells2, NC, d_aln2, nullptr, 0, "k1s_cells_rev", 1);
        if (rc != SP_OK) return rc;
        hipLaunchKernelGGL(k1s_rescore_cells_kernel, dim3(nb), dim3(256), 0, ctx->stream, d_cells2, d_aln2, (uint32_t)NC, d_rc, 0, d_ctr);
        rc = sp_rescore_mappings(ctx, alleles, &rset, d_rc, d_aln2, NC, true, ao, 64, d_af2, "k1s_af_rev", 128);
        if (rc != SP_OK) return rc;
        {
            sp_affine_aln* d_afw = (sp_affine_aln*)sp_pool(ctx, "k1s_af_wide", NC * sizeof(sp_affine_aln));
            if (!d_afw) return sp_fail(ctx, SP_ERR_OUT_OF_MEMORY, "seeded K1: wide re-score");
            hipLaunchKernelGGL(k1s_rescore_cells_kernel, dim3(nb), dim3(256), 0, ctx->stream, d_cells2, d_aln2, (uint32_t)NC, d_rc, 1, (SeedCounters*)nullptr);
            rc = sp_rescore_mappings(ctx, alleles, &rset, d_rc, d_aln2, NC, true, ao, 256, d_afw, "k1s_afw_rev", 128, 1);
            if (rc != SP_OK) return rc;
            hipLaunchKernelGGL(k1s_merge_wide_kernel, dim3(nb), dim3(256), 0, ctx->stream, d_rc, d_afw, (uint32_t)NC, d_af2);
        }
        hipLaunchKernelGGL(k1s_merge_rev_kernel, dim3(nb), dim3(256), 0, ctx->stream, d_sel, d_sel_cnt, R, d_aln2, d_af2, d_aln, d_af);
        SP_HIP_CHECK(ctx, hipStreamSynchronize(ctx->stream));
    }
    sp_k1_seed_hit* dbg_hits = nullptr; uint32_t* dbg_nh = nullptr;
    if (dbg) {
        dbg_hits = (sp_k1_seed_hit*)sp_pool(ctx, "k1s_dbg_hits", SEL_CAP * sizeof(sp_k1_seed_hit));
        if (!dbg_hits) return sp_fail(ctx, SP_ERR_OUT_OF_MEMORY, "seeded K1: debug buffers");
        dbg_nh = dbg_n + 1;
    }
    hipLaunchKernelGGL(k1s_pick_kernel, dim3((R + 63) / 64), dim3(64), 0, ctx->stream, reads->view(), d_sel, d_sel_cnt, R, d_aln, d_af, idx->d_rid_allele, alleles->d_len, best_n,
                       d_best, d_info, d_win_aln, d_win_af, dbg_hits, dbg_nh, dbg ? dbg->read : 0u, d_rev);
    SP_HIP_CHECK(ctx, hipGetLastError());
    if (dbg) {
        uint32_t n2[2] = { 0, 0 };
        SP_HIP_CHECK(ctx, hipMemcpyAsync(n2, dbg_n, 8, hipMemcpyDeviceToHost, ctx->stream));
        SP_HIP_CHECK(ctx, hipStreamSynchronize(ctx->stream));
        std::vector<SChain> ch(n2[0]); std::vector<int32_t> par(n2[0]);
        if (n2[0]) { SP_HIP_CHECK(ctx, hipMemcpy(ch.data(), dbg_chains, (size_t)n2[0] * sizeof(SChain), hipMemcpyDeviceToHost)); SP_HIP_CHECK(ctx, hipMemcpy(par.data(), dbg_parent, (size_t)n2[0] * 4, hipMemcpyDeviceToHost)); }
        std::vector<uint32_t> order(n2[0]);
        for (uint32_t i = 0; i < n2[0]; ++i) order[i] = i;
        std::sort(order.begin(), order.end(), [&](uint32_t x, uint32_t y) {
            const unsigned long long x1 = (unsigned long long)(uint32_t)ch[x].score << 32 | (uint32_t)ch[x].f_end, y1 = (unsigned long long)(uint32_t)ch[y].score << 32 | (uint32_t)ch[y].f_end;
            if (x1 != y1) return x1 > y1;
            const unsigned long long x2 = (unsigned long long)ch[x].key << 32 | ch[x].end, y2 = (unsigned long long)ch[y].key << 32 | ch[y].end;
            return x2 > y2; });
        const int qlen = reads->h_len[dbg->read];
        *dbg->n_chains = n2[0];
        for (uint32_t i = 0; i < n2[0] && i < dbg->chain_cap; ++i) {
            const SChain& c = ch[order[i]]; int32_t* o = dbg->chains + (size_t)i * 10;
            int rs = (int)(c.first >> 16) + 1 - MZ_K, re = (int)(c.end >> 16) + 1, s = (int)(c.first & 0xFFFFu) + 1 - MZ_K, e = (int)(c.end & 0xFFFFu) + 1;
            const int rev = (int)(c.key >> 15);
            o[0] = (int32_t)(c.key & 0x7FFFu); o[1] = rev; o[2] = c.score; o[3] = (int32_t)c.cnt; o[4] = rev ? qlen - e : s; o[5] = rev ? qlen - s : e; o[6] = rs; o[7] = re;
            const int32_t p = par[order[i]];
            o[8] = p; o[9] = (p == (int32_t)order[i] || p <= -2) ? 1 : 0;
        }
        *dbg->n_hits = n2[1];
        if (n2[1]) SP_HIP_CHECK(ctx, hipMemcpy(dbg->hits, dbg_hits, (size_t)std::min<uint32_t>(n2[1], SEL_CAP) * sizeof(sp_k1_seed_hit), hipMemcpyDeviceToHost));
        dbg->counters[0] = hc.seeds; dbg->counters[1] = hc.anchors; dbg->counters[2] = hc.max_anchors; dbg->counters[3] = hc.overflow_reads;
    }
    return SP_OK;
}
```

pb-starphase_amd/csrc/sp_internal.h:

```cpp
#pragma once
#include <hip/hip_runtime.h>
#include <stdint.h>
#include <string>
#include <vector>
#include <chrono>
#include <set>
#include <mutex>
#include <map>
#include "../../include/starphase_hip.h"

#define SP_NEG        (-(1 << 28))
#define SP_SEQ_PAD_WORDS 512
#define SP_LDS_TAIL    288
#define SP_WAVE       64
#define SP_MAXOCC     4
#define SP_CELL_NONE  0xFFFFFFFFu
#define SP_PEAK_SPREAD   48
#define SP_PEAK_SUPPRESS 128

struct SeqSetView {
    const uint32_t* words;
    const uint32_t* nplane;
    const uint64_t* word_off;
    const int32_t*  len;
    uint32_t n;
};

struct KmerIndexView {
    const uint32_t* code;
    const int32_t*  pos;
    const uint64_t* off;
};

struct sp_seqset {
    sp_ctx* ctx = nullptr;
    uint32_t n = 0;
    bool has_n = false;
    std::vector<int32_t>  h_len;
    std::vector<uint64_t> h_word_off;
    std::vector<uint32_t> h_words;
    uint32_t* d_words = nullptr;
    uint32_t* d_nplane = nullptr;
    uint64_t* d_word_off = nullptr;
    int32_t*  d_len = nullptr;
    int32_t   max_len = 0;
    uint32_t  n_skipped = 0;
    struct sp_upload* up = nullptr;
    int32_t up_rc = 0; std::string up_err;
    bool has_index = false;
    uint32_t* d_kcode = nullptr; int32_t* d_kpos = nullptr; uint64_t* d_koff = nullptr;
    SeqSetView view() const { return SeqSetView{d_words, d_nplane, d_word_off, d_len, n}; }
    KmerIndexView kview() const { return KmerIndexView{d_kcode, d_kpos, d_koff}; }
};

struct ProfileEntry { double ms = 0; uint64_t launches = 0; uint64_t cells = 0; };

struct sp_ctx {
    int device = 0;
    hipStream_t stream = nullptr;
    bool own_stream = false;
    std::string err;
    bool profiling = true;
    hipEvent_t ev0 = nullptr, ev1 = nullptr;
    std::map<std::string, ProfileEntry> prof;
    struct PendingProf { hipEvent_t e0, e1; const char* name; uint64_t cells; };
    std::vector<PendingProf> prof_pending;
    std::vector<hipEvent_t> prof_free;
    void* scratch = nullptr; size_t scratch_bytes = 0;
    std::map<std::string, std::pair<void*, size_t>> pool;
    uint64_t pool_allocs = 0;
    std::map<std::string, std::pair<void*, size_t>> host_pool;
    std::multimap<size_t, void*> dev_cache; std::map<void*, size_t> dev_cap; size_t dev_cache_bytes = 0; std::mutex dev_cache_mu;
    std::set<sp_seqset*> live_sets;
    int num_cus = 256;
    int hw_queues = 4; bool hw_queues_by_library = false; std::string warning;
    bool split_genes = true;
    int split_streams = 3;
    bool cons_retry_ladder = false;
    hipStream_t copy_stream = nullptr;
    hipStream_t ctl_stream = nullptr;
    hipEvent_t ev_fork = nullptr, ev_join = nullptr;
    int k1_best_n = 5;
    int profile_rescore_counts = 0;
    int mm2_rescore = 1;
    int k8_persistent = 2;
    int hw_queues_effective = 0;
    int k8_side_orders = 1;
    int k8_compound = 1;
    int k8_side_max_blocks = 4096;
    int k8_persist_backoff = 0;
    int k8_persist_failures = 0;
    sp_seqset* uploading = nullptr;
    int k5_block_pairs = 4096;
    int cyp_cohort_min_group = 12;
    int cyp_cohort_streams = 8;
    sp_ctx* helper[7] = { nullptr, nullptr, nullptr, nullptr, nullptr, nullptr, nullptr };
};

struct CellDesc {
    uint32_t a, b;
    int32_t  diag;
    int32_t  max_ed;
    int32_t  b_lo, b_hi;
};

struct K2Dict {
    bool built = false, failed = false;
    uint32_t* d_ids = nullptr;
    uint64_t* d_id_off = nullptr;
    uint32_t* d_code = nullptr;
    uint32_t* d_dict_off = nullptr;
    std::vector<uint32_t> dict_off;
    uint32_t n_dict = 0, max_dict = 0;
};
void* sp_dev_alloc(sp_ctx* ctx, size_t bytes);
void sp_dev_release(sp_ctx* ctx, void* p);
int  sp_k2_dict_build(sp_ctx* ctx, const sp_seqset* set, const uint32_t* d_gene_of, uint32_t n_genes, K2Dict* out);
void sp_k2_dict_free(K2Dict* d);

struct K1Seed;
struct K1SeedDebug {
    uint32_t read;
    int32_t* chains; uint32_t chain_cap; uint32_t* n_chains;
    sp_k1_seed_hit* hits; uint32_t* n_hits;
    uint64_t* counters;
};
int  sp_k1_seed_build(sp_ctx* ctx, const sp_seqset* alleles, K1Seed** out);
void sp_k1_seed_free(K1Seed* s);
void sp_k1_seed_stats(const K1Seed* s, int64_t out[4]);
int  sp_k1_seed_sketch(sp_ctx* ctx, const sp_seqset* set, uint32_t idx, uint64_t* hash, int32_t* end_pos, uint8_t* strand, uint32_t cap, uint32_t* n_out);
int  sp_k1_seed_map(sp_ctx* ctx, const K1Seed* idx, const sp_seqset* alleles, const sp_seqset* reads, int best_n, int32_t* d_best, sp_k1_seed_info* d_info,
                    sp_aln* d_win_aln, sp_affine_aln* d_win_af, const K1SeedDebug* dbg, sp_hla_rev_hit* d_rev = nullptr);

sp_ctx* sp_ctx_helper(sp_ctx* ctx, int i = 0);
void sp_profile_merge(sp_ctx* into, sp_ctx* from);
int sp_launch_anchor(sp_ctx* ctx, const sp_seqset* A, const sp_seqset* B,
                     const uint32_t* d_a_idx, const uint32_t* d_b_idx, uint64_t n_pairs,
                     int32_t* d_diag, int32_t* d_votes, int topk = 1, const char* prof_name = "anchor", uint32_t a_period = 1);
int sp_launch_cells(sp_ctx* ctx, const sp_seqset* A, const sp_seqset* B,
                    const CellDesc* d_cells, uint64_t n_cells,
                    sp_aln* d_out, uint32_t* d_events, uint32_t events_stride, const char* prof_name, int retry_wide = 0);

int sp_launch_affine(sp_ctx* ctx, const sp_seqset* A, const sp_seqset* B, const void* d_pairs , uint64_t n_pairs, const sp_affine_opts& o, int band,
                     sp_affine_aln* d_out, const char* prof_name, const uint32_t* d_n_live = nullptr, const void* d_wins = nullptr, const void* d_mids = nullptr);
int sp_rescore_mappings(sp_ctx* ctx, const sp_seqset* Aw, const sp_seqset* Bw, const CellDesc* d_cells, const sp_aln* d_ref, uint64_t n, bool target_is_a,
                        const sp_affine_opts& o, int band, sp_affine_aln* d_out, const char* prefix, uint32_t stride, int trace_retry_wide = 0, const sp_aln* d_tr_in = nullptr, const uint32_t* d_ev_in = nullptr, int ends_only = 0, int windows = -1, void* d_audit = nullptr);
int sp_launch_affine_map(sp_ctx* ctx, const sp_seqset* A, const sp_seqset* B, const void* d_pairs , uint64_t n_pairs, const sp_affine_opts& o, int band, sp_affine_aln* d_out,
                         uint32_t* d_n_cigar, uint64_t* d_op_off, uint32_t* d_ops, uint64_t ops_cap, unsigned long long* d_cursor, const char* prof_name,
                         const uint32_t* d_n_live = nullptr, const uint32_t* d_list = nullptr, uint64_t prof_cells = ~0ull);
constexpr uint32_t SP_ANCHOR_SKIP = 0xFFFFFFFFu;
int sp_launch_cells_wide(sp_ctx* ctx, const sp_seqset* A, const sp_seqset* B, const CellDesc* d_cells, uint64_t n_cells, sp_aln* d_out);
int sp_launch_pack_on(hipStream_t stream, int num_cus, int format, const void* d_src, const uint64_t* d_off, const uint64_t* d_word_off, const int32_t* d_len, uint32_t n,
                      uint32_t* d_words, uint32_t* d_nplane, uint32_t* d_flag);
int sp_launch_pack(sp_ctx* ctx, const char* d_ascii, const uint64_t* d_off, const uint64_t* d_word_off, const int32_t* d_len, uint32_t n,
                   uint32_t* d_words, uint32_t* d_nplane, uint32_t* d_flag);
int sp_make_segments(sp_ctx* ctx, const sp_seqset* reads, const std::vector<uint32_t>& idx, const std::vector<int32_t>& start,
                     const std::vector<int32_t>& len, const char* prefix, sp_seqset* seg, sp_seqset* hpc);
int sp_seqset_make_small(sp_ctx* ctx, const char* prefix, const char* bases, const uint64_t* offsets, uint32_t n, bool with_index, sp_seqset* out);
int sp_seqset_fetch_host(sp_ctx* ctx, sp_seqset* s);
std::string sp_seqset_decode(sp_ctx* ctx, const sp_seqset* s, uint32_t i);
enum { SPC_K1_ACTIVE = 0, SPC_K1_EXECUTED, SPC_K1_RESUMED, SPC_K1_BYTES, SPC_CONS_LAUNCHES, SPC_CONS_COLUMNS, SPC_N = 16 };
unsigned long long* sp_counters(sp_ctx* ctx);
void* sp_scratch(sp_ctx* ctx, size_t bytes);
void* sp_pool(sp_ctx* ctx, const char* name, size_t bytes);
size_t sp_pool_bytes(const sp_ctx* ctx, const char* name);
void* sp_host_pool(sp_ctx* ctx, const char* name, size_t bytes);
int   sp_fail(sp_ctx* ctx, int code, const std::string& msg);
#define SP_HIP_CHECK(ctx, expr) do { hipError_t _e = (expr); if (_e != hipSuccess) \
    return sp_fail((ctx), SP_ERR_HIP, std::string(#expr) + ": " + hipGetErrorString(_e)); } while (0)

void sp_profile_flush(sp_ctx* ctx);
struct HostMarks {
    sp_ctx* ctx; std::chrono::steady_clock::time_point t;
    explicit HostMarks(sp_ctx* c) : ctx(c), t(std::chrono::steady_clock::now()) {}
    void mark(const char* name) { const auto now = std::chrono::steady_clock::now(); if (ctx->profiling) { auto& e = ctx->prof[name]; e.ms += std::chrono::duration<double, std::milli>(now - t).count(); e.launches += 1; } t = now; }
};
struct HostScope {
    sp_ctx* ctx; const char* name; std::chrono::steady_clock::time_point t0;
    HostScope(sp_ctx* c, const char* n) : ctx(c), name(n), t0(std::chrono::steady_clock::now()) {}
    ~HostScope() { if (ctx->profiling) { auto& e = ctx->prof[name]; e.ms += std::chrono::duration<double, std::milli>(std::chrono::steady_clock::now() - t0).count(); e.launches += 1; } }
};
struct ProfScope {
    sp_ctx* ctx; const char* name; uint64_t cells; hipEvent_t e0 = nullptr, e1 = nullptr;
    ProfScope(sp_ctx* c, const char* n, uint64_t cells_) : ctx(c), name(n), cells(cells_) {
        if (!(ctx->profiling && name)) return;
        auto take = [&]() { hipEvent_t e = nullptr; if (!ctx->prof_free.empty()) { e = ctx->prof_free.back(); ctx->prof_free.pop_back(); } else if (hipEventCreate(&e) != hipSuccess) e = nullptr; return e; };
        e0 = take(); e1 = take();
        if (e0 && e1) hipEventRecord(e0, ctx->stream);
    }
    ~ProfScope() {
        if (!(e0 && e1)) { if (e0) ctx->prof_free.push_back(e0); if (e1) ctx->prof_free.push_back(e1); return; }
        hipEventRecord(e1, ctx->stream);
        ctx->prof_pending.push_back({e0, e1, name, cells});
        if (ctx->prof_pending.size() >= 2048) sp_profile_flush(ctx);
    }
};


int32_t spi_gene_entry_extras(const sp_database* db, const sp_variant_gene* g, std::string* reference_allele, bool* has_sv, std::string* sv_chrom);
std::string spi_hla_allele_fwd(sp_ctx* ctx, const sp_hla_db* db, uint32_t a);
int spi_hla_gene_fwd(const sp_hla_db* db, uint32_t gene);
int32_t spi_hla_map_type_batch(sp_ctx* ctx, const sp_hla_db* db, uint32_t n, const uint32_t* genes, const char* const* consensus_fwd, const uint32_t* consensus_len,
                               int32_t require_dna, int32_t disable_cdna, sp_hla_map** out, std::vector<uint32_t>* item_of);
namespace spj { struct Value; }
void spi_support_ins_json(spj::Value* column, const sp_pileup_ins* ins, uint64_t n_ins, uint64_t col, const sp_cyp_read_mapping* mappings, uint64_t n_mappings,
                          const char* const* names, uint32_t n_names);
void spi_support_hap_json(spj::Value* consensus, const sp_pileup_col* cols, uint32_t length, const sp_support_hap* haps, uint64_t n_haps, const sp_support_hap_head* head,
                          uint64_t target, const sp_cyp_read_mapping* mappings, uint64_t n_mappings, const char* const* names, uint32_t n_names);
int32_t spi_cyp_diplotype_mappings(sp_ctx* ctx, const sp_cyp_problem* pr, const sp_seqset* reads, sp_cyp_call* call, char* consensus, uint32_t cons_cap,
                                   sp_cyp_region_variants* region_variants, std::vector<sp_cyp_read_mapping>* mappings);
int32_t spi_cyp_diplotype_cohort_mappings(sp_ctx* ctx, const sp_cyp_problem* pr, uint32_t n_samples, const sp_seqset* const* reads, sp_cyp_call* calls,
                                          char* consensus, uint32_t cons_cap, sp_cyp_region_variants* region_variants,
                                          std::vector<sp_cyp_read_mapping>* mappings, int32_t* sample_rc);
```

Before: 357,100 reads/s.

## Deduplicate identical anchor patterns per read before chaining DP in seeded K1

The group kernel now hashes each target's anchor list, shifted by its minimum reference coordinate, into a per-read LDS hash table. Targets with identical shifted anchor patterns are collapsed into one representative group that carries a member list. Chaining DP then runs once per pattern class, and the resulting chains are fanned out to every member with a coordinate shift. Before, this signature-based dedup was applied only to large groups inside the DP kernel. The change aims to cut redundant DP work across the thousands of near-identical HLA alleles, at the cost of extra hashing, atomics and buffers in the group kernel, plus a small risk from hash collisions.

```diff
diff --git a/pb-starphase_amd/csrc/sp_api.hip b/pb-starphase_amd/csrc/sp_api.hip
--- a/pb-starphase_amd/csrc/sp_api.hip
+++ b/pb-starphase_amd/csrc/sp_api.hip
@@ -108,7 +108,7 @@
 sp_ctx* sp_ctx_helper(sp_ctx* ctx, int i) {
     if (i < 0 || i > 6) return nullptr;
     if (!ctx->helper[i] && sp_ctx_create(ctx->device, nullptr, &ctx->helper[i]) != SP_OK) ctx->helper[i] = nullptr;
-    if (ctx->helper[i]) { ctx->helper[i]->profiling = ctx->profiling; ctx->helper[i]->k5_block_pairs = ctx->k5_block_pairs; ctx->helper[i]->k8_persistent = ctx->k8_persistent; ctx->helper[i]->k8_side_orders = ctx->k8_side_orders; ctx->helper[i]->k8_compound = ctx->k8_compound; ctx->helper[i]->k8_side_max_blocks = ctx->k8_side_max_blocks; ctx->helper[i]->mm2_rescore = ctx->mm2_rescore; ctx->helper[i]->profile_rescore_counts = ctx->profile_rescore_counts; ctx->helper[i]->k1_best_n = ctx->k1_best_n; }
+    if (ctx->helper[i]) { ctx->helper[i]->profiling = ctx->profiling; ctx->helper[i]->k5_block_pairs = ctx->k5_block_pairs; ctx->helper[i]->k8_persistent = ctx->k8_persistent; ctx->helper[i]->k8_side_orders = ctx->k8_side_orders; ctx->helper[i]->k8_compound = ctx->k8_compound; ctx->helper[i]->k8_side_max_blocks = ctx->k8_side_max_blocks; ctx->helper[i]->mm2_rescore = ctx->mm2_rescore; ctx->helper[i]->profile_rescore_counts = ctx->profile_rescore_counts; ctx->helper[i]->k1_best_n = ctx->k1_best_n; ctx->helper[i]->k1s_dedup = ctx->k1s_dedup; }
     return ctx->helper[i];
 }
 void sp_profile_merge(sp_ctx* into, sp_ctx* from) {
@@ -194,6 +194,7 @@
     if (!ctx || !name) return SP_ERR_INVALID_ARG;
     if (std::strcmp(name, "hla_split_genes") == 0) { ctx->split_genes = value != 0; return SP_OK; }
     if (std::strcmp(name, "k1_best_n") == 0) { if (value < 0 || value > 8) return sp_fail(ctx, SP_ERR_INVALID_ARG, "sp_ctx_set_option: k1_best_n is 0..8"); ctx->k1_best_n = (int)value; for (sp_ctx* h : ctx->helper) if (h) h->k1_best_n = ctx->k1_best_n; return SP_OK; }
+    if (std::strcmp(name, "k1s_dedup") == 0) { if (value != 0 && value != 1) return sp_fail(ctx, SP_ERR_INVALID_ARG, "sp_ctx_set_option: k1s_dedup is 0 or 1"); ctx->k1s_dedup = (int)value; for (sp_ctx* h : ctx->helper) if (h) h->k1s_dedup = ctx->k1s_dedup; return SP_OK; }
     if (std::strcmp(name, "profile_rescore_counts") == 0) { ctx->profile_rescore_counts = value != 0; for (sp_ctx* h : ctx->helper) if (h) h->profile_rescore_counts = ctx->profile_rescore_counts; return SP_OK; }
     if (std::strcmp(name, "mm2_rescore") == 0) { ctx->mm2_rescore = (int)value; for (sp_ctx* h : ctx->helper) if (h) h->mm2_rescore = ctx->mm2_rescore; return SP_OK; }
     if (std::strcmp(name, "k8_side_orders") == 0) { if (value < 0 || value > 3) return sp_fail(ctx, SP_ERR_INVALID_ARG, "sp_ctx_set_option: k8_side_orders is 0 .. 3"); ctx->k8_side_orders = (int)value; for (sp_ctx* h : ctx->helper) if (h) h->k8_side_orders = ctx->k8_side_orders; return SP_OK; }
diff --git a/pb-starphase_amd/csrc/sp_hla_seed.hip b/pb-starphase_amd/csrc/sp_hla_seed.hip
--- a/pb-starphase_amd/csrc/sp_hla_seed.hip
+++ b/pb-starphase_amd/csrc/sp_hla_seed.hip
@@ -157,7 +157,8 @@
     if (!FILL && threadIdx.x == 0) cnt[rid] = running;
 }
 
-struct SeedCounters { unsigned long long seeds, anchors; uint32_t max_anchors, max_seeds, overflow_reads, seed_overflow, rev_selected, wide_cells; unsigned long long t[8]; };
+struct SeedCounters { unsigned long long seeds, anchors; uint32_t max_anchors, max_seeds, overflow_reads, seed_overflow, rev_selected, wide_cells; unsigned long long t[8];
+                      unsigned long long targets, patterns; };
 #ifdef SP_K1S_TIMING
 #define K1S_T(i) do { if (threadIdx.x == 0) { const unsigned long long now_ = wall_clock64(); atomicAdd(&ctr->t[i], now_ - t_last); t_last = now_; } } while (0)
 #else
@@ -259,7 +260,8 @@
 }
 
 struct SChain { int32_t score, f_end; uint32_t key, end, first, cnt; };
-struct SGroup { uint32_t read, key, off, cnt; };
+struct SGroup { uint32_t read, key, off, cnt, member_off, n_members; };
+struct STarget { uint32_t keymin, off, cnt, cls; };
 struct SSel { int32_t rid, rev, score, cnt, diag, qs, qe, rs, re, n_chains; };
 struct SDp { uint32_t key; int32_t f; int16_t p; uint16_t t; };
 
@@ -311,24 +313,42 @@
     if (c.key >> 15) { qs = qlen - e; qe = qlen - s; } else { qs = s; qe = e; }
 }
 
-struct BatchCursors { unsigned long long groups_anchors; uint32_t chains, dp_chunk, big_items, big_members, big_chunk, pad; };
-struct SBigItem { SGroup g; uint32_t member_off, n_members, pad0, pad1; };
-struct SMember { uint32_t read, key, shift, pad; };
+struct BatchCursors { unsigned long long targets_anchors; uint32_t chains, groups, members, big_items, pad0, pad1; };
+struct SBigItem { SGroup g; uint32_t pad0, pad1; };
+typedef uint32_t SMember;
+constexpr uint32_t CLS_BITS = 14, CLS_MASK = (1u << CLS_BITS) - 1u, CLS_EMPTY = 0xFFFFFFFFu;
+
+__device__ __forceinline__ uint32_t anchors_min_r(const uint32_t* __restrict__ a, uint32_t cnt, uint32_t first, uint32_t stride) {
+    uint32_t mn = 0xFFFFu;
+    for (uint32_t i = first; i < cnt; i += stride) { const uint32_t r = a[i] >> 16; mn = r < mn ? r : mn; }
+    return mn;
+}
+__device__ __forceinline__ void anchors_signature(const uint32_t* __restrict__ a, uint32_t cnt, uint32_t first, uint32_t stride, uint32_t mn, unsigned long long& s1, unsigned long long& s2) {
+    s1 = 0; s2 = 0;
+    for (uint32_t i = first; i < cnt; i += stride) {
+        const unsigned long long x = a[i] - (mn << 16);
+        s1 += mix64((x ^ 0x9E3779B97F4A7C15ull) & MZ_MASK) * 0x9E3779B97F4A7C15ull + x;
+        unsigned long long y = (x + 0x632BE59BD9B4E019ull) * 0xD6E8FEB86659FD93ull; y ^= y >> 32; y *= 0xD6E8FEB86659FD93ull; y ^= y >> 32;
+        s2 += y;
+    }
+}
 
 __global__ __launch_bounds__(CH_THREADS) void k1s_group_kernel(SeqSetView reads, IndexView ix, uint32_t r0, uint32_t n_batch, const uint4* __restrict__ seeds, const uint2* __restrict__ read_seed,
-                                                               uint32_t* __restrict__ anchors, uint32_t anchor_cap, SGroup* __restrict__ groups, uint32_t group_cap,
+                                                               uint32_t* __restrict__ anchors, uint32_t anchor_cap, STarget* __restrict__ targets, uint4* __restrict__ sigs, uint32_t target_cap,
+                                                               SGroup* __restrict__ groups, uint32_t group_cap, SMember* __restrict__ members, uint32_t member_cap, int dedup,
                                                                uint3* __restrict__ read_chain, BatchCursors* __restrict__ cur, SeedCounters* __restrict__ ctr) {
     extern __shared__ uint32_t tab[];
     __shared__ uint32_t s_hist[256], s_hista[256], s_first[256];
     __shared__ uint32_t s_scan[CH_THREADS / 64];
     __shared__ unsigned long long s_base;
+    __shared__ uint32_t s_ncls, s_mcur, s_base_r, s_base_m;
     const int tid = threadIdx.x;
     const uint32_t r = r0 + blockIdx.x;
     if (blockIdx.x >= n_batch) return;
     const uint2 rs_ = read_seed[r];
     const uint32_t s0 = rs_.x, K = rs_.y;
     const int qlen = reads.len[r];
-    uint32_t n_groups_read = 0, n_anchors_read = 0;
+    uint32_t n_groups_read = 0, n_anchors_read = 0, n_patterns_read = 0;
     unsigned long long t_last = 0;
 #ifdef SP_K1S_TIMING
     t_last = wall_clock64();
@@ -370,11 +390,11 @@
             }
             (void)my_g;
             if (tot_g == 0) { K1S_T(1); continue; }
-            if (tid == 0) s_base = atomicAdd(&cur->groups_anchors, (unsigned long long)tot_g << 32 | tot_a);
+            if (tid == 0) s_base = atomicAdd(&cur->targets_anchors, (unsigned long long)tot_g << 32 | tot_a);
             __syncthreads();
             const unsigned long long base = s_base;
             const uint32_t base_g = (uint32_t)(base >> 32), base_a = (uint32_t)base;
-            const bool fits = (unsigned long long)base_a + tot_a <= anchor_cap && (unsigned long long)base_g + tot_g <= group_cap;
+            const bool fits = (unsigned long long)base_a + tot_a <= anchor_cap && (unsigned long long)base_g + tot_g <= target_cap;
             if (!fits) { if (tid == 0) atomicAdd(&ctr->overflow_reads, 1u); continue; }
             for (uint32_t i = lo; i < hi; ++i) {
                 const uint32_t c = tab[i];
@@ -382,8 +402,8 @@
                 const uint32_t k = 255 - (c > 255 ? 255 : c);
                 const uint32_t slot = atomicAdd(&s_hist[k], 1u);
                 const uint32_t a_off = base_a + (c < 255 ? s_hista[k] + (slot - s_first[k]) * c : atomicAdd(&s_hista[k], c));
-                SGroup g; g.read = r; g.key = (uint32_t)rev << 15 | (rid_lo + i); g.off = a_off; g.cnt = c;
-                groups[base_g + slot] = g;
+                STarget t; t.keymin = (uint32_t)rev << 15 | (rid_lo + i); t.off = a_off; t.cnt = c; t.cls = 0;
+                targets[base_g + slot] = t;
                 tab[i] = a_off;
             }
             __syncthreads();
@@ -402,10 +422,91 @@
             }
             __syncthreads();
             K1S_T(2);
-            n_groups_read += tot_g; n_anchors_read += tot_a;
+            STarget* wt = targets + base_g;
+            const uint4* wsig = sigs + base_g;
+            if (dedup) {
+                const int lane = tid & 63, wave = tid >> 6;
+                const uint32_t n_wide = s_first[255 - 64];
+                for (uint32_t b = (uint32_t)wave; b < n_wide; b += CH_THREADS / 64) {
+                    const STarget t = wt[b];
+                    uint32_t mn = anchors_min_r(anchors + t.off, t.cnt, (uint32_t)lane, 64u);
+                    for (int o = 32; o > 0; o >>= 1) { const uint32_t x = (uint32_t)__shfl_xor((int)mn, o); mn = x < mn ? x : mn; }
+                    unsigned long long s1, s2;
+                    anchors_signature(anchors + t.off, t.cnt, (uint32_t)lane, 64u, mn, s1, s2);
+                    for (int o = 32; o > 0; o >>= 1) { s1 += __shfl_xor(s1, o); s2 += __shfl_xor(s2, o); }
+                    if (lane == 0) { sigs[base_g + b] = make_uint4((uint32_t)s1, (uint32_t)(s1 >> 32), (uint32_t)s2, (uint32_t)(s2 >> 32)); wt[b].keymin = t.keymin | mn << 16; }
+                }
+                for (uint32_t slot = n_wide + (uint32_t)tid; slot < tot_g; slot += CH_THREADS) {
+                    const STarget t = wt[slot];
+                    const uint32_t mn = anchors_min_r(anchors + t.off, t.cnt, 0u, 1u);
+                    unsigned long long s1, s2;
+                    anchors_signature(anchors + t.off, t.cnt, 0u, 1u, mn, s1, s2);
+                    sigs[base_g + slot] = make_uint4((uint32_t)s1, (uint32_t)(s1 >> 32), (uint32_t)s2, (uint32_t)(s2 >> 32)); wt[slot].keymin = t.keymin | mn << 16;
+                }
+                for (uint32_t i = tid; i < (uint32_t)WIN_KEYS; i += CH_THREADS) tab[i] = CLS_EMPTY;
+                if (tid == 0) { s_ncls = 0; s_mcur = 0; }
+                __syncthreads();
+                for (uint32_t slot = tid; slot < tot_g; slot += CH_THREADS) {
+                    const uint4 sg = wsig[slot]; const uint32_t cnt = wt[slot].cnt;
+                    uint32_t p = (sg.x ^ sg.y * 0x9E3779B1u ^ cnt * 0x85EBCA6Bu) % (uint32_t)WIN_KEYS, ord;
+                    for (;;) {
+                        uint32_t e = tab[p];
+                        if (e == CLS_EMPTY) { e = atomicCAS(&tab[p], CLS_EMPTY, slot << CLS_BITS | 1u); if (e == CLS_EMPTY) { ord = 1; atomicAdd(&s_ncls, 1u); break; } }
+                        const uint32_t rs = e >> CLS_BITS;
+                        const uint4 og = wsig[rs];
+                        if (wt[rs].cnt == cnt && og.x == sg.x && og.y == sg.y && og.z == sg.z && og.w == sg.w) { ord = (atomicAdd(&tab[p], 1u) & CLS_MASK) + 1u; break; }
+                        p = p + 1 == (uint32_t)WIN_KEYS ? 0u : p + 1;
+                    }
+                    wt[slot].cls = p << CLS_BITS | ord;
+                }
+            } else if (tid == 0) s_ncls = tot_g;
+            __syncthreads();
+            const uint32_t n_cls = s_ncls;
+            if (tid == 0) {
+                const uint32_t bm = atomicAdd(&cur->members, tot_g);
+                s_base_m = bm;
+                s_base_r = (unsigned long long)bm + tot_g <= member_cap ? atomicAdd(&cur->groups, n_cls) : 0xFFFFFFFFu;
+            }
+            __syncthreads();
+            const uint32_t base_r = s_base_r, base_m = s_base_m;
+            if (base_r == 0xFFFFFFFFu || (unsigned long long)base_r + n_cls > group_cap) {
+                if (base_r != 0xFFFFFFFFu) for (uint32_t i = tid; i < n_cls; i += CH_THREADS) if (base_r + i < group_cap) { SGroup g; g.read = r; g.key = 0; g.off = 0; g.cnt = 0; g.member_off = 0; g.n_members = 0; groups[base_r + i] = g; }
+                if (tid == 0) atomicAdd(&ctr->overflow_reads, 1u);
+                continue;
+            }
+            uint32_t done = 0;
+            for (uint32_t c0 = 0; c0 < tot_g; c0 += CH_THREADS) {
+                const uint32_t slot = c0 + (uint32_t)tid;
+                const bool in = slot < tot_g;
+                STarget t; t.keymin = 0; t.off = 0; t.cnt = 0; t.cls = 0;
+                if (in) t = wt[slot];
+                const bool is_rep = in && (!dedup || (t.cls & CLS_MASK) == 1u);
+                uint32_t total;
+                const uint32_t rk = block_rank(is_rep, s_scan, total);
+                if (is_rep) {
+                    uint32_t n_mem = 1, mbase = slot;
+                    if (dedup) { const uint32_t p = t.cls >> CLS_BITS; n_mem = tab[p] & CLS_MASK; mbase = atomicAdd(&s_mcur, n_mem); tab[p] = mbase << CLS_BITS | slot; }
+                    SGroup g; g.read = r; g.key = t.keymin & 0xFFFFu; g.off = t.off; g.cnt = t.cnt; g.member_off = base_m + mbase; g.n_members = n_mem;
+                    groups[base_r + done + rk] = g;
+                }
+                done += total;
+            }
+            __syncthreads();
+            for (uint32_t slot = tid; slot < tot_g; slot += CH_THREADS) {
+                const STarget t = wt[slot];
+                uint32_t at = slot, shift = 0;
+                if (dedup) {
+                    const uint32_t e = tab[t.cls >> CLS_BITS];
+                    at = (e >> CLS_BITS) + (t.cls & CLS_MASK) - 1u;
+                    shift = (t.keymin >> 16) - (wt[e & CLS_MASK].keymin >> 16);
+                }
+                members[base_m + at] = (t.keymin & 0xFFFFu) << 16 | (shift & 0xFFFFu);
+            }
+            n_groups_read += tot_g; n_anchors_read += tot_a; n_patterns_read += n_cls;
             K1S_T(3);
         }
     }
+    if (tid == 0 && n_groups_read) { atomicAdd(&ctr->targets, (unsigned long long)n_groups_read); atomicAdd(&ctr->patterns, (unsigned long long)n_patterns_read); }
     if (tid == 0) {
         const uint32_t cap = n_groups_read ? n_anchors_read / CH_MIN_CNT : 0u;
         const uint32_t off = cap ? atomicAdd(&cur->chains, cap) : 0u;
@@ -462,9 +563,35 @@
     }
 }
 
+__device__ __forceinline__ void emit_chain_to_members(uint32_t rd, uint32_t m_off, uint32_t n_mem, int sc, int zf, uint32_t end_key, uint32_t first_key, int cnt,
+                                                      const SMember* __restrict__ members, SChain* __restrict__ chains, uint32_t chain_cap, uint3* __restrict__ read_chain, int lane) {
+    uint32_t base = 0;
+    if (lane == 0) base = atomicAdd(&read_chain[rd].z, n_mem);
+    base = (uint32_t)__builtin_amdgcn_readfirstlane((int)base);
+    const uint3 rc = read_chain[rd];
+    SChain c; c.score = sc; c.f_end = zf; c.cnt = (uint32_t)cnt;
+    for (uint32_t m = (uint32_t)lane; m < n_mem; m += 64) {
+        const SMember mm = members[m_off + m];
+        const uint32_t at = base + m;
+        c.key = mm >> 16; c.end = end_key + (mm << 16); c.first = first_key + (mm << 16);
+        if (at < rc.y && rc.x + at < chain_cap) chains[rc.x + at] = c;
+    }
+}
+__device__ __forceinline__ void emit_class_chains(bool have, const SGroup& grp, int sc, int zf, uint32_t end_key, uint32_t first_key, int cnt, const SMember* __restrict__ members,
+                                                  SChain* __restrict__ chains, uint32_t chain_cap, uint3* __restrict__ read_chain, int lane) {
+    emit_chains(have && grp.n_members == 1u, grp, sc, zf, end_key, first_key, cnt, chains, chain_cap, read_chain, lane);
+    for (unsigned long long todo = __ballot(have && grp.n_members > 1u); todo; todo &= todo - 1) {
+        const int l = __builtin_ctzll(todo);
+        emit_chain_to_members((uint32_t)__builtin_amdgcn_readlane((int)grp.read, l), (uint32_t)__builtin_amdgcn_readlane((int)grp.member_off, l),
+                              (uint32_t)__builtin_amdgcn_readlane((int)grp.n_members, l), __builtin_amdgcn_readlane(sc, l), __builtin_amdgcn_readlane(zf, l),
+                              (uint32_t)__builtin_amdgcn_readlane((int)end_key, l), (uint32_t)__builtin_amdgcn_readlane((int)first_key, l), __builtin_amdgcn_readlane(cnt, l),
+                              members, chains, chain_cap, read_chain, lane);
+    }
+}
+
 template <int NS, int ND>
 __device__ __forceinline__ void dp_in_registers(const SGroup& grp, int n, const uint32_t* __restrict__ anchors, const int32_t* __restrict__ pen, uint32_t* __restrict__ wl, int lane,
-                                                SChain* __restrict__ chains, uint32_t chain_cap, uint3* __restrict__ read_chain) {
+                                                const SMember* __restrict__ members, SChain* __restrict__ chains, uint32_t chain_cap, uint3* __restrict__ read_chain) {
     uint32_t k[NS];
 #pragma unroll
     for (int i = 0; i < NS; ++i) k[i] = i < n ? anchors[grp.off + i] : 0xFFFFFFFFu;
@@ -526,7 +653,7 @@
                 if (have) { end_key = pick_key<NS>(k, zi); first_key = pick_key<NS>(k, first); }
             }
         }
-        emit_chains(have, grp, sc, zf, end_key, first_key, cnt, chains, chain_cap, read_chain, lane);
+        emit_class_chains(have, grp, sc, zf, end_key, first_key, cnt, members, chains, chain_cap, read_chain, lane);
     }
 }
 
@@ -536,7 +663,7 @@
     __builtin_amdgcn_fence(__ATOMIC_ACQUIRE, "wavefront");
 }
 __device__ __forceinline__ void dp_in_lds_rows(const SGroup& grp, int n, int mx, const uint32_t* __restrict__ anchors, const int32_t* __restrict__ pen, unsigned long long* __restrict__ wl, int lane,
-                                               SChain* __restrict__ chains, uint32_t chain_cap, uint3* __restrict__ read_chain) {
+                                               const SMember* __restrict__ members, SChain* __restrict__ chains, uint32_t chain_cap, uint3* __restrict__ read_chain) {
     uint32_t k[32];
 #pragma unroll
     for (int i = 0; i < 32; ++i) k[i] = i < n ? anchors[grp.off + i] : 0xFFFFFFFFu;
@@ -592,7 +719,7 @@
                 if (have) { end_key = (uint32_t)wl[zi * 32 + col]; first_key = (uint32_t)wl[first * 32 + col]; }
             }
         }
-        emit_chains(have, grp, sc, zf, end_key, first_key, cnt, chains, chain_cap, read_chain, lane);
+        emit_class_chains(have, grp, sc, zf, end_key, first_key, cnt, members, chains, chain_cap, read_chain, lane);
     }
     wave_sync_lds();
     }
@@ -625,7 +752,7 @@
 
 __device__ __forceinline__ void dp_by_wave(const SGroup& grp, SDp* __restrict__ a, const uint32_t* __restrict__ anchors, const int32_t* __restrict__ pen,
                                            SChain* __restrict__ chains, uint32_t chain_cap, uint3* __restrict__ read_chain, int lane, SeedCounters* __restrict__ ctr,
-                                           bool member, const SGroup& mine, uint32_t shift) {
+                                           const SMember* __restrict__ members) {
     const int n = (int)grp.cnt;
     unsigned long long t_last = 0;
 #ifdef SP_K1S_TIMING
@@ -711,7 +838,7 @@
         const int sc = i < 0 ? zf : zf - a[i].f;
         if (cnt == 0) a[zi].t = 4;
         wave_sync();
-        emit_chains(member && sc >= CH_MIN_SCORE && cnt >= CH_MIN_CNT, mine, sc, zf, a[zi].key + (shift << 16), a[first].key + (shift << 16), cnt, chains, chain_cap, read_chain, lane);
+        if (sc >= CH_MIN_SCORE && cnt >= CH_MIN_CNT) emit_chain_to_members(grp.read, grp.member_off, grp.n_members, sc, zf, a[zi].key, a[first].key, cnt, members, chains, chain_cap, read_chain, lane);
     }
     wave_sync();
 }
@@ -719,7 +846,7 @@
 __device__ __forceinline__ int rl(int v, int lane_idx) { return __builtin_amdgcn_readlane(v, __builtin_amdgcn_readfirstlane(lane_idx)); }
 
 __device__ __forceinline__ void dp_by_wave_regs(const SGroup& grp, const uint32_t* __restrict__ anchors, const int32_t* __restrict__ pen, SChain* __restrict__ chains, uint32_t chain_cap,
-                                                uint3* __restrict__ read_chain, int lane, bool member, const SGroup& mine, uint32_t shift) {
+                                                uint3* __restrict__ read_chain, int lane, const SMember* __restrict__ members) {
     const int n = (int)grp.cnt;
     const int my_j = 63 - lane;
     uint32_t raw = lane < n ? anchors[grp.off + lane] : 0xFFFFFFFFu;
@@ -794,20 +921,20 @@
         const int sc = i < 0 ? zf : zf - rl(f, 63 - i);
         if (cnt == 0 && my_j == zi) t = 4;
         const uint32_t end_key = (uint32_t)rl((int)key, 63 - zi), first_key = (uint32_t)rl((int)key, 63 - first);
-        emit_chains(member && sc >= CH_MIN_SCORE && cnt >= CH_MIN_CNT, mine, sc, zf, end_key + (shift << 16), first_key + (shift << 16), cnt, chains, chain_cap, read_chain, lane);
+        if (sc >= CH_MIN_SCORE && cnt >= CH_MIN_CNT) emit_chain_to_members(grp.read, grp.member_off, grp.n_members, sc, zf, end_key, first_key, cnt, members, chains, chain_cap, read_chain, lane);
     }
 }
 
 __global__ __launch_bounds__(CH_THREADS) void k1s_dp_kernel(const SGroup* __restrict__ groups, const uint32_t* __restrict__ anchors, const int32_t* __restrict__ pen_tab,
                                                             BatchCursors* __restrict__ cur, SChain* __restrict__ chains, uint32_t chain_cap, uint3* __restrict__ read_chain,
-                                                            SBigItem* __restrict__ items, SMember* __restrict__ members, uint32_t big_cap, SeedCounters* __restrict__ ctr) {
+                                                            SBigItem* __restrict__ items, const SMember* __restrict__ members, uint32_t big_cap, uint32_t group_cap, SeedCounters* __restrict__ ctr) {
     extern __shared__ uint32_t lds[];
     int32_t* pen = reinterpret_cast<int32_t*>(lds);
     const int tid = threadIdx.x, lane = tid & 63, wave = tid >> 6;
     uint32_t* wl = lds + 512 + wave * DP_WAVE_WORDS;
     for (int i = tid; i <= CH_BW; i += CH_THREADS) pen[i] = pen_tab[i];
     __syncthreads();
-    const uint32_t n_groups = (uint32_t)(cur->groups_anchors >> 32);
+    const uint32_t n_groups = cur->groups < group_cap ? cur->groups : group_cap;
     unsigned long long t_last = 0;
 #ifdef SP_K1S_TIMING
     t_last = wall_clock64();
@@ -821,7 +948,7 @@
         if (task >= n_tasks) continue;
         const uint32_t g0 = task * 64;
         const uint32_t gi = g0 + lane;
-        SGroup grp; grp.read = 0; grp.key = 0; grp.off = 0; grp.cnt = 0;
+        SGroup grp; grp.read = 0; grp.key = 0; grp.off = 0; grp.cnt = 0; grp.member_off = 0; grp.n_members = 0;
         if (gi < n_groups) grp = groups[gi];
         const int n = (int)grp.cnt;
         const int small_n = n <= DP_REG_MAX ? n : 0;
@@ -832,9 +959,9 @@
         if (mx > 8) { }
         else
 #endif
-        if (mx > 8) dp_in_lds_rows(grp, small_n, mx, anchors, pen, reinterpret_cast<unsigned long long*>(wl), lane, chains, chain_cap, read_chain);
-        else if (mx > 4) dp_in_registers<8, 8>(grp, small_n, anchors, pen, wl, lane, chains, chain_cap, read_chain);
-        else if (mx > 0) dp_in_registers<4, 4>(grp, small_n, anchors, pen, wl, lane, chains, chain_cap, read_chain);
+        if (mx > 8) dp_in_lds_rows(grp, small_n, mx, anchors, pen, reinterpret_cast<unsigned long long*>(wl), lane, members, chains, chain_cap, read_chain);
+        else if (mx > 4) dp_in_registers<8, 8>(grp, small_n, anchors, pen, wl, lane, members, chains, chain_cap, read_chain);
+        else if (mx > 0) dp_in_registers<4, 4>(grp, small_n, anchors, pen, wl, lane, members, chains, chain_cap, read_chain);
 #ifdef SP_K1S_TIMING
         if (lane == 0) { const unsigned long long now_ = wall_clock64(); atomicAdd(&ctr->t[mx > 8 ? 5 : 4], now_ - t_last); t_last = now_; }
 #endif
@@ -844,47 +971,13 @@
         const unsigned long long big = __ballot(n > DP_REG_MAX);
 #endif
         if (!big) continue;
-        unsigned long long h1 = 0, h2 = 0; uint32_t min_r = 0;
-        for (unsigned long long todo = big; todo; todo &= todo - 1) {
-            const int l = __builtin_ctzll(todo);
-            const uint32_t off = (uint32_t)__builtin_amdgcn_readlane((int)grp.off, l), cnt = (uint32_t)__builtin_amdgcn_readlane((int)grp.cnt, l);
-            uint32_t mn = 0xFFFFu;
-            for (uint32_t i = lane; i < cnt; i += 64) { const uint32_t r = anchors[off + i] >> 16; mn = r < mn ? r : mn; }
-            for (int o = 32; o > 0; o >>= 1) { const uint32_t t = (uint32_t)__shfl_xor((int)mn, o); mn = t < mn ? t : mn; }
-            unsigned long long s1 = 0, s2 = 0;
-            for (uint32_t i = lane; i < cnt; i += 64) {
-                const unsigned long long x = anchors[off + i] - (mn << 16);
-                s1 += mix64((x ^ 0x9E3779B97F4A7C15ull) & MZ_MASK) * 0x9E3779B97F4A7C15ull + x;
-                unsigned long long y = (x + 0x632BE59BD9B4E019ull) * 0xD6E8FEB86659FD93ull; y ^= y >> 32; y *= 0xD6E8FEB86659FD93ull; y ^= y >> 32;
-                s2 += y;
-            }
-            for (int o = 32; o > 0; o >>= 1) { s1 += __shfl_xor(s1, o); s2 += __shfl_xor(s2, o); }
-            if (lane == l) { h1 = s1; h2 = s2; min_r = mn; }
-        }
-        int rep = -1;
-        for (unsigned long long todo = big; todo; todo &= todo - 1) {
-            const int l = __builtin_ctzll(todo);
-            const unsigned long long b1 = __shfl(h1, l), b2 = __shfl(h2, l);
-            const int bn = __builtin_amdgcn_readlane(n, l);
-            if (rep < 0 && n > DP_REG_MAX && n == bn && h1 == b1 && h2 == b2) rep = l;
-        }
-        const unsigned long long reps = __ballot(n > DP_REG_MAX && rep == lane);
-        uint32_t item0 = 0, mem0 = 0;
-        if (lane == 0) { item0 = atomicAdd(&cur->big_items, (uint32_t)__builtin_popcountll(reps)); mem0 = atomicAdd(&cur->big_members, (uint32_t)__builtin_popcountll(big)); }
-        item0 = (uint32_t)__builtin_amdgcn_readfirstlane((int)item0); mem0 = (uint32_t)__builtin_amdgcn_readfirstlane((int)mem0);
-        uint32_t k_item = 0, k_mem = 0;
-        for (unsigned long long todo = reps; todo; todo &= todo - 1) {
-            const int l = __builtin_ctzll(todo);
-            const unsigned long long mem = __ballot(n > DP_REG_MAX && rep == l);
-            const uint32_t rep_min = (uint32_t)__builtin_amdgcn_readlane((int)min_r, l);
-            if (item0 + k_item < big_cap && mem0 + k_mem + (uint32_t)__builtin_popcountll(mem) <= big_cap) {
-                if (rep == l && n > DP_REG_MAX) {
-                    SMember m; m.read = grp.read; m.key = grp.key; m.shift = min_r - rep_min; m.pad = 0;
-                    members[mem0 + k_mem + (uint32_t)__builtin_popcountll(mem & ((1ull << lane) - 1ull))] = m;
-                }
-                if (lane == l) { SBigItem it; it.g = grp; it.member_off = mem0 + k_mem; it.n_members = (uint32_t)__builtin_popcountll(mem); it.pad0 = it.pad1 = 0; items[item0 + k_item] = it; }
-            } else if (lane == l) atomicAdd(&ctr->overflow_reads, 1u);
-            ++k_item; k_mem += (uint32_t)__builtin_popcountll(mem);
+        uint32_t item0 = 0;
+        if (lane == 0) item0 = atomicAdd(&cur->big_items, (uint32_t)__builtin_popcountll(big));
+        item0 = (uint32_t)__builtin_amdgcn_readfirstlane((int)item0);
+        if (n > DP_REG_MAX) {
+            const uint32_t at = item0 + (uint32_t)__builtin_popcountll(big & ((1ull << lane) - 1ull));
+            if (at < big_cap) { SBigItem it; it.g = grp; it.pad0 = it.pad1 = 0; items[at] = it; }
+            else atomicAdd(&ctr->overflow_reads, 1u);
         }
         K1S_TW(6);
     }
@@ -909,13 +1002,8 @@
         const SBigItem it = items[x];
         if ((it.g.cnt > 64) != LONG) continue;
         if (LONG && it.g.cnt > (uint32_t)DP_BIG_MAX) { if (lane == 0) atomicAdd(&ctr->overflow_reads, 1u); continue; }
-        for (uint32_t m0 = 0; m0 < it.n_members; m0 += 64) {
-            const bool member = m0 + lane < it.n_members;
-            SGroup mine = it.g; uint32_t shift = 0;
-            if (member) { const SMember m = members[it.member_off + m0 + lane]; mine.read = m.read; mine.key = m.key; shift = m.shift; }
-            if (!LONG) dp_by_wave_regs(it.g, anchors, pen, chains, chain_cap, read_chain, lane, member, mine, shift);
-            else dp_by_wave(it.g, reinterpret_cast<SDp*>(wl), anchors, pen, chains, chain_cap, read_chain, lane, ctr, member, mine, shift);
-        }
+        if (!LONG) dp_by_wave_regs(it.g, anchors, pen, chains, chain_cap, read_chain, lane, members);
+        else dp_by_wave(it.g, reinterpret_cast<SDp*>(wl), anchors, pen, chains, chain_cap, read_chain, lane, ctr, members);
     }
 }
 
@@ -1313,12 +1401,16 @@
     const uint64_t c_cap = g_cap;
     uint32_t* d_anchors = (uint32_t*)sp_pool(ctx, "k1s_anchors", std::max<uint64_t>(a_cap, 1) * 4);
     SGroup* d_groups = (SGroup*)sp_pool(ctx, "k1s_groups", g_cap * sizeof(SGroup));
+    const char* mc_env = std::getenv("SP_K1S_MEMBER_CAP");
+    const uint64_t m_cap = mc_env && std::atoll(mc_env) > 0 ? std::min<uint64_t>(g_cap, (uint64_t)std::atoll(mc_env)) : g_cap;
+    STarget* d_targets = (STarget*)sp_pool(ctx, "k1s_targets", g_cap * sizeof(STarget));
+    uint4* d_sigs = (uint4*)sp_pool(ctx, "k1s_sigs", g_cap * sizeof(uint4));
+    SMember* d_members = (SMember*)sp_pool(ctx, "k1s_members", g_cap * sizeof(SMember));
     SChain* d_chains = (SChain*)sp_pool(ctx, "k1s_chains", c_cap * sizeof(SChain));
     int32_t* d_parent = (int32_t*)sp_pool(ctx, "k1s_parent", c_cap * 4);
     const uint64_t big_cap = a_cap / (DP_REG_MAX + 1) + 64;
     SBigItem* d_items = (SBigItem*)sp_pool(ctx, "k1s_big_items", big_cap * sizeof(SBigItem));
-    SMember* d_members = (SMember*)sp_pool(ctx, "k1s_big_members", big_cap * sizeof(SMember));
-    if (!d_anchors || !d_groups || !d_chains || !d_parent || !d_items || !d_members) return sp_fail(ctx, SP_ERR_OUT_OF_MEMORY, "seeded K1: chain buffers");
+    if (!d_anchors || !d_groups || !d_chains || !d_parent || !d_items || !d_members || !d_targets || !d_sigs) return sp_fail(ctx, SP_ERR_OUT_OF_MEMORY, "seeded K1: chain buffers");
     const size_t group_lds = (size_t)WIN_KEYS * 4, dp_lds = (size_t)(512 + (CH_THREADS / 64) * DP_WAVE_WORDS) * 4;
     SP_HIP_CHECK(ctx, hipFuncSetAttribute((const void*)k1s_group_kernel, hipFuncAttributeMaxDynamicSharedMemorySize, (int)group_lds));
     SP_HIP_CHECK(ctx, hipFuncSetAttribute((const void*)k1s_dp_kernel, hipFuncAttributeMaxDynamicSharedMemorySize, (int)dp_lds));
@@ -1339,11 +1431,11 @@
         {
             ProfScope ps(ctx, "k1s_groups", a);
             hipLaunchKernelGGL(k1s_group_kernel, dim3(nb_reads), dim3(CH_THREADS), group_lds, ctx->stream, reads->view(), ix, r0, nb_reads, d_seeds, d_read_seed, d_anchors, (uint32_t)a_cap,
-                               d_groups, (uint32_t)g_cap, d_read_chain, d_cur, d_ctr);
+                               d_targets, d_sigs, (uint32_t)g_cap, d_groups, (uint32_t)g_cap, d_members, (uint32_t)m_cap, ctx->k1s_dedup, d_read_chain, d_cur, d_ctr);
         }
         {
             ProfScope ps(ctx, "k1s_dp", a);
-            hipLaunchKernelGGL(k1s_dp_kernel, dim3((unsigned)ctx->num_cus * 8), dim3(CH_THREADS), dp_lds, ctx->stream, d_groups, d_anchors, idx->d_pen, d_cur, d_chains, (uint32_t)c_cap, d_read_chain, d_items, d_members, (uint32_t)big_cap, d_ctr);
+            hipLaunchKernelGGL(k1s_dp_kernel, dim3((unsigned)ctx->num_cus * 8), dim3(CH_THREADS), dp_lds, ctx->stream, d_groups, d_anchors, idx->d_pen, d_cur, d_chains, (uint32_t)c_cap, d_read_chain, d_items, d_members, (uint32_t)big_cap, (uint32_t)g_cap, d_ctr);
         }
         {
             ProfScope ps(ctx, "k1s_dp_big", a);
@@ -1380,6 +1472,7 @@
 #ifdef SP_K1S_TIMING
     fprintf(stderr, "k1s_group phases (100 MHz ticks summed over workgroups): count %llu scan %llu scatter %llu records %llu; dp kernel waves: task + load %llu, up to 8 anchors %llu, 9..26 %llu, signatures of the large %llu\n", hc.t[0], hc.t[1], hc.t[2], hc.t[3], hc.t[7], hc.t[4], hc.t[5], hc.t[6]);
 #endif
+    ctx->prof["k1s_targets"].cells += hc.targets; ctx->prof["k1s_patterns"].cells += hc.patterns;
     if (hc.overflow_reads) {
         ctx->prof["k1s_truncated_reads"].cells += hc.overflow_reads;
         ctx->warning = "seeded K1: " + std::to_string(hc.overflow_reads) + " capacity events (seed / anchor / chain lists of a read cut short) in the last sp_hla_realign_reads call: "
diff --git a/pb-starphase_amd/csrc/sp_internal.h b/pb-starphase_amd/csrc/sp_internal.h
--- a/pb-starphase_amd/csrc/sp_internal.h
+++ b/pb-starphase_amd/csrc/sp_internal.h
@@ -81,6 +81,7 @@
     hipStream_t ctl_stream = nullptr;
     hipEvent_t ev_fork = nullptr, ev_join = nullptr;
     int k1_best_n = 5;
+    int k1s_dedup = 1;
     int profile_rescore_counts = 0;
     int mm2_rescore = 1;
     int k8_persistent = 2;
```

After: 364,000 reads/s (median of 6 runs). +1.9%, better.
